# sine2pi/ASR-model

Hardware: AMD Instinct MI355X
Metric: audio-sec/sec fwd+bwd on 30s@16kHz LibriSpeech-shaped clips (whole job, all GPUs) (higher is better)
Workload: dtype bf16; 1 GPU; tiny (BASELINE configs[1]): log-mel + 4 enc/4 dec d=384 h=6 fwd+bwd, 32 x 30 s clips per GPU, T=256; model=tiny, global_batch=32, seq_len=3001, text_len=256, pitch_frames=3001, parallelism=dp1

## Files before the change

### asr-model_amd/asrx/gemm.py

```python
from __future__ import annotations

import torch

from . import lib, prec, probe

ACT = {"none": 0, "gelu": 1, "silu": 2, "sigmoid": 3, "relu": 4}


BF16 = torch.bfloat16


def is_bf16(t) -> bool:
    return t is not None and t.dtype == BF16


def gemm(A, B, C, *, M, N, K, lda, ldb, ldc, a_kc=True, b_kc=True, batch=1, sA=0, sB=0, sC=0,
         bias=None, Z=None, alpha=1.0, beta=0.0, act="none", conv_a=False, conv_b=False,
         conv_F=0, conv_C=0, splitk=1, precision=None):
    lib.require_gpu(A, B, C)
    if is_bf16(A) or is_bf16(B) or is_bf16(C):
        raise RuntimeError("asrx_gemm takes fp32 operands; bf16-stored activations go through the wide GEMM")
    p = prec.get() if precision is None else precision
    e0 = probe.begin("gemm")
    lib.call("asrx_gemm", p, lib.ptr(A), lda, sA, int(a_kc), int(conv_a), lib.ptr(B), ldb, sB,
# ... 234 lines not shown

def use_wide(K) -> bool:
    return prec.get() == prec.PREC_BF16 and K % 8 == 0


def gemm_wn_rows(A, Wb, C, *, M, N, K, lda, ldc, mtiles, bias=None, alpha=1.0, beta=0.0):
    return gemm_wn(A, Wb, C, M=M, N=N, K=K, lda=lda, ldc=ldc, bias=bias, alpha=alpha, beta=beta, mtiles=mtiles)


def row_tiles(next_i, layer, L, M, device=None):
    n = int(lib.load().asrx_row_tiles_max(M))
    dev = device if device is not None else next_i.device
    tl = torch.empty(n, dtype=torch.int32, device=dev)
    cnt = torch.empty(1, dtype=torch.int32, device=dev)
    lib.call("asrx_row_tiles", lib.ptr(next_i), layer, L, M, lib.ptr(tl), lib.ptr(cnt), lib.stream())
    return tl, cnt


def linear_fwd(x, W, b=None, act="none", out=None, preact=None, wbf=None, mtiles=None, out_bf16=False):
    x2 = _rows(x)
    if not x2.is_contiguous():
        x2 = x2.contiguous()
    M, K = x2.shape
    N = W.shape[0]
    wide = use_wide(K)
    if is_bf16(x2) and not wide:
        x2 = x2.float()
    odt = BF16 if (out_bf16 and wide and N % 4 == 0) else torch.float32
    y = out if out is not None else torch.empty(*x.shape[:-1], N, device=x.device, dtype=odt)
    if wide and mtiles is not None and act == "none" and preact is None:
        gemm_wn_rows(x2, weight_bf16(W) if wbf is None else wbf, y, M=M, N=N, K=K, lda=K, ldc=N, bias=b,
                     mtiles=mtiles)
    elif use_wide(K):
        gemm_wn(x2, weight_bf16(W) if wbf is None else wbf, y, M=M, N=N, K=K, lda=K, ldc=N, bias=b, act=act,
                Z=preact)
    else:
        gemm(x2, W, y, M=M, N=N, K=K, lda=K, ldb=K, ldc=N, a_kc=True, b_kc=True, bias=b, act=act,
             Z=preact)
    return y


def linear_rot_fwd(x, W, b, m, tab, L, hd, scale, preact=None):
    x2 = _rows(x)
    if not x2.is_contiguous():
        x2 = x2.contiguous()
    M, K = x2.shape
    N = W.shape[0]
    Wb = weight_bf16(W)
    y = torch.empty(*x.shape[:-1], N, device=x.device)
    nj = _nj(M, N)
    ab = int(is_bf16(x2))
    lib.require_gpu(x2, Wb, y, m, tab)
    e0 = probe.begin("gemm")
    lib.call("asrx_gemm_wn_rot", lib.ptr(x2), ab, K, lib.ptr(Wb), Wb.stride(0), lib.ptr(y), lib.ptr(preact), N,
             lib.ptr(b), lib.ptr(m), lib.ptr(tab), L, hd, float(scale), M, N, K, nj, lib.stream())
    probe.end("gemm", e0, 2.0 * M * N * K, ("wn", M, N, K, nj, 0, "rot", preact is not None, False, ab, 0, -1))
    return y


def linear_dgrad(dy, W, out=None, beta=0.0, mtiles=None):
    """dx = dy @ W for dy (..., N), W (N, K); mtiles as in linear_fwd."""
    d2 = _rows(dy)
    if not d2.is_contiguous():
        d2 = d2.contiguous()
    M, N = d2.shape
    K = W.shape[1]
    dx = out if out is not None else torch.empty(*dy.shape[:-1], K, device=dy.device, dtype=torch.float32)
    if use_wide(N) and mtiles is not None:
        gemm_wn_rows(d2, weight_bf16(W, trans=True), dx, M=M, N=K, K=N, lda=N, ldc=K, beta=beta, mtiles=mtiles)
    elif use_wide(N):
        gemm_wn(d2, weight_bf16(W, trans=True), dx, M=M, N=K, K=N, lda=N, ldc=K, beta=beta)
    else:
        gemm(d2, W, dx, M=M, N=K, K=N, lda=N, ldb=K, ldc=K, a_kc=True, b_kc=False, beta=beta)
    return dx


def _splitk_for(m_rows: int, tiles: int) -> int:
    want = max(1, 512 // max(tiles, 1))
    return int(max(1, min(want, m_rows // 256)))


FUSED_BIAS_GRAD = True
BIAS_CHECK = None


def _wgrad(A, lda, x2, out, M, K, rows, db=None):
    tiles = ((M + 127) // 128) * ((K + 127) // 128)
    sk = _splitk_for(rows, tiles)

    def staged(a_bf16, b_bf16, name, *tag):
        lib.require_gpu(A, x2, out)
        e0 = probe.begin("gemm")
        if db is not None and not FUSED_BIAS_GRAD:
            staged_db, db_ = db, None
        else:
            staged_db, db_ = None, db
        if db_ is not None:
            before = db_.clone() if BIAS_CHECK is not None else None
            lib.call("asrx_wgrad_bias", lib.ptr(A), a_bf16, lda, lib.ptr(x2), b_bf16, K, lib.ptr(out), out.stride(0),
                     lib.ptr(db), M, K, rows, sk, lib.stream())
            if before is not None:
                Af = A.float() if a_bf16 else A
                ref = torch.zeros(M, device=A.device)
                lib.call("asrx_colsum_ld", lib.ptr(Af), Af.stride(0) if a_bf16 else lda, lib.ptr(ref), rows, M,
                         lib.stream())
                absum = Af.as_strided((rows, M), (Af.stride(0) if a_bf16 else lda, 1)).abs().sum(0)
                tol = 1e-5 * absum + 2.0 ** -22 * (before.abs() + ref.abs())
                BIAS_CHECK.append((db_ - before, ref, tol, dict(M=M, K=K, rows=rows, sk=sk, a_bf16=a_bf16,
                                                                  b_bf16=b_bf16, lda=lda, ldo=out.stride(0))))
        elif name == "asrx_wgrad_bf16":
            lib.call(name, lib.ptr(A), lda, lib.ptr(x2), K, lib.ptr(out), out.stride(0), M, K, rows, sk, lib.stream())
        else:
            lib.call(name, lib.ptr(A), lda, lib.ptr(x2), b_bf16, K, lib.ptr(out), out.stride(0), M, K, rows, sk,
                     lib.stream())
        probe.end("gemm", e0, 2.0 * M * K * rows, ("wgrad", M, K, rows, sk) + tag)
        if staged_db is not None:
            Af = A.float() if a_bf16 else A
            lib.call("asrx_colsum_ld", lib.ptr(Af), Af.stride(0) if a_bf16 else lda, lib.ptr(staged_db), rows, M,
                     lib.stream())
        return out

    if is_bf16(A):
        xb = is_bf16(x2)
        if M % 8 or K % (8 if xb else 4) or lda % 8 or x2.stride(0) != K or A.data_ptr() % 16 or x2.data_ptr() % 16:
            A = A.float()
            lda = A.stride(0)
        else:
            return staged(1, int(xb), "asrx_wgrad_bf16_ab", 2 + int(xb))
    if is_bf16(x2):
        if M % 4 or K % 8 or lda % 4 or x2.stride(0) != K or A.data_ptr() % 16:
            x2 = x2.float()
        else:
            return staged(0, 1, "asrx_wgrad_bf16_ex", 1)
    ok4 = M % 4 == 0 and K % 4 == 0 and lda % 4 == 0 and A.data_ptr() % 16 == 0 and x2.data_ptr() % 16 == 0
    if prec.get() == prec.PREC_BF16 and ok4 and x2.stride(0) == K and (tiles <= 9 or rows <= 16384
                                                                        or (rows <= 50000 and tiles <= 72)):
        return staged(0, 0, "asrx_wgrad_bf16")
    gemm(A, x2, out, M=M, N=K, K=rows, lda=lda, ldb=K, ldc=K, a_kc=False, b_kc=False, beta=1.0, splitk=sk)
    if db is not None:
        lib.call("asrx_colsum_ld", lib.ptr(A), lda, lib.ptr(db), rows, M, lib.stream())
    return out


def wgrad_cols(dy, c0, n, x, out):
    rows, ld = dy.shape
    return _wgrad(dy[:, c0:], ld, x, out, n, x.shape[1], rows)


def linear_wgrad(dy, x, out=None, accumulate=False, db=None):
    d2 = _rows(dy)
    x2 = _rows(x)
    if not d2.is_contiguous():
        d2 = d2.contiguous()
    if not x2.is_contiguous():
        x2 = x2.contiguous()
    M, N = d2.shape
    K = x2.shape[1]
    if out is None:
        out = torch.zeros(N, K, device=dy.device, dtype=torch.float32)
    elif not accumulate:
        out.zero_()
    return _wgrad(d2, N, x2, out, N, K, M, db=db)
```

### asr-model_amd/asrx/lib.py

```python
from __future__ import annotations

import ctypes
import os

import torch

_HERE = os.path.dirname(os.path.abspath(__file__))
LIB_PATH = os.environ.get("ASRX_LIB") or os.path.join(_HERE, "libasrx.so")

_i64 = ctypes.c_int64
_i32 = ctypes.c_int
_f32 = ctypes.c_float
_p = ctypes.c_void_p
_u32 = ctypes.c_uint32

SIGNATURES = {
    "asrx_last_error": (ctypes.c_char_p, []),
    "asrx_abi_version": (_i32, []),
    "asrx_noise_hash": (_u32, [_u32, _u32]),
    "asrx_set_noise_epoch": (_i32, [_u32, _p]),
    "asrx_set_gemm_variant": (_i32, [_i32]),
    "asrx_set_attn_variant": (_i32, [_i32]),
    "asrx_set_wgrad_variant": (_i32, [_i32]),
    "asrx_mel_frames": (_i32, [_i64]),
    "asrx_logmel_ws_bytes": (_i64, [_i64, _i64]),
    "asrx_flac_info": (_i32, [_p, _i64, _p, _p, _p, _p, _p]),
    "asrx_flac_decode": (_i32, [_p, _i64, _p, _i64]),
    "asrx_pcm_normalize": (_i32, [_p, _i32, _i64, _i64, _i64, _p, _p, _p, _i64, _i32, _p]),
    "asrx_logmel": (_i32, [_p, _i64, _i64, _i64, _p, _p, _p, _p, _i32, _i64, _p, _p, _i64, _p]),
    "asrx_gemm": (
        _i32,
        [_i32, _p, _i64, _i64, _i32, _i32, _p, _i64, _i64, _i32, _i32, _p, _i64, _i64, _p, _p,
         _i64, _i64, _i64, _i64, _f32, _f32, _i32, _i64, _i64, _i32, _p],
    ),
    "asrx_abby_fwd": (_i32, [_p, _p, _p, _p, _p, _p, _p, _i64, _i64, _i64, _i64, _i64, _u32, _i32, _p]),
    "asrx_abby_fwd_logits": (_i32, [_p, _p, _p, _p, _p, _p, _i64, _i64, _i64, _i64, _i64, _u32, _i32, _p]),
    "asrx_abby_bwd": (_i32, [_p, _p, _p, _p, _p, _p, _p, _p, _p, _p, _i64, _i64, _p]),
    "asrx_attn_fwd": (_i32, [_i32, _p, _p, _p, _p, _p, _p, _p, _p, _p, _i64, _i64, _i64, _i64, _i64, _i32, _f32, _p]),
    "asrx_attn_bwd": (_i32, [_i32, _p, _p, _p, _p, _p, _p, _p, _p, _p, _p, _p, _p, _p, _p, _p, _p, _p, _p,
                             _i64, _i64, _i64, _i64, _i64, _i32, _f32, _p]),
    "asrx_layernorm_fwd": (_i32, [_p, _p, _p, _p, _p, _p, _i64, _i64, _f32, _p]),
    "asrx_layernorm_bwd": (_i32, [_p, _p, _p, _p, _p, _p, _p, _p, _i64, _i64, _p]),
    "asrx_layernorm_bwd_acc": (_i32, [_p, _p, _p, _p, _p, _p, _p, _p, _i64, _i64, _i32, _p]),
    "asrx_small_linear_fwd": (_i32, [_p, _p, _p, _p, _i64, _i64, _i64, _i32, _p]),
    "asrx_small_linear_bwd": (_i32, [_p, _p, _p, _p, _p, _p, _p, _i64, _i64, _i64, _i32, _f32, _p]),
    "asrx_rownorm": (_i32, [_p, _p, _i64, _i64, _p]),
    "asrx_rownorm_bwd": (_i32, [_p, _p, _p, _p, _i64, _i64, _p]),
    "asrx_row_normalize": (_i32, [_p, _p, _p, _i64, _i64, _p]),
    "asrx_row_normalize_bwd": (_i32, [_p, _p, _p, _p, _i64, _i64, _i32, _p]),
    "asrx_softmax_small": (_i32, [_p, _p, _i64, _i64, _p]),
    "asrx_softmax_small_bwd": (_i32, [_p, _p, _p, _i64, _i64, _p]),
    "asrx_zero": (_i32, [_p, _i64, _p]),
    "asrx_rotary_fwd": (_i32, [_p, _p, _p, _p, _i64, _i64, _i64, _i64, _f32, _p]),
    "asrx_rotary_bwd": (_i32, [_p, _p, _p, _p, _p, _p, _i64, _i64, _i64, _i64, _f32, _p]),
    "asrx_abby_bwd2": (_i32, [_p] * 10 + [_i64, _i64, _i32, _p]),
    "asrx_rownorm_bwd2": (_i32, [_p, _p, _p, _p, _i64, _i64, _i32, _p]),
    "asrx_colsum_ld": (_i32, [_p, _i64, _p, _i64, _i64, _p]),
    "asrx_ce_fwd1": (_i32, [_p] * 6 + [_i64, _i64, _p]),
    "asrx_ce_bwd2": (_i32, [_p] * 6 + [_i64, _i64, _p]),
    "asrx_bn_running": (_i32, [_p] * 5 + [_i64, _i64, _i64, _f32, _f32, _p]),
    "asrx_rsqrt_eps": (_i32, [_p, _p, _i64, _f32, _p]),
    "asrx_conv3_weight": (_i32, [_p, _p, _i64, _i64] + [_p] * 6),
    "asrx_conv3_weight_bwd": (_i32, [_p] * 4 + [_i64, _i64] + [_p] * 3),
    "asrx_blend_fwd": (_i32, [_p] * 4 + [_i64, _p]),
    "asrx_blend_bwd": (_i32, [_p] * 7 + [_i64, _p]),
    "asrx_add_segments": (_i32, [_p, _i64, _p, _p, _p, _i64, _p]),
    "asrx_cat3": (_i32, [_p] * 3 + [_i64, _p, _p]),
    "asrx_layernorm_fwd2": (_i32, [_p] * 10 + [_i32, _i64, _i64, _f32, _p]),
    "asrx_vgate_weights": (_i32, [_p] * 7 + [_i64, _i64, _i64, _p]),
    "asrx_msheath_row_fwd": (_i32, [_p] * 6 + [_i64] + [_p] * 14 + [_i64] * 4 + [_f32, _f32, _p, _i64, _i64, _p]),
    "asrx_msheath_row_bwd": (_i32, [_p] * 11 + [_i64] + [_p] * 18 + [_i64] * 4 + [_f32, _p, _i64, _i64, _p]),
    "asrx_gemm_wn_rows": (_i32, [_p, _i64, _p, _i64, _p, _i64, _p, _p, _i64, _i64, _i64, _f32, _f32, _i32, _i32, _p,
                                 _p, _p]),
    "asrx_row_tiles_max": (_i64, [_i64]),
    "asrx_wgrad_bf16": (_i32, [_p, _i64, _p, _i64, _p, _i64, _i64, _i64, _i64, _i64, _p]),
    "asrx_pitch_dio": (_i32, [_p, _i64, _i64, _i64] + [ctypes.c_double] * 5 + [_p, _i64, _p, _p, _p, _p, _i64]
                       + [_p] * 4 + [_i64] + [_p] * 4 + [_i64, _p]),
    "asrx_pitch_stonemask": (_i32, [_p, _i64, _i64, _i64, ctypes.c_double, _p, ctypes.c_double, _i64, _p, _p]),
    "asrx_wconv_entry_bytes": (_i64, []),
    "asrx_weights_to_bf16": (_i32, [_p, _i64, _i64, _p]),
    "asrx_row_tiles": (_i32, [_p, _i64, _i64, _i64, _p, _p, _p]),
    "asrx_msheath_ctrl_fwd3": (_i32, [_p, _p, _i64, _p, _p, _p, _p, _p, _i64, _p, _p, _p, _p] + [_i64] * 5 + [_p] * 8),
    "asrx_mem_chunks": (_i64, [_i64]),
    "asrx_seg_colsum_det": (_i32, [_p, _p, _p, _i64, _i64, _i64, _f32, _p]),
    "asrx_msheath_ctrl_bwd3": (_i32, [_p, _p, _p, _p, _p, _p, _i64, _p, _p, _p] + [_i64] * 4 + [_p, _i32] + [_p] * 8),
    "asrx_axpy_row2_colsum": (_i32, [_p] * 6 + [_i64] * 3 + [_p, _i64, _p]),
    "asrx_vgate_fwd": (_i32, [_p, _p, _p, _p, _p, _p, _p, _p, _p, _p, _p, _p, _p, _i64, _i64, _i64, _f32, _p]),
    "asrx_vgate_bwd": (_i32, [_p, _p, _p, _p, _p, _p, _p, _p, _p, _p, _p, _p, _p, _p, _p, _p, _p,
                              _i64, _i64, _i64, _f32, _p]),
    "asrx_tgate_fwd": (_i32, [_p, _p, _p, _i64, _i64, _p]),
    "asrx_tgate_bwd": (_i32, [_p, _p, _p, _p, _p, _i64, _i64, _p]),
    "asrx_axpy_row": (_i32, [_p, _p, _p, _p, _i64, _i64, _p]),
    "asrx_axpy_row_bwd": (_i32, [_p, _p, _p, _p, _p, _i64, _i64, _p]),
    "asrx_axpy_row_bwd2": (_i32, [_p, _p, _p, _p, _p, _p, _i64, _i64, _p]),
    "asrx_jump_select": (_i32, [_p, _p, _p, _p, _p, _p, _p, _p, _i64, _i64, _i64, _p]),
    "asrx_jump_select_bwd": (_i32, [_p, _p, _p, _p, _p, _p, _p, _p, _p, _p, _p, _p, _i64, _i64, _i64, _p]),
    "asrx_seg_colsum": (_i32, [_p, _p, _i64, _i64, _i64, _f32, _i32, _p]),
    "asrx_msheath_ctrl_fwd": (_i32, [_p, _p, _i64, _p, _p, _p, _p, _p, _p, _i64, _i64, _i64, _i64, _i64,
                                     _p, _p, _p, _p, _p, _p, _p, _p]),
    "asrx_msheath_ctrl_bwd": (_i32, [_p, _p, _p, _p, _p, _p, _p, _p, _p, _i64, _i64, _i64, _i64, _p, _p, _p, _p, _p,
                                     _p]),
    "asrx_msheath_rec_bytes": (_i64, []),
    "asrx_msheath_ctrl_fwd2": (_i32, [_p, _p, _i64, _p, _p, _p, _i64, _p, _p, _p, _i64, _i64, _i64, _i64, _i64,
                                      _p, _p, _p, _p, _p, _p, _p, _p]),
    "asrx_msheath_ctrl_bwd2": (_i32, [_p, _p, _p, _p, _p, _p, _i64, _p, _p, _p, _i64, _i64, _i64, _i64, _p, _i32,
                                      _p, _p, _p, _p, _p, _p]),
    "asrx_jump_select4_bwd_acc": (_i32, [_p, _p, _p, _p, _p, _p, _p, _p, _p, _p, _p, _p, _p, _i64, _i64, _i64, _p]),
    "asrx_jump_bwd_part_floats": (_i64, [_i64, _i64, _i64]),
    "asrx_jump_select4_bwd_part": (_i32, [_p] * 11 + [_i64, _i64, _i64, _p]),
    "asrx_msheath_ctrl_bwd4": (_i32, [_p, _i64, _p, _p, _p, _i64, _p, _p, _p, _i64, _i64, _i64, _i64, _p, _i32]
                               + [_p] * 8),
    "asrx_axpy_row2_bwd_acc": (_i32, [_p, _p, _f32, _p, _p, _p, _p, _p, _p, _p, _p, _i64, _i64, _i64, _p]),
    "asrx_msheath_dx_final": (_i32, [_p, _p, _p, _p, _i64, _i64, _i64, _p]),
    "asrx_axpy_row2": (_i32, [_p, _p, _p, _p, _p, _i64, _i64, _p]),
    "asrx_axpy_row2_bwd": (_i32, [_p, _p, _p, _p, _p, _p, _p, _i64, _i64, _p]),
    "asrx_jump_select4": (_i32, [_p, _p, _p, _p, _p, _p, _p, _p, _i64, _i64, _i64, _p]),
    "asrx_jump_select4_bwd": (_i32, [_p, _p, _p, _p, _p, _p, _p, _p, _p, _p, _p, _p, _i64, _i64, _i64, _p]),
    "asrx_colsum": (_i32, [_p, _p, _i64, _i64, _p]),
    "asrx_add_rows": (_i32, [_p, _p, _p, _p, _i64, _i64, _i64, _p]),
    "asrx_lincomb": (_i32, [_p, _p, _p, _f32, _f32, _f32, _p, _i64, _p]),
    "asrx_act_fwd": (_i32, [_p, _p, _i64, _i32, _p]),
    "asrx_act_bwd": (_i32, [_p, _p, _p, _i64, _i32, _p]),
    "asrx_glu_fwd": (_i32, [_p, _p, _i64, _i64, _p]),
    "asrx_glu_bwd": (_i32, [_p, _p, _p, _i64, _i64, _p]),
    "asrx_dropout": (_i32, [_p, _p, _i64, _i64, _i64, _i64, _u32, _f32, _p]),
    "asrx_act_dropout_fwd": (_i32, [_p, _p, _p, _i64, _i64, _i64, _i64, _u32, _f32, _i32, _i32, _p]),
    "asrx_act_dropout_bwd": (_i32, [_p, _p, _p, _i64, _i64, _i64, _i64, _u32, _f32, _i32, _i32, _p]),
    "asrx_dwconv_fwd": (_i32, [_p, _p, _p, _p, _i64, _i64, _i64, _i64, _p]),
    "asrx_dwconv_bwd": (_i32, [_p, _p, _p, _p, _p, _p, _i64, _i64, _i64, _i64, _p]),
    "asrx_bn_fwd": (_i32, [_p, _p, _p, _p, _p, _p, _i64, _i64, _i64, _f32, _i32, _p]),
    "asrx_bn_bwd": (_i32, [_p, _p, _p, _p, _p, _p, _p, _p, _p, _p, _i64, _i64, _i64, _p]),
    "asrx_dwconv_pre_bwd": (_i32, [_p, _p, _p, _p, _p, _p, _p, _i64, _i64, _i64, _i64, _i32, _p]),
    "asrx_bn_silu_fwd": (_i32, [_p, _p, _p, _p, _p, _p, _i64, _i64, _i64, _f32, _i32, _p]),
    "asrx_bn_silu_bwd": (_i32, [_p, _p, _p, _p, _p, _p, _p, _p, _p, _p, _p, _i64, _i64, _i64, _p]),
    "asrx_stem1_fwd": (_i32, [_p, _p, _p, _p, _i64, _i64, _i64, _p]),
    "asrx_stem1_bwd": (_i32, [_p, _p, _p, _p, _i64, _i64, _i64, _p]),
    "asrx_embed_fwd": (_i32, [_p, _p, _p, _i64, _i64, _p]),
    "asrx_embed_bwd": (_i32, [_p, _p, _p, _i64, _i64, _p]),
    "asrx_ce_fwd": (_i32, [_p, _p, _p, _p, _i64, _i64, _p]),
    "asrx_ce_bwd": (_i32, [_p, _p, _p, _p, _p, _i64, _i64, _p]),
    "asrx_policy_noise": (_i32, [_p, _i64, _i64, _i64, _u32, _p]),
    "asrx_weight_to_bf16": (_i32, [_p, _p, _i64, _i64, _i64, _i32, _p]),
    "asrx_gemm_wn_router": (_i32, [_p, _i64, _p, _i64, _p, _p, _p, _i64, _p, _i64, _i64, _i64, _p]),
    "asrx_gemm_wn": (_i32, [_p, _i64, _i32, _i64, _i64, _p, _i64, _p, _i64, _p, _p, _i64, _i64, _i64, _f32, _f32,
                            _i32, _i32, _p]),
    "asrx_gemm_wn_ex": (_i32, [_p, _i32, _i64, _i32, _i64, _i64, _p, _i64, _p, _i32, _i64, _p, _p, _i64, _i64, _i64,
                               _f32, _f32, _i32, _i32, _p, _p, _p]),
    "asrx_wgrad_bf16_ex": (_i32, [_p, _i64, _p, _i32, _i64, _p, _i64, _i64, _i64, _i64, _i64, _p]),
    "asrx_abby_fwd2": (_i32, [_p, _p, _p, _p, _p, _i32, _p, _p, _i64, _i64, _i64, _i64, _i64, _u32, _i32, _p, _p, _p,
                              _p]),
    "asrx_gemm_wn_gact": (_i32, [_p, _i32, _i64, _p, _i64, _p, _p, _i64, _p, _i64, _p, _i64, _i64, _i64, _i32, _i32,
                                 _p]),
    "asrx_rotary_table": (_i32, [_p, _p, _i64, _i64, _p]),
    "asrx_rotary_fwd2": (_i32, [_p, _p, _p, _p, _p, _i64, _i64, _i64, _i64, _f32, _p]),
    "asrx_rotary_bwd2": (_i32, [_p, _p, _p, _p, _p, _p, _p, _i64, _i64, _i64, _i64, _f32, _p]),
    "asrx_abby_fwd3": (_i32, [_p, _p, _p, _p, _p, _p, _i32, _p, _p, _i64, _i64, _i64, _i64, _i64, _u32, _i32, _p, _p,
                               _p, _p, _p]),
    "asrx_abby_fwd_logits2": (_i32, [_p, _p, _p, _p, _i32, _p, _p, _i64, _i64, _i64, _i64, _i64, _u32, _i32, _p, _p,
                                     _p, _p]),
    "asrx_attn_fwd2": (_i32, [_i32, _i32, _p, _p, _p, _p, _p, _p, _p, _p, _p, _i64, _i64, _i64, _i64, _i64, _i32, _f32,
                              _p]),
    "asrx_attn_bwd2": (_i32, [_i32, _i32, _p, _p, _p, _p, _p, _p, _p, _p, _p, _p, _p, _p, _p, _p, _p, _p, _p, _p,
                              _i64, _i64, _i64, _i64, _i64, _i32, _f32, _p]),
    "asrx_small_linear_fwd2": (_i32, [_p, _i32, _p, _p, _p, _i64, _i64, _i64, _i32, _p]),
    "asrx_small_linear_bwd2": (_i32, [_p, _p, _p, _i32, _p, _p, _p, _p, _i64, _i64, _i64, _i32, _f32, _p]),
    "asrx_tgate_fwd2": (_i32, [_p, _p, _p, _i32, _i64, _i64, _p]),
    "asrx_msheath_row_fwd2": (_i32, [_p] * 6 + [_i64] + [_p] * 7 + [_i32] + [_p] * 7 + [_i64] * 4
                                    + [_f32, _f32, _p, _i64, _i64, _p]),
    "asrx_msheath_row_fwd3": (_i32, [_p] * 6 + [_i64] + [_p] * 16 + [_i64] * 4 + [_f32, _f32, _p, _i64, _i64, _p]),
    "asrx_layernorm_fwd3": (_i32, [_p, _p, _p, _p, _i32] + [_p] * 6 + [_i32, _i64, _i64, _f32, _p]),
    "asrx_jump_axpy_inplace": (_i32, [_p] * 10 + [_i64, _i64, _i64, _p]),
    "asrx_wave_pool": (_i32, [_p, _i64, _i64, _i64, _i64, _p, _p]),
    "asrx_maxfactor_param_bytes": (_i32, []),
    "asrx_maxfactor_step": (_i32, [_p, _i32, _i64, _i64, _i64, _i64, _i64, _p, _p]),
    "asrx_maxfactor_step_ex": (_i32, [_p, _i32, _i64, _i64, _i64, _i64, _i64, _p, _p, _i32, _p]),
    "asrx_grad_stats_param_bytes": (_i32, []),
    "asrx_grad_stats": (_i32, [_p, _i32, _i64, _f32, _f32, _f32, _p, _p, _p]),
    "asrx_abby_record_cond": (_i32, [_p]),
    "asrx_gemm_wn_ce": (_i32, [_p, _i64, _p, _i64, _p, _i64, _p, _i64, _i64, _i64, _i32, _p]),
    "asrx_gemm_wn_ce_f32": (_i32, [_p, _i64, _p, _i64, _p, _i64, _p, _i64, _i64, _i64, _i32, _p]),
    "asrx_ce_part_fwd": (_i32, [_p, _i64] + [_p] * 6 + [_i64, _i64, _p]),
    "asrx_ce_part_fwd_f32": (_i32, [_p, _i64] + [_p] * 6 + [_i64, _i64, _p]),
    "asrx_ce_bwd_bf16": (_i32, [_p] * 6 + [_i64, _i64, _p]),
    "asrx_ce_bwd_f32in": (_i32, [_p] * 6 + [_i64, _i64, _p]),
    "asrx_wgrad_bf16_ab": (_i32, [_p, _i64, _p, _i32, _i64, _p, _i64, _i64, _i64, _i64, _i64, _p]),
    "asrx_wgrad_bias": (_i32, [_p, _i32, _i64, _p, _i32, _i64, _p, _i64, _p, _i64, _i64, _i64, _i64, _p]),
    "asrx_act_bwd_bias": (_i32, [_p, _p, _p, _p, _i64, _i64, _i32, _p]),
    "asrx_abby_fwd_res": (_i32, [_p] * 9 + [_i64] * 5 + [_u32, _i32, _p]),
    "asrx_gemm_wn_res": (_i32, [_p, _i64, _p, _i64, _p, _i64, _p, _p, _i64, _i64, _i64, _i64, _i32, _p]),
    "asrx_gemm_wn_rot": (_i32, [_p, _i32, _i64, _p, _i64, _p, _p, _i64, _p, _p, _p, _i64, _i64, _f32, _i64, _i64,
                                _i64, _i32, _p]),
    "asrx_msheath_plan_bytes": (_i64, []),
    "asrx_msheath_layer_bytes": (_i64, []),
    "asrx_msheath_fwd_ws_bytes": (_i64, [_p, _i64, _i64, _i64]),
    "asrx_msheath_fwd": (_i32, [_p, _p, _p, _i64, _p, _p, _i64, _i64, _i64, _i64, _p]),
# ... 95 lines not shown
```

### asr-model_amd/asrx/msheath.py

```python
from __future__ import annotations

import ctypes
import math

import torch

from . import gemm as G
from . import decisions, lib, ops, prec

_E = torch.empty
_P = lib.ptr
_S = lib.stream
SIG = G.ACT["sigmoid"]
SILU = G.ACT["silu"]

_REC = None

ROW_DIMS = (128, 256, 384, 512, 768, 1024)

DETERMINISTIC = True
ROW_COLSUM = __import__("os").environ.get("ASRX_ROW_COLSUM", "1") != "0"


def _rec_bytes():
    global _REC
    if _REC is None:
        _REC = int(lib.load().asrx_msheath_rec_bytes())
    return _REC


def supported(mod, D):
    return D in ROW_DIMS and all(lay["v_gate"].mkey.shape[0] <= 64 for lay in mod.layers)


def _params(mod):
    ps = [mod.pnet.net[0].weight, mod.pnet.net[0].bias, mod.pnet.net[2].weight, mod.pnet.net[2].bias, mod.mem_w,
          mod.mem_gate[0].weight, mod.mem_gate[0].bias, mod.jump_s, mod.mlp_gate[0].weight, mod.mlp_gate[0].bias,
          mod.mlp_ln.weight, mod.mlp_ln.bias, mod.mlp[0].weight, mod.mlp[0].bias, mod.mlp[2].weight, mod.mlp[2].bias]
    for i, lay in enumerate(mod.layers):
        vg = lay["v_gate"]
        ps += [lay["ln"].weight, lay["ln"].bias, lay["gate"][0].weight, lay["gate"][0].bias, vg.mkey, vg.mval,
               vg.mlp[0].weight, vg.mlp[0].bias, vg.mlp[2].weight, vg.mlp[2].bias, vg.concat.weight, vg.concat.bias]
        if lay["adapter"] is not None:
            ps += [lay["adapter"].weight, lay["adapter"].bias]
    return ps


ACT_SOFTMAX = 16


def forward(mod, x0, gpol, save, tag=None):
    B, L, D = x0.shape
    rows = B * L
    dev = x0.device
    st = _S()
    sv = {} if save else None
    nchunk = int(lib.load().asrx_mem_chunks(L))
    part = _E(len(mod.layers) + 1, B, nchunk, D, device=dev)
    pooled = _E(B, D, device=dev)
    lib.call("asrx_seg_colsum_det", _P(x0), _P(part[-1]), _P(pooled), B, L, D, 1.0 / L, st)
    net = mod.pnet.net
    zp = _E(B, net[0].weight.shape[0], device=dev) if save else None
    hp = G.linear_fwd(pooled, net[0].weight, net[0].bias, act="silu", preact=zp)
    policy = _E(B, 3, device=dev)
    lib.call("asrx_small_linear_fwd", _P(hp), _P(net[2].weight), _P(net[2].bias), _P(policy), B, hp.shape[1], 3,
             ACT_SOFTMAX, st)
    nl = len(mod.layers)
    wide = G.use_wide(D)
    mg = mod.mem_gate[0]
    mem_w, ld_mw = mod.mem_w, 0
    next_i = None
    x = x0
    rec_bytes = _rec_bytes()
    wsr = _E(nl, 7, rows, device=dev)
    wsb = _E(nl, 5, B, device=dev)
    wsd = _E(nl, 3, B, D, device=dev)
    wsc = _E(nl, B * rec_bytes, dtype=torch.uint8, device=dev)
    a_r, a_b, a_d, a_c = wsr.data_ptr(), wsb.data_ptr(), wsd.data_ptr(), wsc.data_ptr()
    if save:
        sv["ws"] = (wsr, wsb, wsd, wsc)
    inv_sqrt_d = 1.0 / math.sqrt(D)
    layers = []
    for i, lay in enumerate(mod.layers):
        vg = lay["v_gate"]
        Dh = vg.mlp[0].weight.shape[0]
        M = vg.mkey.shape[0]
        N = M + Dh

        def build(vg=vg, M=M, Dh=Dh, N=N):
            Wc, bc, mkn = _E(N, D, device=dev), _E(N, device=dev), _E(M, device=dev)
            wb = _E(N, D, dtype=torch.int16, device=dev) if wide else None
            lib.call("asrx_vgate_weights", _P(vg.mkey), _P(vg.mlp[0].weight), _P(vg.mlp[0].bias), _P(Wc), _P(bc),
                     _P(mkn), _P(wb), M, Dh, D, st)
            return Wc, bc, mkn, wb

        Wc, bc, mkn, wb = G.derived(("vgate", bool(wide)), build, (vg.mkey, vg.mlp[0].weight, vg.mlp[0].bias))
        mt = G.row_tiles(next_i, i, L, rows, dev) if (wide and next_i is not None) else None
        SH = G.linear_fwd(x, Wc, bc, wbf=wb, mtiles=mt)
        ln, gt = lay["ln"], lay["gate"][0]
        ad = lay["adapter"]
        pxb = int(ad is not None and wide and prec.bf16_storage())
        px = _E(B, L, D, device=dev, dtype=torch.bfloat16 if pxb else torch.float32)
        mean, rstd, nx, gv, ion, kv, m2 = (a_r + 4 * rows * (7 * i + j) for j in range(7))
        x_new = _E(B, L, D, device=dev) if save else None
        if ad is None and ROW_COLSUM:
            lib.call("asrx_msheath_row_fwd3", _P(x), _P(ln.weight), _P(ln.bias), _P(gt.weight), _P(gt.bias), _P(SH),
                     N, _P(vg.mval), _P(vg.mlp[2].weight), _P(vg.mlp[2].bias), _P(vg.concat.weight),
                     _P(vg.concat.bias), _P(vg.tx), _P(px), _P(mean), _P(rstd), _P(nx), _P(gv), _P(ion), _P(kv), _P(m2),
                     _P(x_new), _P(part[i]), rows, D, M, Dh, float(ln.eps), inv_sqrt_d, _P(next_i), i, L, st)
            out = px
        else:
            lib.call("asrx_msheath_row_fwd2", _P(x), _P(ln.weight), _P(ln.bias), _P(gt.weight), _P(gt.bias), _P(SH),
                     N, _P(vg.mval), _P(vg.mlp[2].weight), _P(vg.mlp[2].bias), _P(vg.concat.weight),
                     _P(vg.concat.bias), _P(vg.tx), _P(px), pxb, _P(mean), _P(rstd), _P(nx), _P(gv), _P(ion), _P(kv),
                     _P(m2), rows, D, M, Dh, float(ln.eps), inv_sqrt_d, _P(next_i), i, L, st)
            out = G.linear_fwd(px, ad.weight, ad.bias, mtiles=mt) if ad is not None else px
            lib.call("asrx_axpy_row2_colsum", _P(x), _P(gv), _P(ion), _P(out), _P(x_new), _P(part[i]), B, L, D,
                     _P(next_i), i, st)
        alpha, beta, active, next_out, mem_v = (a_b + 4 * B * (5 * i + j) for j in range(5))
        gam, mwo, mem = (a_d + 4 * B * D * (3 * i + j) for j in range(3))
        rec = a_c + B * rec_bytes * i
        gp = gpol[:, i]
        lib.call("asrx_msheath_ctrl_fwd3", _P(policy), _P(gp), gp.stride(0), _P(ion), _P(mg.weight), _P(mg.bias),
                 _P(mem_v), _P(mem_w), ld_mw, _P(part[i]), _P(mem), _P(mod.jump_s), _P(next_i), i, nl, B, L, D,
                 _P(alpha), _P(beta), _P(gam), _P(mwo), _P(active), _P(next_out), _P(rec), st)
        if tag is not None and decisions.active():
            decisions.msheath_layer(tag[0], tag[1], i, wsr[i, 4].view(B, L), wsc[i].view(torch.float32).view(B, -1))
        if save:
            x_out = _E(B, L, D, device=dev)
            lib.call("asrx_jump_select4", _P(x_new), _P(x0), _P(x), _P(active), _P(alpha), _P(beta), _P(gam),
                     _P(x_out), B, L, D, st)
        else:
            x_out = _E(B, L, D, device=dev) if i == 0 else x
            lib.call("asrx_jump_axpy_inplace", _P(x), _P(x_out), _P(gv), _P(ion), _P(out), _P(x0), _P(active),
                     _P(alpha), _P(beta), _P(gam), B, L, D, st)
        if save:
            layers.append(dict(x=x, Wc=Wc, mkn=mkn, SH=SH, nx=nx, kv=kv, m2=m2, px=px, mean=mean, rstd=rstd,
                               out=out, g=gv, ion=ion, x_new=x_new, mem=mem, mem_v=mem_v, mem_w=mem_w, ld_mw=ld_mw,
                               rec=rec, active=active, alpha=alpha, beta=beta, next_i=next_i, mt=mt))
        mem_w, ld_mw, next_i = mwo, D, next_out
        x = x_out
    gate = _E(rows, device=dev)
    hb = int(wide and prec.bf16_storage())
    hln = _E(B, L, D, device=dev, dtype=torch.bfloat16 if hb else torch.float32)
    mean2, rstd2 = _E(rows, device=dev), _E(rows, device=dev)
    lib.call("asrx_layernorm_fwd3", _P(x), _P(mod.mlp_ln.weight), _P(mod.mlp_ln.bias), _P(hln), hb, _P(mean2),
             _P(rstd2), None, _P(mod.mlp_gate[0].weight), _P(mod.mlp_gate[0].bias), _P(gate), 1, rows, D,
             float(mod.mlp_ln.eps), st)
    rec1 = save and G.can_recompute_act(hln, mod.mlp[0].weight, "silu")
    z1 = _E(B, L, mod.mlp[0].weight.shape[0], device=dev) if save and not rec1 else None
    a1 = G.linear_fwd(hln, mod.mlp[0].weight, mod.mlp[0].bias, act="silu", preact=z1,
                      out_bf16=prec.bf16_storage())
    hh = G.linear_fwd(a1, mod.mlp[2].weight, mod.mlp[2].bias)
    y = _E(B, L, D, device=dev)
    lib.call("asrx_axpy_row", _P(x), _P(gate), _P(hh), _P(y), rows, D, st)
    if save:
        sv.update(x0=x0, pooled=pooled, zp=zp, hp=hp, policy=policy, layers=layers, x=x, gate=gate, hln=hln,
                  mean2=mean2, rstd2=rstd2, z1=z1, a1=a1, hh=hh)
    return y, sv


class MSheathFn(torch.autograd.Function):
    @staticmethod
    def forward(ctx, x0, gpol, mod, tag, *params):
        x0 = x0 if x0.is_contiguous() else x0.contiguous()
        y, sv = forward(mod, x0, gpol, save=True, tag=tag)
        ctx.mod, ctx.sv = mod, sv
        return y

    @staticmethod
    def backward(ctx, gy):
        mod, sv = ctx.mod, ctx.sv
        ctx.sv = None
        gy = gy if gy.is_contiguous() else gy.contiguous()
        x0 = sv["x0"]
        B, L, D = x0.shape
        rows = B * L
        dev = x0.device
        st = _S()
        touched = []

        def gb(p):
            touched.append(p)
            return ops._gbuf(p, True)

        x = sv["x"]
        dx = _E(B, L, D, device=dev)
        dhh = _E(B, L, D, device=dev)
        dgate = _E(rows, device=dev)
        lib.call("asrx_axpy_row_bwd2", _P(gy), _P(sv["gate"]), _P(sv["hh"]), _P(dhh), _P(dgate), _P(dx), rows, D, st)
        mg = mod.mlp_gate[0]
        lib.call("asrx_small_linear_bwd", _P(dgate), _P(sv["gate"]), _P(x), _P(mg.weight), _P(dx), _P(gb(mg.weight)),
                 _P(gb(mg.bias)), rows, D, 1, SIG, 1.0, st)
        m0, m2l = mod.mlp[0], mod.mlp[2]
        da1 = G.linear_dgrad(dhh, m2l.weight)
        G.linear_wgrad(dhh, sv["a1"], out=gb(m2l.weight), accumulate=True, db=gb(m2l.bias))
        H1 = da1.shape[-1]
        if sv["z1"] is None:
            ga1 = _E(da1.shape, dtype=torch.bfloat16, device=dev)
            G.linear_gact(sv["hln"], m0.weight, m0.bias, da1, ga1, "silu", db=gb(m0.bias))
            da1 = ga1
        elif prec.get() == prec.PREC_BF16 and H1 % 8 == 0 and G.use_wide(H1):
            ga1 = _E(da1.shape, dtype=torch.bfloat16, device=dev)
            lib.call("asrx_act_bwd_bias", _P(da1), _P(sv["z1"]), _P(ga1), _P(gb(m0.bias)), rows, H1, SILU, st)
            da1 = ga1
        else:
            lib.call("asrx_act_bwd", _P(da1), _P(sv["z1"]), _P(da1), da1.numel(), SILU, st)
            ops.colsum(da1.view(rows, -1), out=gb(m0.bias))
        dhln = G.linear_dgrad(da1, m0.weight)
        G.linear_wgrad(da1, sv["hln"], out=gb(m0.weight), accumulate=True)
        lib.call("asrx_layernorm_bwd_acc", _P(dhln), _P(x), _P(mod.mlp_ln.weight), _P(sv["mean2"]), _P(sv["rstd2"]),
                 _P(dx), _P(gb(mod.mlp_ln.weight)), _P(gb(mod.mlp_ln.bias)), rows, D, 1, st)
        del dhh, da1, dhln
        nl = len(mod.layers)
        g_policy = _E(B, 3, device=dev)
        has_orig = _E(B, dtype=torch.int32, device=dev)
        lib.call("asrx_zero", _P(has_orig), B * 4, st)
        dorig = _E(B, L, D, device=dev)
        g_mwo = None
        mg_w, mg_b = mod.mem_gate[0].weight, mod.mem_gate[0].bias
        inv_sqrt_d = 1.0 / math.sqrt(D)
        for i in range(nl - 1, -1, -1):
            s = sv["layers"][i]
            lay = mod.layers[i]
            vg = lay["v_gate"]
            M, Dh = vg.mkey.shape[0], vg.mlp[0].weight.shape[0]
            N = M + Dh
            xi = s["x"]
            dxi = _E(B, L, D, device=dev)
            dxn = _E(B, L, D, device=dev)
            g_mem_w, g_mem = _E(B, D, device=dev), _E(B, D, device=dev)
            if DETERMINISTIC:
                part = _E(int(lib.load().asrx_jump_bwd_part_floats(B, L, D)), device=dev)
                lib.call("asrx_jump_select4_bwd_part", _P(dx), _P(s["x_new"]), _P(x0), _P(s["active"]),
                         _P(s["alpha"]), _P(s["beta"]), _P(has_orig), _P(dxn), _P(dorig), _P(dxi), _P(part), B, L, D,
                         st)
                lib.call("asrx_msheath_ctrl_bwd4", _P(part), L, _P(g_mwo), _P(s["mem_v"]), _P(s["mem_w"]),
                         s["ld_mw"], _P(s["mem"]), _P(mod.jump_s), _P(s["rec"]), i, nl, B, D, _P(g_policy),
                         int(i != nl - 1), _P(g_mem_w), _P(g_mem), _P(gb(mod.jump_s)), _P(has_orig), _P(mg_w),
                         _P(gb(mg_w)), _P(gb(mg_b)), st)
            else:
                dctl = _E(B * (2 + D), device=dev)
                dalpha, dbeta, dgam = dctl[:B], dctl[B:2 * B], dctl[2 * B:]
                lib.call("asrx_jump_select4_bwd_acc", _P(dx), _P(s["x_new"]), _P(x0), _P(s["active"]),
                         _P(s["alpha"]), _P(s["beta"]), _P(has_orig), _P(dxn), _P(dorig), _P(dxi), _P(dalpha),
                         _P(dbeta), _P(dgam), B, L, D, st)
                lib.call("asrx_msheath_ctrl_bwd3", _P(dalpha), _P(dbeta), _P(dgam), _P(g_mwo), _P(s["mem_v"]),
                         _P(s["mem_w"]), s["ld_mw"], _P(s["mem"]), _P(mod.jump_s), _P(s["rec"]), i, nl, B, D,
                         _P(g_policy), int(i != nl - 1), _P(g_mem_w), _P(g_mem), _P(gb(mod.jump_s)), _P(has_orig),
                         _P(mg_w), _P(gb(mg_w)), _P(gb(mg_b)), st)
            dout = _E(B, L, D, device=dev)
            dgv, dion = _E(rows, device=dev), _E(rows, device=dev)
            lib.call("asrx_axpy_row2_bwd_acc", _P(dxn), _P(g_mem), 1.0 / L, _P(s["active"]), _P(s["g"]), _P(s["ion"]),
                     _P(s["out"]), _P(dout), _P(dgv), _P(dion), _P(dxi), B, L, D, st)
            del dxn
            ad = lay["adapter"]
            if ad is not None:
                dpx = G.linear_dgrad(dout, ad.weight, mtiles=s["mt"])
                G.linear_wgrad(dout, s["px"], out=gb(ad.weight), accumulate=True, db=gb(ad.bias))
            else:
                dpx = dout
            ln, gt = lay["ln"], lay["gate"][0]
            dSH = _E(rows, N, device=dev)
            lib.call("asrx_msheath_row_bwd", _P(dpx), _P(xi), _P(ln.weight), _P(ln.bias), _P(s["mean"]),
                     _P(s["rstd"]), _P(dgv), _P(s["g"]), _P(gt.weight), _P(dion), _P(s["SH"]), N, _P(s["nx"]),
                     _P(vg.mval), _P(vg.mlp[2].weight), _P(vg.concat.weight), _P(s["kv"]), _P(s["m2"]), _P(dxi),
                     _P(gb(ln.weight)), _P(gb(ln.bias)), _P(gb(gt.weight)), _P(gb(gt.bias)), _P(dSH),
                     _P(gb(vg.mval)), _P(gb(vg.mlp[2].weight)), _P(gb(vg.mlp[2].bias)), _P(gb(vg.concat.weight)),
                     _P(gb(vg.concat.bias)), _P(gb(vg.mlp[0].bias)), rows, D, M, Dh, inv_sqrt_d, _P(s["next_i"]), i,
                     L, st)
            del dout, dpx
            G.linear_dgrad(dSH, s["Wc"], out=dxi, beta=1.0, mtiles=s["mt"])
            x2 = xi.view(rows, D)
            dmk = _E(M, D, device=dev)
            lib.call("asrx_zero", _P(dmk), dmk.numel() * 4, st)
            G.wgrad_cols(dSH, 0, M, x2, dmk)
            lib.call("asrx_row_normalize_bwd", _P(dmk), _P(s["Wc"]), _P(s["mkn"]), _P(gb(vg.mkey)), M, D, 1, st)
            G.wgrad_cols(dSH, M, Dh, x2, gb(vg.mlp[0].weight))
            del dSH, dmk
            g_mwo = g_mem_w
            dx = dxi
        lib.call("asrx_colsum", _P(g_mwo), _P(gb(mod.mem_w)), B, D, st)
        net = mod.pnet.net
        g_pl = _E(B, 3, device=dev)
        lib.call("asrx_softmax_small_bwd", _P(g_policy), _P(sv["policy"]), _P(g_pl), B, 3, st)
        dhp = _E(sv["hp"].shape, device=dev)
        lib.call("asrx_small_linear_bwd", _P(g_pl), None, _P(sv["hp"]), _P(net[2].weight), _P(dhp),
                 _P(gb(net[2].weight)), _P(gb(net[2].bias)), B, dhp.shape[1], 3, 0, 0.0, st)
        lib.call("asrx_act_bwd", _P(dhp), _P(sv["zp"]), _P(dhp), dhp.numel(), SILU, st)
        dpooled = G.linear_dgrad(dhp, net[0].weight)
        G.linear_wgrad(dhp, sv["pooled"], out=gb(net[0].weight), accumulate=True)
        ops.colsum(dhp, out=gb(net[0].bias))
        u = _E(B, D, device=dev)
        lib.call("asrx_lincomb", _P(dpooled), None, None, 1.0 / L, 0.0, 0.0, _P(u), B * D, st)
        lib.call("asrx_msheath_dx_final", _P(dx), _P(dorig), _P(has_orig), _P(u), B, L, D, st)
        seen = set()
        for p in touched:
            if id(p) not in seen:
                seen.add(id(p))
                ops._gret(p, p.grad, True)
        return (dx, None, None, None) + (None,) * len(ctx.needs_input_grad[4:])


COMPOSITE = True


class _Layer(ctypes.Structure):
    _fields_ = [(n, ctypes.c_void_p) for n in ("ln_w", "ln_b", "gate_w", "gate_b", "mval", "vw2", "vb2", "cw", "cb",
                                                "tx", "bc", "wcb", "ad_wb", "ad_b")] + \
               [("M", ctypes.c_int64), ("Dh", ctypes.c_int64), ("ln_eps", ctypes.c_float), ("px_bf16", ctypes.c_int32)]


class _Plan(ctypes.Structure):
    _fields_ = [("p0_wb", ctypes.c_void_p), ("p0_b", ctypes.c_void_p), ("p2_w", ctypes.c_void_p),
                ("p2_b", ctypes.c_void_p), ("p_hidden", ctypes.c_int64), ("mem_w", ctypes.c_void_p),
                ("mg_w", ctypes.c_void_p), ("mg_b", ctypes.c_void_p), ("jump_s", ctypes.c_void_p),
                ("mln_w", ctypes.c_void_p), ("mln_b", ctypes.c_void_p), ("mln_eps", ctypes.c_float),
                ("hln_bf16", ctypes.c_int32), ("mgate_w", ctypes.c_void_p), ("mgate_b", ctypes.c_void_p),
                ("m0_wb", ctypes.c_void_p), ("m0_b", ctypes.c_void_p), ("m2_wb", ctypes.c_void_p),
                ("m2_b", ctypes.c_void_p), ("H1", ctypes.c_int64), ("a1_bf16", ctypes.c_int32),
                ("n_layers", ctypes.c_int32), ("layers", ctypes.c_void_p)]


def _composite_ok(mod, x, gpol, tag):
    from . import probe
    D = x.shape[-1]
    H1 = mod.mlp[0].weight.shape[0]
    return (COMPOSITE and ROW_COLSUM and prec.get() == prec.PREC_BF16 and G.use_wide(D) and G.use_wide(H1) and H1 % 4 == 0
            and G._nj_override is None and not probe.active() and not (tag is not None and decisions.active())
            and x.is_cuda and gpol.is_contiguous() and gpol.dtype == torch.float32 and x.dtype == torch.float32)


def _build_plan(mod, D):
    dev = mod.mem_w.device
    st = _S()
    wide = True
    store = prec.bf16_storage()
    keep = []

    def a(t):
        if t is None:
            return None
        keep.append(t)
        return t.data_ptr()

    layers = (_Layer * len(mod.layers))()
    for i, lay in enumerate(mod.layers):
        vg = lay["v_gate"]
        Dh, M = vg.mlp[0].weight.shape[0], vg.mkey.shape[0]
        N = M + Dh

        def build(vg=vg, M=M, Dh=Dh, N=N):
            Wc, bc, mkn = _E(N, D, device=dev), _E(N, device=dev), _E(M, device=dev)
            wb = _E(N, D, dtype=torch.int16, device=dev) if wide else None
            lib.call("asrx_vgate_weights", _P(vg.mkey), _P(vg.mlp[0].weight), _P(vg.mlp[0].bias), _P(Wc), _P(bc),
                     _P(mkn), _P(wb), M, Dh, D, st)
            return Wc, bc, mkn, wb

        Wc, bc, mkn, wb = G.derived(("vgate", bool(wide)), build, (vg.mkey, vg.mlp[0].weight, vg.mlp[0].bias))
        ad = lay["adapter"]
        ln, gt = lay["ln"], lay["gate"][0]
# ... 47 lines not shown
```

### asr-model_amd/csrc/gemm_wg.hip

```cpp
#include "common.h"

namespace asrx {
namespace wg {

constexpr int TM = 128, TN = 128, TK = 32, NT = 256;
typedef __attribute__((ext_vector_type(8))) __bf16 bf16x8;
typedef __attribute__((ext_vector_type(4))) float f32x4;
typedef short v4i16 __attribute__((ext_vector_type(4)));
typedef __attribute__((address_space(3))) v4i16 lds_v4i16;

__device__ __attribute__((aligned(16))) float zero16[4];

struct Params {
  const float* A;
  const float* B;
  float* C;
  int64_t lda, ldb, ldc;
  int M, N;
  int64_t R, kchunk;
  int splitk;
  float* db;
};

__device__ __forceinline__ int off(int row, int ch) { return 256 * row + 16 * (ch ^ (((row & 3) << 2) | ((row >> 2) & 3))); }

typedef unsigned u32x4 __attribute__((ext_vector_type(4)));
template <bool ABF, bool BBF>
struct Stage {
  float4 a[4], b[4];
};
template <>
struct Stage<false, true> {
  float4 a[4];
  u32x4 bh[2];
};
template <>
struct Stage<true, true> {
  u32x4 ah[2], bh[2];
};
template <>
struct Stage<true, false> {
  u32x4 ah[2];
  float4 b[4];
};

template <bool ABF, bool BBF>
__device__ __forceinline__ void load(const Params& p, Stage<ABF, BBF>& st, int64_t r0, int64_t rend, int m0, int n0) {
  const int t = threadIdx.x;
  const int c = 4 * (t & 31);
  const int cb = 8 * (t & 15);
  if constexpr (BBF) {
    const unsigned short* Bh = reinterpret_cast<const unsigned short*>(p.B);
#pragma unroll
    for (int i = 0; i < 2; ++i) {
      const int64_t r = r0 + (t >> 4) + 16 * i;
      st.bh[i] = *reinterpret_cast<const u32x4*>((r < rend && n0 + cb < p.N) ? (const void*)(Bh + r * p.ldb + n0 + cb)
                                                                            : (const void*)zero16);
    }
  }
  if constexpr (ABF) {
    const unsigned short* Ah = reinterpret_cast<const unsigned short*>(p.A);
#pragma unroll
    for (int i = 0; i < 2; ++i) {
      const int64_t r = r0 + (t >> 4) + 16 * i;
      st.ah[i] = *reinterpret_cast<const u32x4*>((r < rend && m0 + cb < p.M) ? (const void*)(Ah + r * p.lda + m0 + cb)
                                                                            : (const void*)zero16);
    }
    if constexpr (!BBF) {
#pragma unroll
      for (int i = 0; i < 4; ++i) {
        const int64_t r = r0 + (t >> 5) + 8 * i;
        st.b[i] = *reinterpret_cast<const float4*>((r < rend && n0 + c < p.N) ? (const void*)(p.B + r * p.ldb + n0 + c)
                                                                              : (const void*)zero16);
      }
    }
  } else {
#pragma unroll
    for (int i = 0; i < 4; ++i) {
      const int64_t r = r0 + (t >> 5) + 8 * i;
      const bool okr = r < rend;
      st.a[i] = *reinterpret_cast<const float4*>((okr && m0 + c < p.M) ? (const void*)(p.A + r * p.lda + m0 + c)
                                                                       : (const void*)zero16);
      if constexpr (!BBF)
        st.b[i] = *reinterpret_cast<const float4*>((okr && n0 + c < p.N) ? (const void*)(p.B + r * p.ldb + n0 + c)
                                                                         : (const void*)zero16);
    }
  }
}

template <bool ABF, bool BBF>
__device__ __forceinline__ void store(const Stage<ABF, BBF>& st, char* Ai, char* Bi) {
  const int t = threadIdx.x;
  const int c = 4 * (t & 31);
  const int ch = c >> 3, hb = (c >> 2) & 1;
  typedef __attribute__((ext_vector_type(4))) __bf16 bf16x4;
  if constexpr (ABF) {
#pragma unroll
    for (int i = 0; i < 2; ++i) *reinterpret_cast<u32x4*>(Ai + off((t >> 4) + 16 * i, t & 15)) = st.ah[i];
    if constexpr (!BBF) {
#pragma unroll
      for (int i = 0; i < 4; ++i) {
        const int row = (t >> 5) + 8 * i;
        bf16x4 hb4;
        hb4[0] = (__bf16)st.b[i].x; hb4[1] = (__bf16)st.b[i].y; hb4[2] = (__bf16)st.b[i].z; hb4[3] = (__bf16)st.b[i].w;
        *reinterpret_cast<bf16x4*>(Bi + off(row, ch) + 8 * hb) = hb4;
      }
    }
  } else {
#pragma unroll
    for (int i = 0; i < 4; ++i) {
      const int row = (t >> 5) + 8 * i;
      bf16x4 ha;
      ha[0] = (__bf16)st.a[i].x; ha[1] = (__bf16)st.a[i].y; ha[2] = (__bf16)st.a[i].z; ha[3] = (__bf16)st.a[i].w;
      *reinterpret_cast<bf16x4*>(Ai + off(row, ch) + 8 * hb) = ha;
      if constexpr (!BBF) {
        bf16x4 hb4;
        hb4[0] = (__bf16)st.b[i].x; hb4[1] = (__bf16)st.b[i].y; hb4[2] = (__bf16)st.b[i].z; hb4[3] = (__bf16)st.b[i].w;
        *reinterpret_cast<bf16x4*>(Bi + off(row, ch) + 8 * hb) = hb4;
      }
    }
  }
  if constexpr (BBF) {
#pragma unroll
    for (int i = 0; i < 2; ++i) *reinterpret_cast<u32x4*>(Bi + off((t >> 4) + 16 * i, t & 15)) = st.bh[i];
  }
}

__device__ __forceinline__ bf16x8 frag(const char* img, int c0, int lane) {
  const int g = lane >> 4, gi = lane & 15, q = gi >> 2, p = gi & 3;
  const int col = c0 + 4 * p;
  const int ch = col >> 3, hb = (col >> 2) & 1;
  const v4i16 t1 = __builtin_amdgcn_ds_read_tr16_b64_v4i16((lds_v4i16*)(img + off(8 * g + q, ch) + 8 * hb));
  const v4i16 t2 = __builtin_amdgcn_ds_read_tr16_b64_v4i16((lds_v4i16*)(img + off(8 * g + 4 + q, ch) + 8 * hb));
  typedef short v8i16 __attribute__((ext_vector_type(8)));
  const v8i16 a8 = {t1[0], t1[1], t1[2], t1[3], t2[0], t2[1], t2[2], t2[3]};
  return __builtin_bit_cast(bf16x8, a8);
}

__device__ __forceinline__ int xcd_item(int bid, int nblk) {
  const int xcd = bid & 7, q = nblk >> 3, r = nblk & 7;
  return (xcd < r ? xcd * (q + 1) : r * (q + 1) + (xcd - r) * q) + (bid >> 3);
}

template <bool ABF, bool BBF>
__device__ __forceinline__ void colacc(const Stage<ABF, BBF>& st, float (&cs)[8]) {
  if constexpr (ABF) {
#pragma unroll
    for (int i = 0; i < 2; ++i)
#pragma unroll
      for (int w = 0; w < 4; ++w) {
        const unsigned u = st.ah[i][w];
        cs[2 * w] += __builtin_bit_cast(float, u << 16);
        cs[2 * w + 1] += __builtin_bit_cast(float, u & 0xffff0000u);
      }
  } else {
#pragma unroll
    for (int i = 0; i < 4; ++i) {
      cs[0] += st.a[i].x;
      cs[1] += st.a[i].y;
      cs[2] += st.a[i].z;
      cs[3] += st.a[i].w;
    }
  }
}

template <bool ABF, bool BBF>
__global__ __launch_bounds__(NT, 2) void wgrad_wr_kernel(Params p) {
  __shared__ __attribute__((aligned(16))) char Ai[2][TK * TM * 2];
  __shared__ __attribute__((aligned(16))) char Bi[2][TK * TN * 2];
  const int nN = (p.N + TN - 1) / TN, nM = (p.M + TM - 1) / TM;
  const int ntile = nM * nN;
  const int item = xcd_item(blockIdx.x, gridDim.x);
  const int split = item / ntile, tile = item % ntile;
  const int m0 = (tile / nN) * TM, n0 = (tile % nN) * TN;
  const int64_t rb = (int64_t)split * p.kchunk, re = min<int64_t>(p.R, rb + p.kchunk);
  const int nk = rb < re ? (int)((re - rb + TK - 1) / TK) : 0;
  const int lane = threadIdx.x & 63, wid = threadIdx.x >> 6;
  const int wm = wid >> 1, wn = wid & 1;

  f32x4 acc[4][4];
#pragma unroll
  for (int i = 0; i < 4; ++i)
#pragma unroll
    for (int j = 0; j < 4; ++j) acc[i][j] = f32x4{0.f, 0.f, 0.f, 0.f};

  Stage<ABF, BBF> s0, s1;
  const bool dbon = p.db && n0 == 0;
  float cs[8] = {0.f, 0.f, 0.f, 0.f, 0.f, 0.f, 0.f, 0.f};
  load(p, s0, rb, re, m0, n0);
  load(p, s1, rb + TK, re, m0, n0);
  if (dbon && nk > 0) colacc(s0, cs);
  store(s0, Ai[0], Bi[0]);
  __syncthreads();

  auto kstep = [&](int s, Stage<ABF, BBF>& cur, const Stage<ABF, BBF>& nxt) __attribute__((always_inline)) {
    load(p, cur, rb + (int64_t)(s + 2) * TK, re, m0, n0);
    const char* At = Ai[s & 1];
    const char* Bt = Bi[s & 1];
    bf16x8 a[4], b[4];
#pragma unroll
    for (int mt = 0; mt < 4; ++mt) a[mt] = frag(At, wm * 64 + mt * 16, lane);
#pragma unroll
    for (int nt = 0; nt < 4; ++nt) b[nt] = frag(Bt, wn * 64 + nt * 16, lane);
#pragma unroll
    for (int mt = 0; mt < 4; ++mt)
#pragma unroll
      for (int nt = 0; nt < 4; ++nt)
        acc[mt][nt] = __builtin_amdgcn_mfma_f32_16x16x32_bf16(a[mt], b[nt], acc[mt][nt], 0, 0, 0);
    if (s + 1 < nk) {
      if (dbon) colacc(nxt, cs);
      store(nxt, Ai[(s + 1) & 1], Bi[(s + 1) & 1]);
    }
    __syncthreads();
  };
  for (int s = 0; s < nk; s += 2) {
    kstep(s, s0, s1);
    if (s + 1 < nk) kstep(s + 1, s1, s0);
  }

  const int ln = lane & 15, lm = 4 * (lane >> 4);
#pragma unroll
  for (int mt = 0; mt < 4; ++mt)
#pragma unroll
    for (int nt = 0; nt < 4; ++nt) {
      const int n = n0 + wn * 64 + nt * 16 + ln;
      if (n >= p.N) continue;
#pragma unroll
      for (int r = 0; r < 4; ++r) {
        const int m = m0 + wm * 64 + mt * 16 + lm + r;
        if (m < p.M && nk > 0) atomicAdd(p.C + (int64_t)m * p.ldc + n, acc[mt][nt][r]);
      }
    }
  if (dbon && nk > 0) {
    constexpr int F = ABF ? 8 : 4;
#pragma unroll
    for (int f = 0; f < F; ++f) {
      cs[f] += __shfl_xor(cs[f], 32);
      if (ABF) cs[f] += __shfl_xor(cs[f], 16);
    }
    __syncthreads();
    float* red = reinterpret_cast<float*>(Ai[0]);
    const int t = threadIdx.x, lane = t & 63;
    const bool wr = ABF ? lane < 16 : lane < 32;
    if (wr) {
      const int f0 = ABF ? 8 * (lane & 15) : 4 * (lane & 31);
#pragma unroll
      for (int f = 0; f < F; ++f) red[(t >> 6) * TM + f0 + f] = cs[f];
    }
    __syncthreads();
    if (t < TM && m0 + t < p.M)
      atomicAdd(p.db + m0 + t, red[t] + red[TM + t] + red[2 * TM + t] + red[3 * TM + t]);
  }
}

constexpr int TN3 = 384, NT3 = 512;
__device__ __forceinline__ int off3(int row, int ch) {
  return 768 * row + 16 * ((ch & ~15) | ((ch ^ (((row & 3) << 2) | ((row >> 2) & 3))) & 15));
}
__device__ __forceinline__ bf16x8 frag3(const char* img, int c0, int lane) {
  const int g = lane >> 4, gi = lane & 15, q = gi >> 2, p = gi & 3;
  const int col = c0 + 4 * p;
  const int ch = col >> 3, hb = (col >> 2) & 1;
  const v4i16 t1 = __builtin_amdgcn_ds_read_tr16_b64_v4i16((lds_v4i16*)(img + off3(8 * g + q, ch) + 8 * hb));
  const v4i16 t2 = __builtin_amdgcn_ds_read_tr16_b64_v4i16((lds_v4i16*)(img + off3(8 * g + 4 + q, ch) + 8 * hb));
  typedef short v8i16 __attribute__((ext_vector_type(8)));
  const v8i16 a8 = {t1[0], t1[1], t1[2], t1[3], t2[0], t2[1], t2[2], t2[3]};
  return __builtin_bit_cast(bf16x8, a8);
}
template <bool BBF>
struct Stage3 {
  float4 a[2];
  float4 b[6];
};
template <>
struct Stage3<true> {
  float4 a[2];
  u32x4 bh[3];
};
template <bool BBF>
__device__ __forceinline__ void load3(const Params& p, Stage3<BBF>& st, int64_t r0, int64_t rend, int m0, int n0) {
  const int t = threadIdx.x;
  const int c = 4 * (t & 31);
#pragma unroll
  for (int i = 0; i < 2; ++i) {
    const int64_t r = r0 + (t >> 5) + 16 * i;
    st.a[i] = *reinterpret_cast<const float4*>((r < rend && m0 + c < p.M) ? (const void*)(p.A + r * p.lda + m0 + c)
                                                                          : (const void*)zero16);
  }
  if constexpr (BBF) {
    const unsigned short* Bh = reinterpret_cast<const unsigned short*>(p.B);
#pragma unroll
    for (int i = 0; i < 3; ++i) {
      const int q = t + NT3 * i;
      const int64_t r = r0 + q / 48;
      const int f = 8 * (q % 48);
      st.bh[i] = *reinterpret_cast<const u32x4*>((r < rend && n0 + f < p.N) ? (const void*)(Bh + r * p.ldb + n0 + f)
                                                                            : (const void*)zero16);
    }
  } else {
#pragma unroll
    for (int i = 0; i < 6; ++i) {
      const int q = t + NT3 * i;
      const int64_t r = r0 + q / 96;
      const int f = 4 * (q % 96);
      st.b[i] = *reinterpret_cast<const float4*>((r < rend && n0 + f < p.N) ? (const void*)(p.B + r * p.ldb + n0 + f)
                                                                            : (const void*)zero16);
    }
  }
}
template <bool BBF>
__device__ __forceinline__ void store3(const Stage3<BBF>& st, char* Ai, char* Bi) {
  const int t = threadIdx.x;
  typedef __attribute__((ext_vector_type(4))) __bf16 bf16x4;
// ... 115 lines not shown
    if (t < TM && m0 + t < p.M) {
      float v = red[t];
#pragma unroll
      for (int w = 1; w < NT3 / 64; ++w) v += red[w * TM + t];
      atomicAdd(p.db + m0 + t, v);
    }
  }
}

}
}

using namespace asrx;

static int g_wgrad_variant = 1;
extern "C" int asrx_set_wgrad_variant(int v) {
  const int old = g_wgrad_variant;
  g_wgrad_variant = v;
  return old;
}

static int wgrad_launch(const void* A, int a_bf16, int64_t lda, const void* B, int b_bf16, int64_t ldb, float* C,
                        int64_t ldc, int64_t M, int64_t N, int64_t R, int64_t splitk, hipStream_t stream,
                        float* db = nullptr) {
  ASRX_REQUIRE(M > 0 && N > 0 && R >= 0, "asrx_wgrad_bf16: empty problem");
  ASRX_REQUIRE(M % 4 == 0 && N % 4 == 0 && lda % 4 == 0 && ldb % 4 == 0, "asrx_wgrad_bf16: M, N, lda, ldb %% 4 required");
  ASRX_REQUIRE(!b_bf16 || (N % 8 == 0 && ldb % 8 == 0), "asrx_wgrad_bf16: a bf16 X needs N, ldb %% 8");
  ASRX_REQUIRE(!a_bf16 || (M % 8 == 0 && lda % 8 == 0), "asrx_wgrad_bf16: a bf16 dY needs M, lda %% 8");
  ASRX_REQUIRE((((uintptr_t)A | (uintptr_t)B) & 15) == 0, "asrx_wgrad_bf16: operands must be 16-byte aligned");
  if (R == 0) return 0;
  if (splitk < 1) splitk = 1;
  int64_t kchunk = (R + splitk - 1) / splitk;
  kchunk = (kchunk + wg::TK - 1) / wg::TK * wg::TK;
  splitk = (R + kchunk - 1) / kchunk;
  if (!a_bf16 && b_bf16 && g_wgrad_variant == 1 && N % wg::TN3 == 0 && R >= 4096 &&
      ((M + wg::TM - 1) / wg::TM) * (N / wg::TN3) >= 8) {
    static int cus = 0;
    if (!cus) {
      int dev = 0;
      (void)hipGetDevice(&dev);
      (void)hipDeviceGetAttribute(&cus, hipDeviceAttributeMultiprocessorCount, dev);
      cus = cus > 0 ? cus : 1;
    }
    const int64_t tiles = ((M + wg::TM - 1) / wg::TM) * (N / wg::TN3);
    int64_t sk = cus / tiles;
    if (sk > R / 512) sk = R / 512;
    if (sk < 1) sk = 1;
    int64_t kc = (R + sk - 1) / sk;
    kc = (kc + wg::TK - 1) / wg::TK * wg::TK;
    sk = (R + kc - 1) / kc;
    wg::Params p3{(const float*)A, (const float*)B, C, lda, ldb, ldc, (int)M, (int)N, R, kc, (int)sk, db};
    wg::wgrad_w3_kernel<true><<<(unsigned)(tiles * sk), wg::NT3, 0, stream>>>(p3);
    ASRX_LAUNCHED("asrx_wgrad_bf16");
  }
  wg::Params p{(const float*)A, (const float*)B, C, lda, ldb, ldc, (int)M, (int)N, R, kchunk, (int)splitk, db};
  const int64_t items = ((M + wg::TM - 1) / wg::TM) * ((N + wg::TN - 1) / wg::TN) * splitk;
  ASRX_REQUIRE(items < (1LL << 31), "asrx_wgrad_bf16: too many work items");
  if (a_bf16 && b_bf16)
    wg::wgrad_wr_kernel<true, true><<<(unsigned)items, wg::NT, 0, stream>>>(p);
  else if (a_bf16)
    wg::wgrad_wr_kernel<true, false><<<(unsigned)items, wg::NT, 0, stream>>>(p);
  else if (b_bf16)
    wg::wgrad_wr_kernel<false, true><<<(unsigned)items, wg::NT, 0, stream>>>(p);
  else
    wg::wgrad_wr_kernel<false, false><<<(unsigned)items, wg::NT, 0, stream>>>(p);
  ASRX_LAUNCHED("asrx_wgrad_bf16");
}

extern "C" int asrx_wgrad_bf16(const float* A, int64_t lda, const float* B, int64_t ldb, float* C, int64_t ldc,
                               int64_t M, int64_t N, int64_t R, int64_t splitk, hipStream_t stream) {
  return wgrad_launch(A, 0, lda, B, 0, ldb, C, ldc, M, N, R, splitk, stream);
}

extern "C" int asrx_wgrad_bf16_ex(const float* A, int64_t lda, const void* B, int b_bf16, int64_t ldb, float* C,
                                  int64_t ldc, int64_t M, int64_t N, int64_t R, int64_t splitk, hipStream_t stream) {
  return wgrad_launch(A, 0, lda, B, b_bf16, ldb, C, ldc, M, N, R, splitk, stream);
}

extern "C" int asrx_wgrad_bf16_ab(const void* A, int64_t lda, const void* B, int b_bf16, int64_t ldb, float* C,
                                  int64_t ldc, int64_t M, int64_t N, int64_t R, int64_t splitk, hipStream_t stream) {
  return wgrad_launch(A, 1, lda, B, b_bf16, ldb, C, ldc, M, N, R, splitk, stream);
}

extern "C" int asrx_wgrad_bias(const void* A, int a_bf16, int64_t lda, const void* B, int b_bf16, int64_t ldb,
                               float* C, int64_t ldc, float* db, int64_t M, int64_t N, int64_t R, int64_t splitk,
                               hipStream_t stream) {
  ASRX_REQUIRE(db, "asrx_wgrad_bias: db required");
  return wgrad_launch(A, a_bf16, lda, B, b_bf16, ldb, C, ldc, M, N, R, splitk, stream, db);
}
```

### asr-model_amd/csrc/msheath.hip

```cpp
#include <type_traits>
#include "common.h"

namespace asrx {

struct CtrlRec {
  float ys[3];
  float action;
  float low;
  float jump_g;
  float cg;
  float act;
};

template <int CT>
__global__ __launch_bounds__(CT) void msheath_ctrl_fwd_kernel(
    const float* __restrict__ policy, const float* __restrict__ gpol, int64_t ld_gpol, const float* __restrict__ ion,
    const float* __restrict__ mem_v, const float* __restrict__ mem_w, const float* __restrict__ mem,
    const float* __restrict__ jump_s, const float* __restrict__ next_i, int layer_i, int layers, int64_t L, int D,
    float* __restrict__ alpha, float* __restrict__ beta, float* __restrict__ gam, float* __restrict__ mem_w_out,
    float* __restrict__ active, float* __restrict__ next_out, CtrlRec* __restrict__ rec, int64_t ld_mem_w,
    const float* __restrict__ mg_w, const float* __restrict__ mg_b, float* __restrict__ mem_v_out,
    const float* __restrict__ mem_part, int nchunk, float* __restrict__ mem_out) {
  __shared__ float red[CT / 64];
  const int64_t b = blockIdx.x;
// ... 361 lines not shown
  const int64_t l0 = (int64_t)(blockIdx.x / cchunks) * lchunk;
  const int64_t l1 = min(L, l0 + lchunk);
  const int c4 = cc * 32 + lane;
  const bool a = act[b] != 0.f;
  const float al = alpha[b], be = beta[b];
  float sa = 0.f, sb = 0.f;
  float4 sgv = make_float4(0.f, 0.f, 0.f, 0.f);
  const float4 z4 = make_float4(0.f, 0.f, 0.f, 0.f);
  if (c4 < d4) {
    for (int64_t l = l0 + grp; l < l1; l += 8) {
      const int64_t i = (b * L + l) * d4 + c4;
      const float4 gv = g[i];
      if (a) {
        const float4 u = xn[i], v = orig[i];
        sa += gv.x * u.x + gv.y * u.y + gv.z * u.z + gv.w * u.w;
        sb += gv.x * v.x + gv.y * v.y + gv.z * v.z + gv.w * v.w;
        sgv.x += gv.x; sgv.y += gv.y; sgv.z += gv.z; sgv.w += gv.w;
        dxn[i] = make_float4(al * gv.x, al * gv.y, al * gv.z, al * gv.w);
        dorig[i] = make_float4(be * gv.x, be * gv.y, be * gv.z, be * gv.w);
        dxold[i] = z4;
      } else {
        dxn[i] = z4;
        dorig[i] = z4;
        dxold[i] = gv;
      }
    }
  }
  if (!a) return;
  sg_s[grp][lane] = sgv;
  sa = wave_sum(sa);
  sb = wave_sum(sb);
  if ((threadIdx.x & 63) == 0) {
    red[0][threadIdx.x >> 6] = sa;
    red[1][threadIdx.x >> 6] = sb;
  }
  __syncthreads();
  if (threadIdx.x < 128) {
    const int cl = threadIdx.x >> 2, q = threadIdx.x & 3;
    const int c4b = cc * 32 + cl;
    if (c4b < d4) {
      float t = 0.f;
      for (int g2 = 0; g2 < 8; ++g2) {
        const float4 v = sg_s[g2][cl];
        t += q == 0 ? v.x : q == 1 ? v.y : q == 2 ? v.z : v.w;
      }
      atomicAdd(dgam + b * 4 * d4 + 4 * c4b + q, t);
    }
  } else if (threadIdx.x == 128) {
    atomicAdd(dalpha + b, red[0][0] + red[0][1] + red[0][2] + red[0][3]);
    atomicAdd(dbeta + b, red[1][0] + red[1][1] + red[1][2] + red[1][3]);
  }
}

__global__ __launch_bounds__(256) void jump_select4_bwd_acc_kernel(
    const float4* __restrict__ g, const float4* __restrict__ xn, const float4* __restrict__ orig,
    const float* __restrict__ act, const float* __restrict__ alpha, const float* __restrict__ beta,
    const int* __restrict__ has_orig, float4* __restrict__ dxn, float4* __restrict__ dorig, float4* __restrict__ dx,
    float* __restrict__ dalpha, float* __restrict__ dbeta, float* __restrict__ dgam, int64_t L, int d4, int lchunk,
    float2* __restrict__ part_ab = nullptr, float* __restrict__ part_g = nullptr) {
  __shared__ float4 sg_s[8][32];
  __shared__ float red[2][4];
  const int lane = threadIdx.x & 31, grp = threadIdx.x >> 5;
  const int cchunks = (d4 + 31) / 32;
  const int cc = blockIdx.x % cchunks;
  const int lc = blockIdx.x / cchunks, nlc = gridDim.x / cchunks;
  const int64_t b = blockIdx.y;
  const int64_t l0 = (int64_t)lc * lchunk;
  const int64_t l1 = min(L, l0 + lchunk);
  const int c4 = cc * 32 + lane;
  const bool a = act[b] != 0.f;
  const float al = alpha[b], be = beta[b];
  const bool jo = be != 0.f, acc_o = has_orig[b] != 0;
  float sa = 0.f, sb = 0.f;
  float4 sgv = make_float4(0.f, 0.f, 0.f, 0.f);
  if (c4 < d4) {
    for (int64_t l = l0 + grp; l < l1; l += 8) {
      const int64_t i = (b * L + l) * d4 + c4;
      const float4 gv = g[i];
      if (a) {
        const float4 u = xn[i], v = orig[i];
        sa += gv.x * u.x + gv.y * u.y + gv.z * u.z + gv.w * u.w;
        sb += gv.x * v.x + gv.y * v.y + gv.z * v.z + gv.w * v.w;
        sgv.x += gv.x; sgv.y += gv.y; sgv.z += gv.z; sgv.w += gv.w;
        dxn[i] = make_float4(al * gv.x, al * gv.y, al * gv.z, al * gv.w);
        if (jo) {
          float4 o = make_float4(be * gv.x, be * gv.y, be * gv.z, be * gv.w);
          if (acc_o) {
            const float4 p = dorig[i];
            o.x += p.x; o.y += p.y; o.z += p.z; o.w += p.w;
          }
          dorig[i] = o;
        }
      } else {
        dx[i] = gv;
      }
    }
  }
  if (!a && !part_g) return;
  sg_s[grp][lane] = sgv;
  sa = wave_sum(sa);
  sb = wave_sum(sb);
  if ((threadIdx.x & 63) == 0) {
    red[0][threadIdx.x >> 6] = sa;
    red[1][threadIdx.x >> 6] = sb;
  }
  __syncthreads();
  if (threadIdx.x < 128) {
    const int cl = threadIdx.x >> 2, q = threadIdx.x & 3;
    const int c4b = cc * 32 + cl;
    if (c4b < d4) {
      float t = 0.f;
      for (int g2 = 0; g2 < 8; ++g2) {
        const float4 v = sg_s[g2][cl];
        t += q == 0 ? v.x : q == 1 ? v.y : q == 2 ? v.z : v.w;
      }
      if (part_g)
        part_g[(b * nlc + lc) * 4 * d4 + 4 * c4b + q] = t;
      else
        atomicAdd(dgam + b * 4 * d4 + 4 * c4b + q, t);
    }
  } else if (threadIdx.x == 128) {
    const float A = red[0][0] + red[0][1] + red[0][2] + red[0][3];
    const float Bv = red[1][0] + red[1][1] + red[1][2] + red[1][3];
    if (part_ab) {
      part_ab[(b * nlc + lc) * cchunks + cc] = make_float2(A, Bv);
    } else {
      atomicAdd(dalpha + b, A);
      atomicAdd(dbeta + b, Bv);
    }
  }
}

__global__ __launch_bounds__(256) void axpy_row2_bwd_acc_kernel(const float4* __restrict__ dxn,
                                                                const float* __restrict__ gm, float invL,
                                                                const float* __restrict__ act,
                                                                const float* __restrict__ s1, const float* __restrict__ s2,
                                                                const float4* __restrict__ y, float4* __restrict__ dy,
                                                                float* __restrict__ ds1, float* __restrict__ ds2,
                                                                float4* __restrict__ dx, int64_t rows, int64_t L, int d4) {
  const int lane = threadIdx.x & 63;
  const float4 z4 = make_float4(0.f, 0.f, 0.f, 0.f);
  for (int64_t r = (int64_t)blockIdx.x * 4 + (threadIdx.x >> 6); r < rows; r += (int64_t)gridDim.x * 4) {
    const int64_t b = r / L;
    if (act[b] == 0.f) {
      for (int j = lane; j < d4; j += 64) dy[r * d4 + j] = z4;
      if (lane == 0) {
        ds1[r] = 0.f;
        if (ds2) ds2[r] = 0.f;
      }
      continue;
    }
    const float a = s1[r], c = s2 ? s2[r] : 1.f;
    const float sc = a * c;
    const float4* gm4 = reinterpret_cast<const float4*>(gm + b * 4 * d4);
    float t = 0.f;
    for (int j = lane; j < d4; j += 64) {
      float4 gv = dxn[r * d4 + j];
      if (gm) {
        const float4 m = gm4[j];
        gv.x += m.x * invL; gv.y += m.y * invL; gv.z += m.z * invL; gv.w += m.w * invL;
      }
      const float4 yv = y[r * d4 + j];
      t += gv.x * yv.x + gv.y * yv.y + gv.z * yv.z + gv.w * yv.w;
      dy[r * d4 + j] = make_float4(sc * gv.x, sc * gv.y, sc * gv.z, sc * gv.w);
      dx[r * d4 + j] = gv;
    }
    t = wave_sum(t);
    if (lane == 0) {
      ds1[r] = c * t;
      if (ds2) ds2[r] = a * t;
    }
  }
}

__global__ void msheath_dx_final_kernel(float4* __restrict__ dx, const float4* __restrict__ dorig,
                                        const int* __restrict__ has_orig, const float4* __restrict__ u, int64_t B,
                                        int64_t L, int d4) {
  const int64_t total = B * L * d4;
  for (int64_t i = (int64_t)blockIdx.x * blockDim.x + threadIdx.x; i < total; i += (int64_t)gridDim.x * blockDim.x) {
    const int64_t b = i / (L * d4);
    float4 v = dx[i];
    if (u) {
      const float4 w = u[b * d4 + i % d4];
      v.x += w.x; v.y += w.y; v.z += w.z; v.w += w.w;
    }
    if (has_orig[b]) {
      const float4 w = dorig[i];
      v.x += w.x; v.y += w.y; v.z += w.z; v.w += w.w;
    }
    dx[i] = v;
  }
}

}

using namespace asrx;


template <typename... A>
static void ctrl_fwd_launch(int64_t D, int64_t B, hipStream_t stream, A... a) {
  if (D > 512) msheath_ctrl_fwd_kernel<512><<<(unsigned)B, 512, 0, stream>>>(a...);
  else msheath_ctrl_fwd_kernel<256><<<(unsigned)B, 256, 0, stream>>>(a...);
}

extern "C" {

int asrx_jump_select4_bwd_acc(const float* g, const float* xn, const float* orig, const float* act,
                              const float* alpha, const float* beta, const int* has_orig, float* dxn, float* dorig,
                              float* dx, float* dalpha, float* dbeta, float* dgam, int64_t B, int64_t L, int64_t d,
                              hipStream_t stream) {
  ASRX_REQUIRE(d % 4 == 0, "asrx_jump_select4_bwd_acc: d % 4 != 0");
  if (B * L == 0) return 0;
  if (dbeta == dalpha + B && dgam == dalpha + 2 * B) {
    (void)hipMemsetAsync(dalpha, 0, B * (2 + d) * sizeof(float), stream);
  } else {
    (void)hipMemsetAsync(dalpha, 0, B * sizeof(float), stream);
    (void)hipMemsetAsync(dbeta, 0, B * sizeof(float), stream);
    (void)hipMemsetAsync(dgam, 0, B * d * sizeof(float), stream);
  }
  const int d4 = (int)(d / 4);
  const int lchunk = 128;
  dim3 grid((unsigned)(((d4 + 31) / 32) * ((L + lchunk - 1) / lchunk)), (unsigned)B);
  jump_select4_bwd_acc_kernel<<<grid, 256, 0, stream>>>((const float4*)g, (const float4*)xn, (const float4*)orig, act,
                                                        alpha, beta, has_orig, (float4*)dxn, (float4*)dorig,
                                                        (float4*)dx, dalpha, dbeta, dgam, L, d4, lchunk);
  ASRX_LAUNCHED("asrx_jump_select4_bwd_acc");
}

int64_t asrx_jump_bwd_part_floats(int64_t B, int64_t L, int64_t d) {
  const int64_t nlc = (L + 127) / 128, ncc = (d / 4 + 31) / 32;
  return B * nlc * (2 * ncc + d);
}

int asrx_jump_select4_bwd_part(const float* g, const float* xn, const float* orig, const float* act,
                               const float* alpha, const float* beta, const int* has_orig, float* dxn, float* dorig,
                               float* dx, float* part, int64_t B, int64_t L, int64_t d, hipStream_t stream) {
  ASRX_REQUIRE(d % 4 == 0, "asrx_jump_select4_bwd_part: d % 4 != 0");
  if (B * L == 0) return 0;
  const int d4 = (int)(d / 4);
  const int lchunk = 128;
  const int64_t nlc = (L + lchunk - 1) / lchunk, ncc = (d4 + 31) / 32;
  float2* part_ab = reinterpret_cast<float2*>(part);
  float* part_g = part + 2 * B * nlc * ncc;
  dim3 grid((unsigned)(ncc * nlc), (unsigned)B);
  jump_select4_bwd_acc_kernel<<<grid, 256, 0, stream>>>((const float4*)g, (const float4*)xn, (const float4*)orig, act,
                                                        alpha, beta, has_orig, (float4*)dxn, (float4*)dorig,
                                                        (float4*)dx, nullptr, nullptr, nullptr, L, d4, lchunk,
                                                        part_ab, part_g);
  ASRX_LAUNCHED("asrx_jump_select4_bwd_part");
}

int asrx_axpy_row2_bwd_acc(const float* dxn, const float* gm, float invL, const float* act, const float* s1,
                           const float* s2, const float* y, float* dy, float* ds1, float* ds2, float* dx, int64_t B,
                           int64_t L, int64_t d, hipStream_t stream) {
  ASRX_REQUIRE(d % 4 == 0, "asrx_axpy_row2_bwd_acc: d % 4 != 0");
  const int64_t rows = B * L;
  if (rows == 0) return 0;
  axpy_row2_bwd_acc_kernel<<<(unsigned)std::min<int64_t>((rows + 3) / 4, 8192), 256, 0, stream>>>(
      (const float4*)dxn, gm, invL, act, s1, s2, (const float4*)y, (float4*)dy, ds1, ds2, (float4*)dx, rows, L,
      (int)(d / 4));
  ASRX_LAUNCHED("asrx_axpy_row2_bwd_acc");
}

int asrx_msheath_dx_final(float* dx, const float* dorig, const int* has_orig, const float* u, int64_t B, int64_t L,
                          int64_t d, hipStream_t stream) {
  ASRX_REQUIRE(d % 4 == 0, "asrx_msheath_dx_final: d % 4 != 0");
  if (B * L == 0) return 0;
  const int64_t n = B * L * d / 4;
  msheath_dx_final_kernel<<<(unsigned)std::min<int64_t>((n + 255) / 256, 16384), 256, 0, stream>>>(
      (float4*)dx, (const float4*)dorig, has_orig, (const float4*)u, B, L, (int)(d / 4));
  ASRX_LAUNCHED("asrx_msheath_dx_final");
}

int asrx_msheath_ctrl_fwd(const float* policy, const float* gpol, int64_t ld_gpol, const float* ion,
                          const float* mem_v, const float* mem_w, const float* mem, const float* jump_s,
                          const float* next_i, int64_t layer_i, int64_t layers, int64_t B, int64_t L, int64_t D,
                          float* alpha, float* beta, float* gam, float* mem_w_out, float* active, float* next_out,
                          void* rec, hipStream_t stream) {
  if (B == 0) return 0;
  ctrl_fwd_launch(D, B, stream, policy, gpol, ld_gpol, ion, mem_v, mem_w, mem, jump_s,
                                                           next_i, (int)layer_i, (int)layers, L, (int)D, alpha, beta,
                                                           gam, mem_w_out, active, next_out, (CtrlRec*)rec, D, nullptr,
                                                           nullptr, nullptr, nullptr, 0, nullptr);
  ASRX_LAUNCHED("asrx_msheath_ctrl_fwd");
}

int asrx_msheath_ctrl_fwd2(const float* policy, const float* gpol, int64_t ld_gpol, const float* ion,
                           const float* mem_v, const float* mem_w, int64_t ld_mem_w, const float* mem,
                           const float* jump_s, const float* next_i, int64_t layer_i, int64_t layers, int64_t B,
                           int64_t L, int64_t D, float* alpha, float* beta, float* gam, float* mem_w_out, float* active,
                           float* next_out, void* rec, hipStream_t stream) {
  if (B == 0) return 0;
  ctrl_fwd_launch(D, B, stream, policy, gpol, ld_gpol, ion, mem_v, mem_w, mem, jump_s,
                                                           next_i, (int)layer_i, (int)layers, L, (int)D, alpha, beta,
                                                           gam, mem_w_out, active, next_out, (CtrlRec*)rec, ld_mem_w,
                                                           nullptr, nullptr, nullptr, nullptr, 0, nullptr);
  ASRX_LAUNCHED("asrx_msheath_ctrl_fwd2");
}

int asrx_msheath_ctrl_fwd3(const float* policy, const float* gpol, int64_t ld_gpol, const float* ion,
                           const float* mg_w, const float* mg_b, float* mem_v_out, const float* mem_w,
                           int64_t ld_mem_w, const float* mem_part, float* mem, const float* jump_s,
                           const float* next_i, int64_t layer_i, int64_t layers, int64_t B, int64_t L, int64_t D,
                           float* alpha, float* beta, float* gam, float* mem_w_out, float* active, float* next_out,
                           void* rec, hipStream_t stream) {
  if (B == 0) return 0;
  const int nchunk = (int)((L + MEM_CHUNK - 1) / MEM_CHUNK);
  ctrl_fwd_launch(D, B, stream, policy, gpol, ld_gpol, ion, nullptr, mem_w, mem, jump_s,
                                                           next_i, (int)layer_i, (int)layers, L, (int)D, alpha, beta,
                                                           gam, mem_w_out, active, next_out, (CtrlRec*)rec, ld_mem_w,
                                                           mg_w, mg_b, mem_v_out, mem_part, nchunk, mem);
  ASRX_LAUNCHED("asrx_msheath_ctrl_fwd3");
}

int asrx_msheath_ctrl_bwd(const float* g_alpha, const float* g_beta, const float* g_gam, const float* g_mwo,
                          const float* mem_v, const float* mem_w, const float* mem, const float* jump_s,
                          const void* rec, int64_t layer_i, int64_t layers, int64_t B, int64_t D, float* g_policy,
                          float* g_mem_v, float* g_mem_w, float* g_mem, float* g_jump_s, hipStream_t stream) {
  if (B == 0) return 0;
  msheath_ctrl_bwd_kernel<<<(unsigned)B, 256, 0, stream>>>(g_alpha, g_beta, g_gam, g_mwo, mem_v, mem_w, mem, jump_s,
                                                           (const CtrlRec*)rec, (int)layer_i, (int)layers, (int)D,
                                                           g_policy, g_mem_v, g_mem_w, g_mem, g_jump_s, D, nullptr, 0,
                                                           nullptr, nullptr, nullptr);
  ASRX_LAUNCHED("asrx_msheath_ctrl_bwd");
}

int asrx_msheath_ctrl_bwd2(const float* g_alpha, const float* g_beta, const float* g_gam, const float* g_mwo,
                           const float* mem_v, const float* mem_w, int64_t ld_mem_w, const float* mem,
                           const float* jump_s, const void* rec, int64_t layer_i, int64_t layers, int64_t B, int64_t D,
                           float* g_policy, int acc_policy, float* g_mem_v, float* g_mem_w, float* g_mem,
                           float* g_jump_s, int* has_orig, hipStream_t stream) {
  if (B == 0) return 0;
  msheath_ctrl_bwd_kernel<<<(unsigned)B, 256, 0, stream>>>(g_alpha, g_beta, g_gam, g_mwo, mem_v, mem_w, mem, jump_s,
                                                           (const CtrlRec*)rec, (int)layer_i, (int)layers, (int)D,
                                                           g_policy, g_mem_v, g_mem_w, g_mem, g_jump_s, ld_mem_w,
                                                           has_orig, acc_policy, nullptr, nullptr, nullptr);
  ASRX_LAUNCHED("asrx_msheath_ctrl_bwd2");
}

int asrx_msheath_ctrl_bwd3(const float* g_alpha, const float* g_beta, const float* g_gam, const float* g_mwo,
                           const float* mem_v, const float* mem_w, int64_t ld_mem_w, const float* mem,
                           const float* jump_s, const void* rec, int64_t layer_i, int64_t layers, int64_t B, int64_t D,
                           float* g_policy, int acc_policy, float* g_mem_w, float* g_mem, float* g_jump_s,
                           int* has_orig, const float* mg_w, float* g_mg_w, float* g_mg_b, hipStream_t stream) {
// ... 105 lines not shown
```

### asr-model_amd/csrc/rowops.hip

```cpp
#include "common.h"
#include <algorithm>
#include <mutex>
#include <map>
#include <unordered_map>
#include <utility>

namespace asrx {

constexpr int RW = 4;

__device__ __forceinline__ int64_t row_begin() { return (int64_t)blockIdx.x * RW + (threadIdx.x >> 6); }
__device__ __forceinline__ int64_t row_step() { return (int64_t)gridDim.x * RW; }

static unsigned row_grid(int64_t rows, int64_t cap = 8192) {
  int64_t g = (rows + RW - 1) / RW;
  if (g > cap) g = cap;
  if (g < 1) g = 1;
  return (unsigned)g;
}
static unsigned ew_grid(int64_t n, int64_t cap = 16384) {
  int64_t g = (n + 255) / 256;
  if (g > cap) g = cap;
  if (g < 1) g = 1;
  return (unsigned)g;
// ... 521 lines not shown
                                                                const float* __restrict__ W1,
                                                                const float* __restrict__ b1, float* __restrict__ Wc,
                                                                float* __restrict__ bc, float* __restrict__ mkn,
                                                                unsigned short* __restrict__ wb, int M, int Dh, int D) {
  const int lane = threadIdx.x & 63;
  for (int64_t r = row_begin(); r < M + Dh; r += row_step()) {
    const bool key = r < M;
    const float* src = key ? mkey + r * D : W1 + (r - M) * D;
    float nn = 1.f;
    if (key) {
      float s = 0.f;
      for (int j = lane; j < D; j += 64) s += src[j] * src[j];
      nn = fmaxf(sqrtf(wave_sum(s)), 1e-12f);
    }
    for (int j = lane; j < D; j += 64) {
      const float v = key ? src[j] / nn : src[j];
      Wc[r * D + j] = v;
      if (wb) wb[r * D + j] = __builtin_bit_cast(unsigned short, (__bf16)v);
    }
    if (lane == 0) {
      if (key) mkn[r] = nn;
      bc[r] = key ? 0.f : b1[r - M];
    }
  }
}

struct MSRowFwd {
  const float *x, *lnw, *lnb, *gw, *gb;
  const float *SH, *mval, *w2, *b2, *cw, *cb, *tx;
  float *px, *mean, *rstd, *nx, *g, *ion, *kv, *m2;
  int64_t rows, ldsh;
  int M, Dh;
  float eps, inv_sqrt_d;
  const float* next_i;
  int layer;
  int64_t L;
  unsigned short* pxb;
  float* part;
  float* xnew;
  int nchunk;
  int nofill;
};

template <int E>
__global__ __launch_bounds__(64 * RW) void msheath_row_fwd_kernel(MSRowFwd p) {
  constexpr int D = 64 * E;
  const int lane = threadIdx.x & 63;
  float wv[E], bv[E], gwv[E];
  ld_lane<E>(p.lnw, lane, wv);
  ld_lane<E>(p.lnb, lane, bv);
  ld_lane<E>(p.gw, lane, gwv);
  const float gbias = p.gb[0];
  const float mv_l = lane < p.M ? p.mval[lane] : 0.f;
  const float b2 = p.b2[0], cw0 = p.cw[0], cw1 = p.cw[1], cb = p.cb[0], tx = p.tx[0];
  extern __shared__ float ni_s[];
  if (p.next_i) {
    const int nb = (int)((p.rows + p.L - 1) / p.L);
    for (int b = threadIdx.x; b < nb; b += 64 * RW) ni_s[b] = p.next_i[b];
    __syncthreads();
  }
  auto at_layer = [&](int64_t rr) __attribute__((always_inline)) -> bool {
    return !p.next_i || ni_s[(unsigned)rr / (unsigned)p.L] == (float)p.layer;
  };
  constexpr int HQ = (E + 1) / 2;
  float w2v[HQ];
#pragma unroll
  for (int i = 0; i < HQ; ++i) w2v[i] = lane + 64 * i < p.Dh ? p.w2[lane + 64 * i] : 0.f;
  float csum[E];
  auto fetch = [&](int64_t rr, float (&xs)[E], float& ss, float (&hs)[HQ]) __attribute__((always_inline)) {
    const int64_t rc = (rr < p.rows && at_layer(rr)) ? rr : 0;
    ld_lane<E>(p.x + rc * D, lane, xs);
    const float* S = p.SH + rc * p.ldsh;
    ss = S[lane < p.M ? lane : 0];
#pragma unroll
    for (int i = 0; i < HQ; ++i) hs[i] = S[p.M + min(lane + 64 * i, p.Dh - 1)];
  };
  auto row_body = [&](int64_t r, const float (&xv)[E], float sv, const float (&hv)[HQ]) __attribute__((always_inline)) {
    if (!at_layer(r)) {
      if (p.nofill) return;
      float z[E];
#pragma unroll
      for (int e = 0; e < E; ++e) z[e] = 0.f;
      if (p.pxb) st_lane<E>(p.pxb + r * D, lane, z);
      else st_lane<E>(p.px + r * D, lane, z);
      if (lane == 0) {
        p.mean[r] = 0.f;
        p.rstd[r] = 0.f;
        p.nx[r] = 0.f;
        p.g[r] = 0.f;
        p.ion[r] = 0.f;
        p.kv[r] = 0.f;
        p.m2[r] = 0.f;
      }
      return;
    }
    float s = 0.f, q = 0.f;
#pragma unroll
    for (int e = 0; e < E; ++e) {
      s += xv[e];
      q += xv[e] * xv[e];
    }
    float acc = 0.f;
#pragma unroll
    for (int i = 0; i < HQ; ++i)
      if (lane + 64 * i < p.Dh) acc += silu_f(hv[i]) * w2v[i];
    wave_sum3_dpp(s, q, acc);
    const float mu = s * (1.0f / D);
    const float nrm = sqrtf(q);
    const float m2 = acc + b2;
    float v = 0.f;
#pragma unroll
    for (int e = 0; e < E; ++e) {
      const float t = xv[e] - mu;
      v += t * t;
    }
    const float inx = 1.0f / fmaxf(nrm, 1e-12f);
    const float z = lane < p.M ? sv * inx * p.inv_sqrt_d : -INFINITY;
    float zm = z;
    wave_sum_max_dpp(v, zm);
    const float rs = rsqrtf(v * (1.0f / D) + p.eps);
    float yv[E], gd = 0.f;
#pragma unroll
    for (int e = 0; e < E; ++e) {
      yv[e] = __builtin_fmaf((xv[e] - mu) * rs, wv[e], bv[e]);
      gd += yv[e] * gwv[e];
    }
    if (p.pxb) st_lane<E>(p.pxb + r * D, lane, yv);
    else st_lane<E>(p.px + r * D, lane, yv);
    const float ez = lane < p.M ? expf(z - zm) : 0.f;
    float se = ez;
    wave_sum2_dpp(gd, se);
    const float gate = sigmoid_f(gd + gbias);
    const float kv = wave_sum_dpp(lane < p.M ? ez / se * mv_l : 0.f);
    const float xval = cw0 * kv + cw1 * m2 + cb;
    if (p.part) {
      const float sc = gate * (xval > tx ? 1.f : 0.f);
      float xn[E];
#pragma unroll
      for (int e = 0; e < E; ++e) {
        xn[e] = __builtin_fmaf(sc, yv[e], xv[e]);
        csum[e] += xn[e];
      }
      if (p.xnew) st_lane<E>(p.xnew + r * D, lane, xn);
    }
    if (lane == 0) {
      p.mean[r] = mu;
      p.rstd[r] = rs;
      p.nx[r] = nrm;
      p.g[r] = gate;
      p.ion[r] = xval > tx ? 1.f : 0.f;
      p.kv[r] = kv;
      p.m2[r] = m2;
    }
  };
  if (p.part) {
    float* red = ni_s + (p.next_i ? (((p.rows + p.L - 1) / p.L + 3) & ~(int64_t)3) : 0);
    const int w = threadIdx.x >> 6;
    const int64_t nb = (p.rows + p.L - 1) / p.L, nc = (int64_t)nb * p.nchunk;
    for (int64_t cid = blockIdx.x; cid < nc; cid += gridDim.x) {
      const int64_t b = cid / p.nchunk, c = cid - b * p.nchunk;
      const int64_t r0 = b * p.L + c * 64, r1 = min(min(r0 + 64, (b + 1) * p.L), p.rows);
#pragma unroll
      for (int e = 0; e < E; ++e) csum[e] = 0.f;
      const bool act = r0 < r1 && at_layer(r0);
      if (act) {
        float xa[E], sa, ha[HQ];
        fetch(r0 + w, xa, sa, ha);
        for (int64_t r = r0 + w; r < r1; r += RW) {
          float xv[E], hv[HQ];
#pragma unroll
          for (int e = 0; e < E; ++e) xv[e] = xa[e];
#pragma unroll
          for (int i = 0; i < HQ; ++i) hv[i] = ha[i];
          const float sv = sa;
          fetch(r + RW < r1 ? r + RW : r0, xa, sa, ha);
          row_body(r, xv, sv, hv);
        }
      } else {
        float xv[E], hv[HQ];
        for (int64_t r = r0 + w; r < r1; r += RW) row_body(r, xv, 0.f, hv);
      }
      if (act) {
        st_lane<E>(red + w * D, lane, csum);
        __syncthreads();
        if (w == 0) {
          for (int k = 1; k < RW; ++k) {
            float t[E];
            ld_lane<E>(red + k * D, lane, t);
#pragma unroll
            for (int e = 0; e < E; ++e) csum[e] += t[e];
          }
        }
        __syncthreads();
      }
      if (w == 0) st_lane<E>(p.part + cid * D, lane, csum);
    }
    return;
  }
  const int64_t st = row_step();
  int64_t r = row_begin();
  float xa[E], xb[E], sa, sb, ha[HQ], hb[HQ];
  fetch(r, xa, sa, ha);
  fetch(r + st, xb, sb, hb);
  for (; r < p.rows; r += 2 * st) {
    {
      float xv[E], hv[HQ];
#pragma unroll
      for (int e = 0; e < E; ++e) xv[e] = xa[e];
#pragma unroll
      for (int i = 0; i < HQ; ++i) hv[i] = ha[i];
      const float sv = sa;
      fetch(r + 2 * st, xa, sa, ha);
      row_body(r, xv, sv, hv);
    }
    if (r + st >= p.rows) break;
    {
      float xv[E], hv[HQ];
#pragma unroll
      for (int e = 0; e < E; ++e) xv[e] = xb[e];
#pragma unroll
      for (int i = 0; i < HQ; ++i) hv[i] = hb[i];
      const float sv = sb;
      fetch(r + 3 * st, xb, sb, hb);
      row_body(r + st, xv, sv, hv);
    }
  }
}

struct MSRowBwd {
  const float *dpx;
  const float *x, *lnw, *lnb, *mean, *rstd;
  const float *dg, *g, *gw;
  const float *dion, *SH, *nx, *mval, *w2, *cw, *kv, *m2;
  float *dx;
  float *dlnw, *dlnb, *dgw, *dgb;
  float *dSH, *dmval, *dw2, *db2, *dcw, *dcb, *db1;
  int64_t rows, ldsh;
  int M, Dh;
  float inv_sqrt_d;
  const float* next_i;
  int layer;
  int64_t L;
};

template <int E>
__global__ __launch_bounds__(64 * RW) void msheath_row_bwd_kernel(MSRowBwd p) {
  constexpr int D = 64 * E;
  extern __shared__ float part[];
  const int lane = threadIdx.x & 63, wid = threadIdx.x >> 6;
  const int M = p.M, Dh = p.Dh;
  const int PN = M + 2 * Dh + 5;
  float* pw = part + RW * 3 * D + wid * PN;
  for (int j = lane; j < PN; j += 64) pw[j] = 0.f;
  float wv[E], bv[E], gwv[E], aw[E], ab[E], ag[E];
  ld_lane<E>(p.lnw, lane, wv);
  ld_lane<E>(p.lnb, lane, bv);
  ld_lane<E>(p.gw, lane, gwv);
#pragma unroll
  for (int e = 0; e < E; ++e) aw[e] = ab[e] = ag[e] = 0.f;
  const float mv_l = lane < M ? p.mval[lane] : 0.f;
  const float cw0 = p.cw[0], cw1 = p.cw[1];
  constexpr int HQ = (E + 1) / 2;
  struct Pre {
    float x[E], gp[E], dx[E], h[HQ];
    float s, gi, nx, g, dg, mu, rs, kv, m2;
  };
  const int ni_off = RW * (3 * D + PN);
  if (p.next_i) {
    const int nb = (int)((p.rows + p.L - 1) / p.L);
    for (int b = threadIdx.x; b < nb; b += 64 * RW) part[ni_off + b] = p.next_i[b];
  }
  __syncthreads();
  auto at_layer = [&](int64_t rr) __attribute__((always_inline)) -> bool {
    return !p.next_i || part[ni_off + (int)((unsigned)rr / (unsigned)p.L)] == (float)p.layer;
  };
  float w2v[HQ];
#pragma unroll
  for (int i = 0; i < HQ; ++i) w2v[i] = lane + 64 * i < Dh ? p.w2[lane + 64 * i] : 0.f;
  auto fetch = [&](int64_t rr, Pre& q) __attribute__((always_inline)) {
    const int64_t rc = (rr < p.rows && at_layer(rr)) ? rr : 0;
    const float* S = p.SH + rc * p.ldsh;
    q.s = S[lane < M ? lane : 0];
#pragma unroll
    for (int i = 0; i < HQ; ++i) q.h[i] = S[M + min(lane + 64 * i, Dh - 1)];
    ld_lane<E>(p.x + rc * D, lane, q.x);
    ld_lane<E>(p.dpx + rc * D, lane, q.gp);
    ld_lane<E>(p.dx + rc * D, lane, q.dx);
    q.gi = p.dion[rc];
    q.nx = p.nx[rc];
    q.g = p.g[rc];
    q.dg = p.dg[rc];
    q.mu = p.mean[rc];
    q.rs = p.rstd[rc];
    q.kv = p.kv[rc];
    q.m2 = p.m2[rc];
  };
  const int64_t st = row_step();
  int64_t r0 = row_begin();
  Pre pa, pb;
  fetch(r0, pa);
  fetch(r0 + st, pb);
  auto row_body = [&](int64_t r, Pre& q) __attribute__((always_inline)) {
    const Pre c = q;
    fetch(r + 2 * st, q);
    if (!at_layer(r)) {
      float* dz = p.dSH + r * p.ldsh;
      for (int j = lane; j < M + Dh; j += 64) dz[j] = 0.f;
      return;
    }
    const float gi = c.gi;
    const float nxr = c.nx;
    const float inx = 1.0f / fmaxf(nxr, 1e-12f);
    float* dS = p.dSH + r * p.ldsh;
    float* dh = dS + M;
    const float sl = c.s;
    const float z = lane < M ? sl * inx * p.inv_sqrt_d : -INFINITY;
    const float zm = wave_max_dpp(z);
    const float ez = lane < M ? expf(z - zm) : 0.f;
    const float key = ez / wave_sum_dpp(ez);
    const float dkv = gi * cw0, dm2 = gi * cw1;
    const float dkey = lane < M ? dkv * mv_l : 0.f;
    const float dot = wave_sum_dpp(key * dkey);
    const float dz = lane < M ? key * (dkey - dot) : 0.f;
    if (lane < M) {
      dS[lane] = dz * inx * p.inv_sqrt_d;
      pw[lane] += dkv * key;
    }
    const float dinx = wave_sum_dpp(lane < M ? dz * sl * p.inv_sqrt_d : 0.f);
    const float dnx = nxr > 1e-12f ? -dinx * inx * inx : 0.f;
#pragma unroll
    for (int i = 0; i < HQ; ++i) {
      const int j = lane + 64 * i;
      if (j < Dh) {
        const float hv = c.h[i];
        const float t = dm2 * w2v[i] * silu_grad(hv);
        dh[j] = t;
        pw[M + j] += dm2 * silu_f(hv);
        pw[M + Dh + j] += t;
      }
    }
    const float gg = c.g;
    const float dzg = c.dg * gg * (1.f - gg);
    if (lane == 0) {
      pw[M + 2 * Dh + 0] += dm2;
      pw[M + 2 * Dh + 1] += gi * c.kv;
      pw[M + 2 * Dh + 2] += gi * c.m2;
      pw[M + 2 * Dh + 3] += gi;
      pw[M + 2 * Dh + 4] += dzg;
    }
    float xv[E], gv[E];
#pragma unroll
    for (int e = 0; e < E; ++e) {
      xv[e] = c.x[e];
      gv[e] = c.gp[e];
    }
    const float mu = c.mu, rs = c.rs;
    const float cn = nxr > 0.f ? dnx / nxr : 0.f;
    float s1 = 0.f, s2 = 0.f, xh[E];
#pragma unroll
    for (int e = 0; e < E; ++e) {
      xh[e] = (xv[e] - mu) * rs;
      gv[e] += dzg * gwv[e];
      const float t = gv[e] * wv[e];
      s1 += t;
      s2 += t * xh[e];
      aw[e] += gv[e] * xh[e];
      ab[e] += gv[e];
      ag[e] += dzg * (xh[e] * wv[e] + bv[e]);
    }
    wave_sum2_dpp(s1, s2);
    s1 *= (1.0f / D);
    s2 *= (1.0f / D);
    float dv[E];
#pragma unroll
    for (int e = 0; e < E; ++e) dv[e] = c.dx[e] + rs * (gv[e] * wv[e] - s1 - xh[e] * s2) + cn * xv[e];
    st_lane<E>(p.dx + r * D, lane, dv);
  };
  for (int64_t r = r0; r < p.rows; r += 2 * st) {
    row_body(r, pa);
    if (r + st >= p.rows) break;
    row_body(r + st, pb);
  }
  float* pl = part + wid * 3 * D;
#pragma unroll
  for (int e = 0; e < E; ++e) {
    pl[lane_feat<E>(lane, e)] = aw[e];
    pl[D + lane_feat<E>(lane, e)] = ab[e];
    pl[2 * D + lane_feat<E>(lane, e)] = ag[e];
  }
  __syncthreads();
  for (int j = threadIdx.x; j < 3 * D; j += 64 * RW) {
    float a = 0.f;
#pragma unroll
    for (int ww = 0; ww < RW; ++ww) a += part[ww * 3 * D + j];
    atomicAdd(j < D ? p.dlnw + j : j < 2 * D ? p.dlnb + (j - D) : p.dgw + (j - 2 * D), a);
  }
  const float* pv = part + RW * 3 * D;
  for (int j = threadIdx.x; j < PN; j += 64 * RW) {
    float a = 0.f;
    for (int ww = 0; ww < RW; ++ww) a += pv[ww * PN + j];
    float* dst = j < M ? p.dmval + j
                 : j < M + Dh ? p.dw2 + (j - M)
                 : j < M + 2 * Dh ? p.db1 + (j - M - Dh)
                 : j == M + 2 * Dh ? p.db2
                 : j == M + 2 * Dh + 1 ? p.dcw
                 : j == M + 2 * Dh + 2 ? p.dcw + 1
                 : j == M + 2 * Dh + 3 ? p.dcb
                                       : p.dgb;
    atomicAdd(dst, a);
  }
}

template <typename TO = float>
__global__ __launch_bounds__(64 * RW) void tgate_fwd_kernel(const float* __restrict__ G, const float* __restrict__ c,
                                                            TO* __restrict__ out, int64_t rows, int D) {
  const int lane = threadIdx.x & 63;
  for (int64_t r = row_begin(); r < rows; r += row_step()) {
    const float c0 = c[r * 3], c1 = c[r * 3 + 1], c2 = c[r * 3 + 2];
    const float cm = fmaxf(c0, fmaxf(c1, c2));
    const float e0 = expf(c0 - cm), e1 = expf(c1 - cm), e2 = expf(c2 - cm);
    const float inv = 1.f / (e0 + e1 + e2);
    const float t0 = e0 * inv, t1 = e1 * inv, t2 = e2 * inv;
    const float* gr = G + r * 3 * D;
    for (int j = lane; j < D; j += 64) {
      const float v = __builtin_fmaf(gr[2 * D + j], t2, __builtin_fmaf(gr[D + j], t1, gr[j] * t0));
      if constexpr (sizeof(TO) == 4) out[r * D + j] = v;
      else out[r * D + j] = __builtin_bit_cast(unsigned short, (__bf16)v);
    }
  }
}

__global__ __launch_bounds__(64 * RW) void tgate_bwd_kernel(const float* __restrict__ dout, const float* __restrict__ G,
                                                            const float* __restrict__ c, float* __restrict__ dGz,
                                                            float* __restrict__ dc, int64_t rows, int D) {
  const int lane = threadIdx.x & 63;
  for (int64_t r = row_begin(); r < rows; r += row_step()) {
    const float c0 = c[r * 3], c1 = c[r * 3 + 1], c2 = c[r * 3 + 2];
    const float cm = fmaxf(c0, fmaxf(c1, c2));
    const float e0 = expf(c0 - cm), e1 = expf(c1 - cm), e2 = expf(c2 - cm);
    const float inv = 1.f / (e0 + e1 + e2);
    const float t0 = e0 * inv, t1 = e1 * inv, t2 = e2 * inv;
    const float* gr = G + r * 3 * D;
    float* dg = dGz + r * 3 * D;
    float a0 = 0.f, a1 = 0.f, a2 = 0.f;
    for (int j = lane; j < D; j += 64) {
      const float go = dout[r * D + j];
      const float g0 = gr[j], g1 = gr[D + j], g2 = gr[2 * D + j];
      a0 += go * g0;
      a1 += go * g1;
      a2 += go * g2;
      dg[j] = go * t0 * g0 * (1.f - g0);
      dg[D + j] = go * t1 * g1 * (1.f - g1);
      dg[2 * D + j] = go * t2 * g2 * (1.f - g2);
    }
    wave_sum3_dpp(a0, a1, a2);
    const float dot = t0 * a0 + t1 * a1 + t2 * a2;
    if (lane == 0) {
      dc[r * 3] = t0 * (a0 - dot);
// ... 1430 lines not shown
                   const float* b2, const float* cw, const float* cb, const float* tx, float* ion, float* xval,
                   float* kv, float* m2, int64_t rows, int64_t M, int64_t Dh, float inv_sqrt_d, hipStream_t stream) {
  ASRX_REQUIRE(M <= 64, "vgate: memory size must be <= 64");
  if (rows == 0) return 0;
  LAUNCH_ROWS(vgate_fwd_kernel, rows, 0, S, nx, mval, h, w2, b2, cw, cb, tx, ion, xval, kv, m2, rows, (int)M,
              (int)Dh, inv_sqrt_d);
  ASRX_LAUNCHED("asrx_vgate_fwd");
}

int asrx_vgate_bwd(const float* dion, const float* S, const float* nx, const float* mval, const float* h,
                   const float* w2, const float* cw, const float* kv, const float* m2, float* dS, float* dnx,
                   float* dh, float* dmval, float* dw2, float* db2, float* dcw, float* dcb, int64_t rows, int64_t M,
                   int64_t Dh, float inv_sqrt_d, hipStream_t stream) {
  if (rows == 0) return 0;
  const size_t shm = (size_t)RW * (M + Dh + 4) * sizeof(float);
  vgate_bwd_kernel<<<row_grid(rows, 1024), 64 * RW, shm, stream>>>(dion, S, nx, mval, h, w2, cw, kv, m2, dS, dnx, dh,
                                                                    dmval, dw2, db2, dcw, dcb, rows, (int)M, (int)Dh,
                                                                    inv_sqrt_d);
  ASRX_LAUNCHED("asrx_vgate_bwd");
}

int asrx_vgate_weights(const float* mkey, const float* W1, const float* b1, float* Wc, float* bc, float* mkn,
                       unsigned short* wb, int64_t M, int64_t Dh, int64_t D, hipStream_t stream) {
  if (M + Dh == 0) return 0;
  LAUNCH_ROWS(vgate_weights_kernel, M + Dh, 0, mkey, W1, b1, Wc, bc, mkn, wb, (int)M, (int)Dh, (int)D);
  ASRX_LAUNCHED("asrx_vgate_weights");
}

#define MS_DISPATCH(KER, GRID, SHM, P)                                             \
  switch (d) {                                                                     \
    case 128: KER<2><<<GRID, 64 * RW, SHM, stream>>>(P); break;                    \
    case 256: KER<4><<<GRID, 64 * RW, SHM, stream>>>(P); break;                    \
    case 384: KER<6><<<GRID, 64 * RW, SHM, stream>>>(P); break;                    \
    case 512: KER<8><<<GRID, 64 * RW, SHM, stream>>>(P); break;                    \
    case 768: KER<12><<<GRID, 64 * RW, SHM, stream>>>(P); break;                   \
    case 1024: KER<16><<<GRID, 64 * RW, SHM, stream>>>(P); break;                  \
    default: ASRX_REQUIRE(false, #KER ": d=%ld unsupported", (long)d);             \
  }

static bool ms_aligned(std::initializer_list<const void*> ps) {
  for (const void* q : ps)
    if ((uintptr_t)q & 7) return false;
  return true;
}

}
namespace asrx {
static bool g_row_nofill = false;
void set_msheath_row_nofill(bool on) { g_row_nofill = on; }
}
extern "C" {

int asrx_msheath_row_fwd2(const float* x, const float* lnw, const float* lnb, const float* gw, const float* gb,
                          const float* SH, int64_t ldsh, const float* mval, const float* w2, const float* b2,
                          const float* cw, const float* cb, const float* tx, void* px, int px_bf16, float* mean,
                          float* rstd, float* nx, float* g, float* ion, float* kv, float* m2, int64_t rows, int64_t d,
                          int64_t M, int64_t Dh, float eps, float inv_sqrt_d, const float* next_i, int64_t layer,
                          int64_t L, hipStream_t stream) {
  ASRX_REQUIRE(M <= 64 && ldsh >= M + Dh, "asrx_msheath_row_fwd: M <= 64 and ldsh >= M + Dh required");
  ASRX_REQUIRE(Dh <= 64 * ((d / 64 + 1) / 2), "asrx_msheath_row_fwd: v_gate hidden size Dh <= d / 2 required");
  ASRX_REQUIRE(ms_aligned({x, lnw, lnb, gw, (const float*)px}), "asrx_msheath_row_fwd: 8-byte aligned rows required");
  ASRX_REQUIRE(!next_i || L > 0, "asrx_msheath_row_fwd: L > 0 required with next_i");
  if (rows == 0) return 0;
  MSRowFwd p{x, lnw, lnb, gw, gb, SH, mval, w2, b2, cw, cb, tx, px_bf16 ? nullptr : (float*)px, mean, rstd, nx, g,
             ion, kv, m2, rows, ldsh, (int)M, (int)Dh, eps, inv_sqrt_d, next_i, (int)layer, L > 0 ? L : 1,
             px_bf16 ? (unsigned short*)px : nullptr, nullptr, nullptr, 0, asrx::g_row_nofill ? 1 : 0};
  const size_t shm = next_i ? (size_t)((rows + p.L - 1) / p.L) * sizeof(float) : 0;
  ASRX_REQUIRE(shm <= 48 * 1024, "msheath_row_fwd: %ld samples exceed the next_i LDS copy", (long)(shm / 4));
  MS_DISPATCH(msheath_row_fwd_kernel, row_grid(rows), shm, p);
  ASRX_LAUNCHED("asrx_msheath_row_fwd");
}

int asrx_msheath_row_fwd3(const float* x, const float* lnw, const float* lnb, const float* gw, const float* gb,
                          const float* SH, int64_t ldsh, const float* mval, const float* w2, const float* b2,
                          const float* cw, const float* cb, const float* tx, float* px, float* mean, float* rstd,
                          float* nx, float* g, float* ion, float* kv, float* m2, float* xnew, float* part, int64_t rows,
                          int64_t d, int64_t M, int64_t Dh, float eps, float inv_sqrt_d, const float* next_i,
                          int64_t layer, int64_t L, hipStream_t stream) {
  ASRX_REQUIRE(M <= 64 && ldsh >= M + Dh, "asrx_msheath_row_fwd3: M <= 64 and ldsh >= M + Dh required");
  ASRX_REQUIRE(Dh <= 64 * ((d / 64 + 1) / 2), "asrx_msheath_row_fwd3: v_gate hidden size Dh <= d / 2 required");
  ASRX_REQUIRE(ms_aligned({x, lnw, lnb, gw, (const float*)px, (const float*)xnew, (const float*)part}),
               "asrx_msheath_row_fwd3: 8-byte aligned rows required");
  ASRX_REQUIRE(part && L > 0 && rows % L == 0, "asrx_msheath_row_fwd3: part and rows = B L required");
  if (rows == 0) return 0;
  MSRowFwd p{x, lnw, lnb, gw, gb, SH, mval, w2, b2, cw, cb, tx, px, mean, rstd, nx, g, ion, kv, m2, rows, ldsh,
             (int)M, (int)Dh, eps, inv_sqrt_d, next_i, (int)layer, L, nullptr, part, xnew, (int)((L + 63) / 64),
             asrx::g_row_nofill ? 1 : 0};
  const size_t shm = (next_i ? (size_t)((rows / L + 3) & ~(int64_t)3) : 0) * sizeof(float) + (size_t)RW * d * sizeof(float);
  ASRX_REQUIRE(shm <= 48 * 1024, "msheath_row_fwd3: %ld samples exceed the next_i LDS copy", (long)(rows / L));
  const int64_t chunks = (rows / L) * p.nchunk;
  MS_DISPATCH(msheath_row_fwd_kernel, (unsigned)std::min<int64_t>(chunks, 65535), shm, p);
  ASRX_LAUNCHED("asrx_msheath_row_fwd3");
}

int asrx_msheath_row_fwd(const float* x, const float* lnw, const float* lnb, const float* gw, const float* gb,
                         const float* SH, int64_t ldsh, const float* mval, const float* w2, const float* b2,
                         const float* cw, const float* cb, const float* tx, float* px, float* mean, float* rstd,
                         float* nx, float* g, float* ion, float* kv, float* m2, int64_t rows, int64_t d, int64_t M,
                         int64_t Dh, float eps, float inv_sqrt_d, const float* next_i, int64_t layer, int64_t L,
                         hipStream_t stream) {
  return asrx_msheath_row_fwd2(x, lnw, lnb, gw, gb, SH, ldsh, mval, w2, b2, cw, cb, tx, px, 0, mean, rstd, nx, g, ion,
                               kv, m2, rows, d, M, Dh, eps, inv_sqrt_d, next_i, layer, L, stream);
}

int asrx_msheath_row_bwd(const float* dpx, const float* x, const float* lnw, const float* lnb, const float* mean,
                         const float* rstd, const float* dg, const float* g, const float* gw, const float* dion,
                         const float* SH, int64_t ldsh, const float* nx, const float* mval, const float* w2,
                         const float* cw, const float* kv, const float* m2, float* dx, float* dlnw, float* dlnb,
                         float* dgw, float* dgb, float* dSH, float* dmval, float* dw2, float* db2, float* dcw,
                         float* dcb, float* db1, int64_t rows, int64_t d, int64_t M, int64_t Dh, float inv_sqrt_d,
                         const float* next_i, int64_t layer, int64_t L, hipStream_t stream) {
  ASRX_REQUIRE(M <= 64 && ldsh >= M + Dh, "asrx_msheath_row_bwd: M <= 64 and ldsh >= M + Dh required");
  ASRX_REQUIRE(Dh <= 64 * ((d / 64 + 1) / 2), "asrx_msheath_row_bwd: v_gate hidden size Dh <= d / 2 required");
  ASRX_REQUIRE(ms_aligned({dpx, x, lnw, lnb, gw, dx}), "asrx_msheath_row_bwd: 8-byte aligned rows required");
  ASRX_REQUIRE(!next_i || L > 0, "asrx_msheath_row_bwd: L > 0 required with next_i");
  if (rows == 0) return 0;
  MSRowBwd p{dpx, x, lnw, lnb, mean, rstd, dg, g, gw, dion, SH, nx, mval, w2, cw, kv, m2, dx, dlnw, dlnb, dgw, dgb,
             dSH, dmval, dw2, db2, dcw, dcb, db1, rows, ldsh, (int)M, (int)Dh, inv_sqrt_d, next_i, (int)layer,
             L > 0 ? L : 1};
  const size_t nb = next_i ? (size_t)((rows + p.L - 1) / p.L) : 0;
  const size_t shm = ((size_t)RW * (3 * d + M + 2 * Dh + 5) + nb) * sizeof(float);
  ASRX_REQUIRE(shm <= 160 * 1024, "msheath_row_bwd: %ld samples exceed the LDS budget", (long)nb);
  MS_DISPATCH(msheath_row_bwd_kernel, row_grid(rows, 1024), shm, p);
  ASRX_LAUNCHED("asrx_msheath_row_bwd");
}
#undef MS_DISPATCH

int asrx_tgate_fwd2(const float* G, const float* c, void* out, int out_bf16, int64_t rows, int64_t D,
                    hipStream_t stream) {
  if (rows == 0) return 0;
  if (out_bf16)
    LAUNCH_ROWS(tgate_fwd_kernel<unsigned short>, rows, 0, G, c, (unsigned short*)out, rows, (int)D);
  else
    LAUNCH_ROWS(tgate_fwd_kernel<float>, rows, 0, G, c, (float*)out, rows, (int)D);
  ASRX_LAUNCHED("asrx_tgate_fwd");
}

int asrx_tgate_fwd(const float* G, const float* c, float* out, int64_t rows, int64_t D, hipStream_t stream) {
  return asrx_tgate_fwd2(G, c, out, 0, rows, D, stream);
}

int asrx_tgate_bwd(const float* dout, const float* G, const float* c, float* dGz, float* dc, int64_t rows, int64_t D,
                   hipStream_t stream) {
  if (rows == 0) return 0;
  LAUNCH_ROWS(tgate_bwd_kernel, rows, 0, dout, G, c, dGz, dc, rows, (int)D);
  ASRX_LAUNCHED("asrx_tgate_bwd");
}

int asrx_axpy_row(const float* x, const float* s, const float* y, float* out, int64_t rows, int64_t d,
                  hipStream_t stream) {
  if (rows == 0) return 0;
  if (d % 4 == 0 && rows * d / 4 < (1LL << 31) &&
      ((((uintptr_t)x | (uintptr_t)y | (uintptr_t)out) & 15) == 0)) {
    const int64_t n4 = rows * d / 4;
    axpy_row4_kernel<<<ew_grid((n4 + 1) / 2, 8192), 256, 0, stream>>>((const float4*)x, s, (const float4*)y,
                                                                      (float4*)out, (uint32_t)n4, (uint32_t)(d / 4));
  } else {
    LAUNCH_EW(axpy_row_kernel, rows * d, x, s, y, out, rows, (int)d);
  }
  ASRX_LAUNCHED("asrx_axpy_row");
}

int asrx_axpy_row_bwd(const float* g, const float* s, const float* y, float* dy, float* ds, int64_t rows, int64_t d,
                      hipStream_t stream) {
  if (rows == 0) return 0;
  LAUNCH_ROWS(axpy_row_bwd_kernel, rows, 0, g, s, y, dy, ds, rows, (int)d, (float*)nullptr);
  ASRX_LAUNCHED("asrx_axpy_row_bwd");
}

int asrx_axpy_row_bwd2(const float* g, const float* s, const float* y, float* dy, float* ds, float* dxc, int64_t rows,
                       int64_t d, hipStream_t stream) {
  if (rows == 0) return 0;
  LAUNCH_ROWS(axpy_row_bwd_kernel, rows, 0, g, s, y, dy, ds, rows, (int)d, dxc);
  ASRX_LAUNCHED("asrx_axpy_row_bwd2");
}

int asrx_jump_select(const float* xn, const float* orig, const float* xold, const float* act, const float* alpha,
                     const float* beta, const float* gam, float* out, int64_t B, int64_t L, int64_t d,
                     hipStream_t stream) {
  if (B * L == 0) return 0;
  LAUNCH_EW(jump_select_kernel, B * L * d, xn, orig, xold, act, alpha, beta, gam, out, B, L, (int)d);
  ASRX_LAUNCHED("asrx_jump_select");
}

int asrx_jump_select_bwd(const float* g, const float* xn, const float* orig, const float* act, const float* alpha,
                         const float* beta, float* dxn, float* dorig, float* dxold, float* dalpha, float* dbeta,
                         float* dgam, int64_t B, int64_t L, int64_t d, hipStream_t stream) {
  if (B * L == 0) return 0;
  dim3 grid((unsigned)((d + 63) / 64), (unsigned)B);
  jump_select_bwd_kernel<<<grid, 256, 0, stream>>>(g, xn, orig, act, alpha, beta, dxn, dorig, dxold, dalpha, dbeta,
                                                   dgam, L, (int)d);
  ASRX_LAUNCHED("asrx_jump_select_bwd");
}

int asrx_seg_colsum(const float* x, float* out, int64_t B, int64_t L, int64_t d, float scale, int accumulate,
                    hipStream_t stream) {
  if (B == 0) return 0;
  if (!accumulate) (void)hipMemsetAsync(out, 0, (size_t)B * d * sizeof(float), stream);
  const int64_t chunk = 64;
  dim3 grid((unsigned)((d + 63) / 64), (unsigned)B, (unsigned)((L + chunk - 1) / chunk));
  seg_colsum_kernel<<<grid, 256, 0, stream>>>(x, out, L, (int)d, scale, chunk);
  ASRX_LAUNCHED("asrx_seg_colsum");
}

int asrx_seg_colsum_det(const float* x, float* part, float* out, int64_t B, int64_t L, int64_t d, float scale,
                        hipStream_t stream) {
  if (B == 0) return 0;
  const int64_t chunk = 64, nchunk = (L + chunk - 1) / chunk;
// ... 312 lines not shown
```

### include/asrx.h

```cpp
#ifndef ASRX_H
#define ASRX_H
#include <stdint.h>

#ifdef __cplusplus
extern "C" {
#endif

typedef void* asrx_stream_t;

const char* asrx_last_error(void);
int asrx_abi_version(void);
uint32_t asrx_noise_hash(uint32_t key, uint32_t idx);
int asrx_set_noise_epoch(uint32_t epoch, asrx_stream_t stream);
int asrx_set_gemm_variant(int variant);
int asrx_set_attn_variant(int variant);
int asrx_set_wgrad_variant(int variant);

int asrx_mel_frames(int64_t n_samples);
int64_t asrx_logmel_ws_bytes(int64_t B, int64_t N);
int asrx_logmel(const float* wav, int64_t B, int64_t N, int64_t ld_wav, const float* consts,
                const float* fbw, const int* fbs, float* out, int layout, int64_t ld_out,
                void* ws, float* pool, int64_t T_pool, asrx_stream_t stream);
int asrx_wave_pool(const float* wav, int64_t B, int64_t N, int64_t ld_wav, int64_t T, float* out,
                   asrx_stream_t stream);
// ... 83 lines not shown
int asrx_layernorm_fwd(const float* x, const float* w, const float* b, float* y, float* mean, float* rstd,
                       int64_t rows, int64_t d, float eps, asrx_stream_t stream);
int asrx_layernorm_bwd(const float* dy, const float* x, const float* w, const float* mean, const float* rstd,
                       float* dx, float* dw, float* db, int64_t rows, int64_t d, asrx_stream_t stream);
int asrx_layernorm_bwd_acc(const float* dy, const float* x, const float* w, const float* mean, const float* rstd,
                           float* dx, float* dw, float* db, int64_t rows, int64_t d, int acc, asrx_stream_t stream);

int asrx_layernorm_fwd2(const float* x, const float* w, const float* b, float* y, float* mean, float* rstd,
                        float* nrm, const float* gw, const float* gb, float* gout, int gate_on_x, int64_t rows,
                        int64_t d, float eps, asrx_stream_t stream);
int asrx_layernorm_fwd3(const float* x, const float* w, const float* b, void* y, int y_bf16, float* mean, float* rstd,
                        float* nrm, const float* gw, const float* gb, float* gout, int gate_on_x, int64_t rows,
                        int64_t d, float eps, asrx_stream_t stream);

int asrx_small_linear_fwd(const float* x, const float* W, const float* b, float* y, int64_t rows, int64_t K,
                          int64_t N, int act, asrx_stream_t stream);
int asrx_small_linear_bwd(const float* dy, const float* y, const float* x, const float* W, float* dx, float* dW,
                          float* db, int64_t rows, int64_t K, int64_t N, int act, float beta,
                          asrx_stream_t stream);
int asrx_small_linear_fwd2(const void* x, int x_bf16, const float* W, const float* b, float* y, int64_t rows,
                           int64_t K, int64_t N, int act, asrx_stream_t stream);
int asrx_small_linear_bwd2(const float* dy, const float* y, const void* x, int x_bf16, const float* W, float* dx,
                           float* dW, float* db, int64_t rows, int64_t K, int64_t N, int act, float beta,
                           asrx_stream_t stream);

int asrx_rownorm(const float* x, float* n, int64_t rows, int64_t d, asrx_stream_t stream);
int asrx_rownorm_bwd(const float* dn, const float* x, const float* n, float* dx, int64_t rows, int64_t d,
                     asrx_stream_t stream);
int asrx_rownorm_bwd2(const float* dn, const float* x, const float* n, float* dx, int64_t rows, int64_t d, int acc,
                      asrx_stream_t stream);
int asrx_row_normalize(const float* x, float* y, float* n, int64_t rows, int64_t d, asrx_stream_t stream);
int asrx_row_normalize_bwd(const float* dy, const float* y, const float* n, float* dx, int64_t rows, int64_t d,
                           int acc, asrx_stream_t stream);
int asrx_softmax_small(const float* x, float* y, int64_t rows, int64_t N, asrx_stream_t stream);
int asrx_softmax_small_bwd(const float* g, const float* y, float* dx, int64_t rows, int64_t N, asrx_stream_t stream);
int asrx_zero(void* p, int64_t bytes, asrx_stream_t stream);

int asrx_rotary_fwd(const float* x, const float* m, const float* f, float* y, int64_t BL, int64_t L, int64_t D,
                    int64_t hd, float scale, asrx_stream_t stream);
int asrx_rotary_bwd(const float* g, const float* x, const float* m, const float* f, float* dx, float* dm,
                    int64_t BL, int64_t L, int64_t D, int64_t hd, float scale, asrx_stream_t stream);
int asrx_rotary_table(const float* f, float* tab, int64_t L, int64_t hd, asrx_stream_t stream);
int asrx_rotary_fwd2(const float* x, const float* m, const float* f, const float* tab, float* y, int64_t BL, int64_t L,
                     int64_t D, int64_t hd, float scale, asrx_stream_t stream);
int asrx_rotary_bwd2(const float* g, const float* x, const float* m, const float* f, const float* tab, float* dx,
                     float* dm, int64_t BL, int64_t L, int64_t D, int64_t hd, float scale, asrx_stream_t stream);

int asrx_vgate_fwd(const float* S, const float* nx, const float* mval, const float* h, const float* w2,
                   const float* b2, const float* cw, const float* cb, const float* tx, float* ion, float* xval,
                   float* kv, float* m2, int64_t rows, int64_t M, int64_t Dh, float inv_sqrt_d,
                   asrx_stream_t stream);
int asrx_vgate_bwd(const float* dion, const float* S, const float* nx, const float* mval, const float* h,
                   const float* w2, const float* cw, const float* kv, const float* m2, float* dS, float* dnx,
                   float* dh, float* dmval, float* dw2, float* db2, float* dcw, float* dcb, int64_t rows, int64_t M,
                   int64_t Dh, float inv_sqrt_d, asrx_stream_t stream);

int asrx_vgate_weights(const float* mkey, const float* W1, const float* b1, float* Wc, float* bc, float* mkn,
                       unsigned short* wb, int64_t M, int64_t Dh, int64_t D, asrx_stream_t stream);
int asrx_msheath_row_fwd(const float* x, const float* lnw, const float* lnb, const float* gw, const float* gb,
                         const float* SH, int64_t ldsh, const float* mval, const float* w2, const float* b2,
                         const float* cw, const float* cb, const float* tx, float* px, float* mean, float* rstd,
                         float* nx, float* g, float* ion, float* kv, float* m2, int64_t rows, int64_t d, int64_t M,
                         int64_t Dh, float eps, float inv_sqrt_d, const float* next_i, int64_t layer, int64_t L,
                         asrx_stream_t stream);
int asrx_msheath_row_fwd2(const float* x, const float* lnw, const float* lnb, const float* gw, const float* gb,
                          const float* SH, int64_t ldsh, const float* mval, const float* w2, const float* b2,
                          const float* cw, const float* cb, const float* tx, void* px, int px_bf16, float* mean,
                          float* rstd, float* nx, float* g, float* ion, float* kv, float* m2, int64_t rows, int64_t d,
                          int64_t M, int64_t Dh, float eps, float inv_sqrt_d, const float* next_i, int64_t layer,
                          int64_t L, asrx_stream_t stream);
int asrx_msheath_row_fwd3(const float* x, const float* lnw, const float* lnb, const float* gw, const float* gb,
                          const float* SH, int64_t ldsh, const float* mval, const float* w2, const float* b2,
                          const float* cw, const float* cb, const float* tx, float* px, float* mean, float* rstd,
                          float* nx, float* g, float* ion, float* kv, float* m2, float* xnew, float* part, int64_t rows,
                          int64_t d, int64_t M, int64_t Dh, float eps, float inv_sqrt_d, const float* next_i,
                          int64_t layer, int64_t L, asrx_stream_t stream);
int asrx_msheath_row_bwd(const float* dpx, const float* x, const float* lnw, const float* lnb, const float* mean,
                         const float* rstd, const float* dg, const float* g, const float* gw, const float* dion,
                         const float* SH, int64_t ldsh, const float* nx, const float* mval, const float* w2,
                         const float* cw, const float* kv, const float* m2, float* dx, float* dlnw, float* dlnb,
                         float* dgw, float* dgb, float* dSH, float* dmval, float* dw2, float* db2, float* dcw,
                         float* dcb, float* db1, int64_t rows, int64_t d, int64_t M, int64_t Dh, float inv_sqrt_d,
                         const float* next_i, int64_t layer, int64_t L, asrx_stream_t stream);

int asrx_tgate_fwd(const float* G, const float* c, float* out, int64_t rows, int64_t D, asrx_stream_t stream);
int asrx_tgate_fwd2(const float* G, const float* c, void* out, int out_bf16, int64_t rows, int64_t D,
                    asrx_stream_t stream);
int asrx_tgate_bwd(const float* dout, const float* G, const float* c, float* dGz, float* dc, int64_t rows,
                   int64_t D, asrx_stream_t stream);

int asrx_axpy_row(const float* x, const float* s, const float* y, float* out, int64_t rows, int64_t d,
                  asrx_stream_t stream);
int asrx_axpy_row_bwd(const float* g, const float* s, const float* y, float* dy, float* ds, int64_t rows,
                      int64_t d, asrx_stream_t stream);
int asrx_axpy_row_bwd2(const float* g, const float* s, const float* y, float* dy, float* ds, float* dxc,
                       int64_t rows, int64_t d, asrx_stream_t stream);
int asrx_jump_select(const float* xn, const float* orig, const float* xold, const float* act, const float* alpha,
                     const float* beta, const float* gam, float* out, int64_t B, int64_t L, int64_t d,
                     asrx_stream_t stream);
int asrx_jump_select_bwd(const float* g, const float* xn, const float* orig, const float* act, const float* alpha,
                         const float* beta, float* dxn, float* dorig, float* dxold, float* dalpha, float* dbeta,
                         float* dgam, int64_t B, int64_t L, int64_t d, asrx_stream_t stream);
int asrx_msheath_ctrl_fwd(const float* policy, const float* gpol, int64_t ld_gpol, const float* ion,
                          const float* mem_v, const float* mem_w, const float* mem, const float* jump_s,
                          const float* next_i, int64_t layer_i, int64_t layers, int64_t B, int64_t L, int64_t D,
                          float* alpha, float* beta, float* gam, float* mem_w_out, float* active, float* next_out,
                          void* rec, asrx_stream_t stream);
int asrx_msheath_ctrl_bwd(const float* g_alpha, const float* g_beta, const float* g_gam, const float* g_mwo,
                          const float* mem_v, const float* mem_w, const float* mem, const float* jump_s,
                          const void* rec, int64_t layer_i, int64_t layers, int64_t B, int64_t D, float* g_policy,
                          float* g_mem_v, float* g_mem_w, float* g_mem, float* g_jump_s, asrx_stream_t stream);
int64_t asrx_msheath_rec_bytes(void);
int asrx_msheath_ctrl_fwd2(const float* policy, const float* gpol, int64_t ld_gpol, const float* ion,
                           const float* mem_v, const float* mem_w, int64_t ld_mem_w, const float* mem,
                           const float* jump_s, const float* next_i, int64_t layer_i, int64_t layers, int64_t B,
                           int64_t L, int64_t D, float* alpha, float* beta, float* gam, float* mem_w_out, float* active,
                           float* next_out, void* rec, asrx_stream_t stream);
int asrx_msheath_ctrl_bwd2(const float* g_alpha, const float* g_beta, const float* g_gam, const float* g_mwo,
                           const float* mem_v, const float* mem_w, int64_t ld_mem_w, const float* mem,
                           const float* jump_s, const void* rec, int64_t layer_i, int64_t layers, int64_t B, int64_t D,
                           float* g_policy, int acc_policy, float* g_mem_v, float* g_mem_w, float* g_mem,
                           float* g_jump_s, int* has_orig, asrx_stream_t stream);
int asrx_msheath_ctrl_fwd3(const float* policy, const float* gpol, int64_t ld_gpol, const float* ion,
                           const float* mg_w, const float* mg_b, float* mem_v_out, const float* mem_w,
                           int64_t ld_mem_w, const float* mem_part, float* mem, const float* jump_s,
                           const float* next_i, int64_t layer_i, int64_t layers, int64_t B, int64_t L, int64_t D,
                           float* alpha, float* beta, float* gam, float* mem_w_out, float* active, float* next_out,
                           void* rec, asrx_stream_t stream);
int asrx_msheath_ctrl_bwd3(const float* g_alpha, const float* g_beta, const float* g_gam, const float* g_mwo,
                           const float* mem_v, const float* mem_w, int64_t ld_mem_w, const float* mem,
                           const float* jump_s, const void* rec, int64_t layer_i, int64_t layers, int64_t B, int64_t D,
                           float* g_policy, int acc_policy, float* g_mem_w, float* g_mem, float* g_jump_s,
                           int* has_orig, const float* mg_w, float* g_mg_w, float* g_mg_b, asrx_stream_t stream);
int64_t asrx_mem_chunks(int64_t L);
int asrx_axpy_row2_colsum(const float* x, const float* s1, const float* s2, const float* y, float* out, float* part,
                          int64_t B, int64_t L, int64_t d, const float* next_i, int64_t layer, asrx_stream_t stream);
int asrx_jump_select4_bwd_acc(const float* g, const float* xn, const float* orig, const float* act,
                              const float* alpha, const float* beta, const int* has_orig, float* dxn, float* dorig,
                              float* dx, float* dalpha, float* dbeta, float* dgam, int64_t B, int64_t L, int64_t d,
                              asrx_stream_t stream);
int asrx_axpy_row2_bwd_acc(const float* dxn, const float* gm, float invL, const float* act, const float* s1,
                           const float* s2, const float* y, float* dy, float* ds1, float* ds2, float* dx, int64_t B,
                           int64_t L, int64_t d, asrx_stream_t stream);
int64_t asrx_jump_bwd_part_floats(int64_t B, int64_t L, int64_t d);
int asrx_jump_select4_bwd_part(const float* g, const float* xn, const float* orig, const float* act,
                               const float* alpha, const float* beta, const int* has_orig, float* dxn, float* dorig,
                               float* dx, float* part, int64_t B, int64_t L, int64_t d, asrx_stream_t stream);
int asrx_msheath_ctrl_bwd4(const float* part, int64_t L, const float* g_mwo, const float* mem_v, const float* mem_w,
                           int64_t ld_mem_w, const float* mem, const float* jump_s, const void* rec, int64_t layer_i,
                           int64_t layers, int64_t B, int64_t D, float* g_policy, int acc_policy, float* g_mem_w,
                           float* g_mem, float* g_jump_s, int* has_orig, const float* mg_w, float* g_mg_w,
                           float* g_mg_b, asrx_stream_t stream);

int asrx_msheath_dx_final(float* dx, const float* dorig, const int* has_orig, const float* u, int64_t B, int64_t L,
                          int64_t d, asrx_stream_t stream);

typedef struct asrx_msheath_layer {
  const float *ln_w, *ln_b, *gate_w, *gate_b, *mval, *vw2, *vb2, *cw, *cb, *tx, *bc;
  const unsigned short *wcb;
  const unsigned short *ad_wb;
  const float *ad_b;
  int64_t M, Dh;
  float ln_eps;
  int32_t px_bf16;
} asrx_msheath_layer;
typedef struct asrx_msheath_plan {
  const unsigned short *p0_wb;
  const float *p0_b, *p2_w, *p2_b;
  int64_t p_hidden;
  const float *mem_w, *mg_w, *mg_b, *jump_s, *mln_w, *mln_b;
  float mln_eps;
  int32_t hln_bf16;
  const float *mgate_w, *mgate_b;
  const unsigned short *m0_wb;
  const float *m0_b;
  const unsigned short *m2_wb;
  const float *m2_b;
  int64_t H1;
  int32_t a1_bf16, n_layers;
  const asrx_msheath_layer* layers;
} asrx_msheath_plan;
int64_t asrx_msheath_plan_bytes(void);
int64_t asrx_msheath_layer_bytes(void);
int64_t asrx_msheath_fwd_ws_bytes(const asrx_msheath_plan* plan, int64_t B, int64_t L, int64_t D);
int asrx_msheath_fwd(const asrx_msheath_plan* plan, const float* x0, const float* gpol, int64_t ld_gpol, float* y,
                     void* ws, int64_t ws_bytes, int64_t B, int64_t L, int64_t D, asrx_stream_t stream);
int asrx_axpy_row2(const float* x, const float* s1, const float* s2, const float* y, float* out, int64_t rows,
                   int64_t d, asrx_stream_t stream);
int asrx_axpy_row2_bwd(const float* g, const float* s1, const float* s2, const float* y, float* dy, float* ds1,
                       float* ds2, int64_t rows, int64_t d, asrx_stream_t stream);
int asrx_jump_axpy_inplace(const float* xin, float* xout, const float* s1, const float* s2, const float* y,
                           const float* orig, const float* act, const float* alpha, const float* beta, const float* gam,
                           int64_t B, int64_t L, int64_t d, asrx_stream_t stream);
int asrx_jump_select4(const float* xn, const float* orig, const float* xold, const float* act, const float* alpha,
                      const float* beta, const float* gam, float* out, int64_t B, int64_t L, int64_t d,
                      asrx_stream_t stream);
int asrx_jump_select4_bwd(const float* g, const float* xn, const float* orig, const float* act, const float* alpha,
                          const float* beta, float* dxn, float* dorig, float* dxold, float* dalpha, float* dbeta,
                          float* dgam, int64_t B, int64_t L, int64_t d, asrx_stream_t stream);
int asrx_seg_colsum(const float* x, float* out, int64_t B, int64_t L, int64_t d, float scale, int accumulate,
                    asrx_stream_t stream);
int asrx_colsum(const float* x, float* out, int64_t rows, int64_t d, asrx_stream_t stream);
int asrx_seg_colsum_det(const float* x, float* part, float* out, int64_t B, int64_t L, int64_t d, float scale,
                        asrx_stream_t stream);
int asrx_colsum_ld(const float* x, int64_t ld, float* out, int64_t rows, int64_t d, asrx_stream_t stream);
int asrx_add_rows(const float* x, const float* t, const float* u, float* out, int64_t B, int64_t L, int64_t d,
                  asrx_stream_t stream);
int asrx_lincomb(const float* x, const float* y, const float* z, float a, float b, float c, float* out, int64_t n,
                 asrx_stream_t stream);
int asrx_policy_noise(float* out, int64_t B, int64_t layers, int64_t sid_base, uint32_t key,
                      asrx_stream_t stream);

int asrx_act_fwd(const float* x, float* y, int64_t n, int act, asrx_stream_t stream);
int asrx_act_bwd(const float* g, const float* x, float* dx, int64_t n, int act, asrx_stream_t stream);
int asrx_glu_fwd(const float* x, float* y, int64_t rows, int64_t C, asrx_stream_t stream);
int asrx_glu_bwd(const float* g, const float* x, float* dx, int64_t rows, int64_t C, asrx_stream_t stream);
int asrx_dropout(const float* x, float* y, int64_t B, int64_t T, int64_t C, int64_t sid_base, uint32_t key,
                 float p, asrx_stream_t stream);
int asrx_act_dropout_fwd(const float* z, const float* res, float* y, int64_t B, int64_t T, int64_t C,
                         int64_t sid_base, uint32_t key, float p, int act, int act2, asrx_stream_t stream);
int asrx_act_dropout_bwd(const float* g, const float* z, float* dz, int64_t B, int64_t T, int64_t C,
                         int64_t sid_base, uint32_t key, float p, int act, int act2, asrx_stream_t stream);
int asrx_dwconv_fwd(const float* x, const float* w, const float* b, float* y, int64_t B, int64_t T, int64_t C,
                    int64_t K, asrx_stream_t stream);
int asrx_dwconv_bwd(const float* g, const float* x, const float* w, float* dx, float* dw, float* db, int64_t B,
                    int64_t T, int64_t C, int64_t K, asrx_stream_t stream);
int asrx_dwconv_pre_bwd(const float* g, const float* x, const float* z, const float* w, float* dz, float* dw,
                        float* db, int64_t B, int64_t T, int64_t C, int64_t K, int pre, asrx_stream_t stream);
int asrx_bn_fwd(const float* x, const float* w, const float* b, float* y, float* mean, float* rstd, int64_t B,
                int64_t T, int64_t C, float eps, int use_batch_stats, asrx_stream_t stream);
int asrx_bn_bwd(const float* g, const float* x, const float* mean, const float* rstd, const float* w, float* sg_ws,
                float* sgx_ws, float* dx, float* dw, float* db, int64_t B, int64_t T, int64_t C,
                asrx_stream_t stream);
int asrx_bn_silu_fwd(const float* x, const float* w, const float* b, float* y, float* mean, float* rstd, int64_t B,
                     int64_t T, int64_t C, float eps, int use_batch_stats, asrx_stream_t stream);
int asrx_bn_silu_bwd(const float* g, const float* x, const float* mean, const float* rstd, const float* w,
                     const float* b, float* sg_ws, float* sgx_ws, float* dx, float* dw, float* db, int64_t B,
                     int64_t T, int64_t C, asrx_stream_t stream);
int asrx_stem1_fwd(const float* x, const float* W, const float* bias, float* y, int64_t B, int64_t T, int64_t D,
                   asrx_stream_t stream);
int asrx_stem1_bwd(const float* g, const float* x, float* dW, float* db, int64_t B, int64_t T, int64_t D,
                   asrx_stream_t stream);

int asrx_embed_fwd(const int64_t* ids, const float* E, float* y, int64_t rows, int64_t d, asrx_stream_t stream);
int asrx_embed_bwd(const int64_t* ids, const float* g, float* dE, int64_t rows, int64_t d, asrx_stream_t stream);
int asrx_ce_fwd(const float* z, const int64_t* labels, float* loss, float* lse, int64_t rows, int64_t V,
                asrx_stream_t stream);
int asrx_ce_bwd(const float* z, const int64_t* labels, const float* lse, const float* scale, float* dz,
                int64_t rows, int64_t V, asrx_stream_t stream);

int asrx_maxfactor_param_bytes(void);
int asrx_maxfactor_step(const void* table, int np, int64_t nrows, int64_t ncols, int64_t ncc, int64_t nmats,
                        int64_t nitems, float* ws, asrx_stream_t stream);
int asrx_maxfactor_step_ex(const void* table, int np, int64_t nrows, int64_t ncols, int64_t ncc, int64_t nmats,
                           int64_t nitems, float* ws, const float* ctl, int clip_any, asrx_stream_t stream);

int asrx_grad_stats_param_bytes(void);
int asrx_grad_stats(const void* table, int np, int64_t nitems, float inv_scale, float max_norm, float eps,
                    float* stats, float* ws, asrx_stream_t stream);


int asrx_ce_fwd1(const float* z, const int64_t* labels, float* loss_r, float* lse, float* loss, float* count,
                 int64_t rows, int64_t V, asrx_stream_t stream);
int asrx_ce_bwd2(const float* z, const int64_t* labels, const float* lse, const float* g, const float* count, float* dz,
                 int64_t rows, int64_t V, asrx_stream_t stream);
int asrx_gemm_wn_ce(const void* A, int64_t lda, const unsigned short* W, int64_t ldw, unsigned short* Zb, int64_t ldc,
                    float* part, int64_t M, int64_t N, int64_t K, int nj, asrx_stream_t stream);
int asrx_ce_part_fwd(const float* part, int64_t nparts, const unsigned short* zb, const int64_t* labels, float* loss_r,
                     float* lse, float* loss, float* count, int64_t rows, int64_t V, asrx_stream_t stream);
int asrx_ce_bwd_bf16(const unsigned short* zb, const int64_t* labels, const float* lse, const float* g,
                     const float* count, unsigned short* dzb, int64_t rows, int64_t V, asrx_stream_t stream);
int asrx_gemm_wn_ce_f32(const void* A, int64_t lda, const unsigned short* W, int64_t ldw, float* Zf, int64_t ldc,
                        float* part, int64_t M, int64_t N, int64_t K, int nj, asrx_stream_t stream);
int asrx_ce_part_fwd_f32(const float* part, int64_t nparts, const float* zf, const int64_t* labels, float* loss_r,
                         float* lse, float* loss, float* count, int64_t rows, int64_t V, asrx_stream_t stream);
int asrx_ce_bwd_f32in(const float* zf, const int64_t* labels, const float* lse, const float* g, const float* count,
                      unsigned short* dzb, int64_t rows, int64_t V, asrx_stream_t stream);
int asrx_gemm_wn_gact(const void* A, int a_bf16, int64_t lda, const unsigned short* W, int64_t ldw, const float* bias,
                      const float* G, int64_t ldg, unsigned short* gz, int64_t ldc, float* db, int64_t M, int64_t N,
                      int64_t K, int act, int nj, asrx_stream_t stream);
int asrx_gemm_wn_rot(const void* A, int a_bf16, int64_t lda, const unsigned short* W, int64_t ldw, float* C, float* Z,
                     int64_t ldc, const float* bias, const float* m, const float* tab, int64_t L, int64_t hd,
                     float scale, int64_t M, int64_t N, int64_t K, int nj, asrx_stream_t stream);
int asrx_gemm_lt(const void* A, int64_t lda, const unsigned short* W, int64_t ldw, void* C, int c_bf16, int64_t ldc,
                 const float* bias, int64_t M, int64_t N, int64_t K, float alpha, float beta, asrx_stream_t stream);
int asrx_gemm_wn_res(const float* A, int64_t lda, const unsigned short* W, int64_t ldw, float* C, int64_t ldc,
                     const float* bias, const float* R, int64_t ldr, int64_t M, int64_t N, int64_t K, int nj,
                     asrx_stream_t stream);
int asrx_act_bwd_bias(const float* g, const float* z, unsigned short* gz, float* db, int64_t rows, int64_t N, int act,
                      asrx_stream_t stream);
int asrx_wgrad_bf16_ab(const void* A, int64_t lda, const void* B, int b_bf16, int64_t ldb, float* C, int64_t ldc,
                       int64_t M, int64_t N, int64_t R, int64_t splitk, asrx_stream_t stream);
int asrx_wgrad_bias(const void* A, int a_bf16, int64_t lda, const void* B, int b_bf16, int64_t ldb, float* C,
                    int64_t ldc, float* db, int64_t M, int64_t N, int64_t R, int64_t splitk, asrx_stream_t stream);
int asrx_bn_running(const float* mean, const float* rstd, float* rm, float* rv, int64_t* nbt, int64_t B, int64_t C,
                    int64_t T, float eps, float momentum, asrx_stream_t stream);
int asrx_rsqrt_eps(const float* v, float* out, int64_t n, float eps, asrx_stream_t stream);
int asrx_conv3_weight(const float* g, const float* v, int64_t Co, int64_t Ci, float* Wt, unsigned short* Wtb, float* Wf,
                      unsigned short* Wfb, float* nrm, asrx_stream_t stream);
int asrx_conv3_weight_bwd(const float* dWt, const float* g, const float* v, const float* nrm, int64_t Co, int64_t Ci,
                          float* dg, float* dv, asrx_stream_t stream);
int asrx_blend_fwd(const float* d, const float* g, const float* blend, float* out, int64_t n, asrx_stream_t stream);
int asrx_blend_bwd(const float* go, const float* d, const float* g, const float* blend, float* dd, float* dg,
                   float* dblend, int64_t n, asrx_stream_t stream);
int asrx_add_segments(const float* src, int64_t n, float* d0, float* d1, float* d2, int64_t nseg, asrx_stream_t stream);
int asrx_cat3(const float* a, const float* b, const float* c, int64_t n, float* out, asrx_stream_t stream);


int asrx_pitch_dio(const float* x, int64_t ldx, int64_t B, int64_t N, double fs, double f0_floor, double f0_ceil,
                   double fp, double allowed_range, const double* lc, int64_t c, const double* nut,
                   const int64_t* nut_off, const int64_t* nut_len, const double* bf0, int64_t nb, double* mean,
                   double* hp, double* f, double* ev, int64_t cap, double* cand, double* score, double* work,
                   double* f0, int64_t F, asrx_stream_t stream);
int asrx_pitch_stonemask(const float* x, int64_t ldx, int64_t B, int64_t N, double fs, const double* f0, double fp,
                         int64_t F, double* out, asrx_stream_t stream);

#ifdef __cplusplus
}
#endif
#endif
```

Baseline: 5488 audio-sec/sec.

## Fuse msheath backward elementwise pass into row kernel and merge split weight-grad GEMMs

```diff
diff --git a/asr-model_amd/asrx/gemm.py b/asr-model_amd/asrx/gemm.py
--- a/asr-model_amd/asrx/gemm.py
+++ b/asr-model_amd/asrx/gemm.py
@@ -340,6 +340,17 @@
 
 FUSED_BIAS_GRAD = True
 BIAS_CHECK = None
+
+
+def _staged_f32_dy(A, lda, x2, M, K, rows):
+    if is_bf16(x2):
+        return None if (M % 4 or K % 8 or lda % 4 or x2.stride(0) != K or A.data_ptr() % 16) else 1
+    tiles = ((M + 127) // 128) * ((K + 127) // 128)
+    ok4 = M % 4 == 0 and K % 4 == 0 and lda % 4 == 0 and A.data_ptr() % 16 == 0 and x2.data_ptr() % 16 == 0
+    if prec.get() == prec.PREC_BF16 and ok4 and x2.stride(0) == K and (tiles <= 9 or rows <= 16384
+                                                                        or (rows <= 50000 and tiles <= 72)):
+        return 0
+    return None
 
 
 def _wgrad(A, lda, x2, out, M, K, rows, db=None):
@@ -386,13 +397,11 @@
         else:
             return staged(1, int(xb), "asrx_wgrad_bf16_ab", 2 + int(xb))
     if is_bf16(x2):
-        if M % 4 or K % 8 or lda % 4 or x2.stride(0) != K or A.data_ptr() % 16:
+        if _staged_f32_dy(A, lda, x2, M, K, rows) != 1:
             x2 = x2.float()
         else:
             return staged(0, 1, "asrx_wgrad_bf16_ex", 1)
-    ok4 = M % 4 == 0 and K % 4 == 0 and lda % 4 == 0 and A.data_ptr() % 16 == 0 and x2.data_ptr() % 16 == 0
-    if prec.get() == prec.PREC_BF16 and ok4 and x2.stride(0) == K and (tiles <= 9 or rows <= 16384
-                                                                        or (rows <= 50000 and tiles <= 72)):
+    if _staged_f32_dy(A, lda, x2, M, K, rows) == 0:
         return staged(0, 0, "asrx_wgrad_bf16")
     gemm(A, x2, out, M=M, N=K, K=rows, lda=lda, ldb=K, ldc=K, a_kc=False, b_kc=False, beta=1.0, splitk=sk)
     if db is not None:
@@ -403,6 +412,25 @@
 def wgrad_cols(dy, c0, n, x, out):
     rows, ld = dy.shape
     return _wgrad(dy[:, c0:], ld, x, out, n, x.shape[1], rows)
+
+
+def wgrad_cols2(dy, n0, out0, out1, x):
+    rows, n = dy.shape
+    K = x.shape[1]
+    n1 = n - n0
+    if not (0 < n0 < n and n0 % 4 == 0 and out0.stride(1) == 1 and out1.stride(1) == 1
+            and not is_bf16(dy) and _staged_f32_dy(dy, n, x, n0, K, rows) == 0
+            and _staged_f32_dy(dy[:, n0:], n, x, n1, K, rows) == 0):
+        wgrad_cols(dy, 0, n0, x, out0)
+        return wgrad_cols(dy, n0, n1, x, out1)
+    lib.require_gpu(dy, x, out0, out1)
+    tiles = ((n + 127) // 128) * ((K + 127) // 128)
+    sk = _splitk_for(rows, tiles)
+    e0 = probe.begin("gemm")
+    lib.call("asrx_wgrad_split", lib.ptr(dy), n, lib.ptr(x), 0, K, lib.ptr(out0), out0.stride(0),
+             lib.ptr(out1), out1.stride(0), n0, n, K, rows, sk, lib.stream())
+    probe.end("gemm", e0, 2.0 * n * K * rows, ("wgrad", n, K, rows, sk, "split"))
+    return out1
 
 
 def linear_wgrad(dy, x, out=None, accumulate=False, db=None):
diff --git a/asr-model_amd/asrx/lib.py b/asr-model_amd/asrx/lib.py
--- a/asr-model_amd/asrx/lib.py
+++ b/asr-model_amd/asrx/lib.py
@@ -70,6 +70,8 @@
     "asrx_vgate_weights": (_i32, [_p] * 7 + [_i64, _i64, _i64, _p]),
     "asrx_msheath_row_fwd": (_i32, [_p] * 6 + [_i64] + [_p] * 14 + [_i64] * 4 + [_f32, _f32, _p, _i64, _i64, _p]),
     "asrx_msheath_row_bwd": (_i32, [_p] * 11 + [_i64] + [_p] * 18 + [_i64] * 4 + [_f32, _p, _i64, _i64, _p]),
+    "asrx_msheath_row_bwd2": (_i32, [_i32, _p, _p, _p, _f32, _p] + [_p] * 11 + [_i64] + [_p] * 18 + [_i64] * 4
+                              + [_f32, _p, _i64, _i64, _p]),
     "asrx_gemm_wn_rows": (_i32, [_p, _i64, _p, _i64, _p, _i64, _p, _p, _i64, _i64, _i64, _f32, _f32, _i32, _i32, _p,
                                  _p, _p]),
     "asrx_row_tiles_max": (_i64, [_i64]),
@@ -111,6 +113,10 @@
     "asrx_msheath_ctrl_bwd4": (_i32, [_p, _i64, _p, _p, _p, _i64, _p, _p, _p, _i64, _i64, _i64, _i64, _p, _i32]
                                + [_p] * 8),
     "asrx_axpy_row2_bwd_acc": (_i32, [_p, _p, _f32, _p, _p, _p, _p, _p, _p, _p, _p, _i64, _i64, _i64, _p]),
+    "asrx_jump_select4_bwd_part2": (_i32, [_p] * 11 + [_i64, _i64, _i64, _p]),
+    "asrx_jump_select4_bwd_acc2": (_i32, [_p] * 13 + [_i64, _i64, _i64, _p]),
+    "asrx_axpy_row2_bwd_acc2": (_i32, [_p, _p, _p, _f32, _p, _p, _p, _p, _p, _p, _p, _p, _i64, _i64, _i64, _p]),
+    "asrx_wgrad_split": (_i32, [_p, _i64, _p, _i32, _i64, _p, _i64, _p, _i64, _i64, _i64, _i64, _i64, _i64, _p]),
     "asrx_msheath_dx_final": (_i32, [_p, _p, _p, _p, _i64, _i64, _i64, _p]),
     "asrx_axpy_row2": (_i32, [_p, _p, _p, _p, _p, _i64, _i64, _p]),
     "asrx_axpy_row2_bwd": (_i32, [_p, _p, _p, _p, _p, _p, _p, _i64, _i64, _p]),
diff --git a/asr-model_amd/asrx/msheath.py b/asr-model_amd/asrx/msheath.py
--- a/asr-model_amd/asrx/msheath.py
+++ b/asr-model_amd/asrx/msheath.py
@@ -20,6 +20,8 @@
 
 DETERMINISTIC = True
 ROW_COLSUM = __import__("os").environ.get("ASRX_ROW_COLSUM", "1") != "0"
+BWD_FUSED = __import__("os").environ.get("ASRX_MSHEATH_BWD_FUSED", "1") != "0"
+WGRAD_MERGED = __import__("os").environ.get("ASRX_MSHEATH_WGRAD_MERGED", "1") != "0"
 
 
 def _rec_bytes():
@@ -79,6 +81,7 @@
     a_r, a_b, a_d, a_c = wsr.data_ptr(), wsb.data_ptr(), wsd.data_ptr(), wsc.data_ptr()
     if save:
         sv["ws"] = (wsr, wsb, wsd, wsc)
+        sv["bwd_fused"] = BWD_FUSED
     inv_sqrt_d = 1.0 / math.sqrt(D)
     layers = []
     for i, lay in enumerate(mod.layers):
@@ -100,7 +103,8 @@
         ln, gt = lay["ln"], lay["gate"][0]
         ad = lay["adapter"]
         pxb = int(ad is not None and wide and prec.bf16_storage())
-        px = _E(B, L, D, device=dev, dtype=torch.bfloat16 if pxb else torch.float32)
+        no_px = save and BWD_FUSED and ad is None and ROW_COLSUM
+        px = None if no_px else _E(B, L, D, device=dev, dtype=torch.bfloat16 if pxb else torch.float32)
         mean, rstd, nx, gv, ion, kv, m2 = (a_r + 4 * rows * (7 * i + j) for j in range(7))
         x_new = _E(B, L, D, device=dev) if save else None
         if ad is None and ROW_COLSUM:
@@ -220,6 +224,7 @@
         g_mwo = None
         mg_w, mg_b = mod.mem_gate[0].weight, mod.mem_gate[0].bias
         inv_sqrt_d = 1.0 / math.sqrt(D)
+        fused = sv["bwd_fused"]
         for i in range(nl - 1, -1, -1):
             s = sv["layers"][i]
             lay = mod.layers[i]
@@ -228,13 +233,13 @@
             N = M + Dh
             xi = s["x"]
             dxi = _E(B, L, D, device=dev)
-            dxn = _E(B, L, D, device=dev)
+            dxn = None if fused else _E(B, L, D, device=dev)
             g_mem_w, g_mem = _E(B, D, device=dev), _E(B, D, device=dev)
             if DETERMINISTIC:
                 part = _E(int(lib.load().asrx_jump_bwd_part_floats(B, L, D)), device=dev)
-                lib.call("asrx_jump_select4_bwd_part", _P(dx), _P(s["x_new"]), _P(x0), _P(s["active"]),
-                         _P(s["alpha"]), _P(s["beta"]), _P(has_orig), _P(dxn), _P(dorig), _P(dxi), _P(part), B, L, D,
-                         st)
+                lib.call("asrx_jump_select4_bwd_part2" if fused else "asrx_jump_select4_bwd_part",
+                         _P(dx), _P(s["x_new"]), _P(x0), _P(s["active"]), _P(s["alpha"]), _P(s["beta"]), _P(has_orig),
+                         _P(dxn), _P(dorig), _P(dxi), _P(part), B, L, D, st)
                 lib.call("asrx_msheath_ctrl_bwd4", _P(part), L, _P(g_mwo), _P(s["mem_v"]), _P(s["mem_w"]),
                          s["ld_mw"], _P(s["mem"]), _P(mod.jump_s), _P(s["rec"]), i, nl, B, D, _P(g_policy),
                          int(i != nl - 1), _P(g_mem_w), _P(g_mem), _P(gb(mod.jump_s)), _P(has_orig), _P(mg_w),
@@ -242,19 +247,27 @@
             else:
                 dctl = _E(B * (2 + D), device=dev)
                 dalpha, dbeta, dgam = dctl[:B], dctl[B:2 * B], dctl[2 * B:]
-                lib.call("asrx_jump_select4_bwd_acc", _P(dx), _P(s["x_new"]), _P(x0), _P(s["active"]),
-                         _P(s["alpha"]), _P(s["beta"]), _P(has_orig), _P(dxn), _P(dorig), _P(dxi), _P(dalpha),
-                         _P(dbeta), _P(dgam), B, L, D, st)
+                lib.call("asrx_jump_select4_bwd_acc2" if fused else "asrx_jump_select4_bwd_acc",
+                         _P(dx), _P(s["x_new"]), _P(x0), _P(s["active"]), _P(s["alpha"]), _P(s["beta"]), _P(has_orig),
+                         _P(dxn), _P(dorig), _P(dxi), _P(dalpha), _P(dbeta), _P(dgam), B, L, D, st)
                 lib.call("asrx_msheath_ctrl_bwd3", _P(dalpha), _P(dbeta), _P(dgam), _P(g_mwo), _P(s["mem_v"]),
                          _P(s["mem_w"]), s["ld_mw"], _P(s["mem"]), _P(mod.jump_s), _P(s["rec"]), i, nl, B, D,
                          _P(g_policy), int(i != nl - 1), _P(g_mem_w), _P(g_mem), _P(gb(mod.jump_s)), _P(has_orig),
                          _P(mg_w), _P(gb(mg_w)), _P(gb(mg_b)), st)
-            dout = _E(B, L, D, device=dev)
-            dgv, dion = _E(rows, device=dev), _E(rows, device=dev)
-            lib.call("asrx_axpy_row2_bwd_acc", _P(dxn), _P(g_mem), 1.0 / L, _P(s["active"]), _P(s["g"]), _P(s["ion"]),
-                     _P(s["out"]), _P(dout), _P(dgv), _P(dion), _P(dxi), B, L, D, st)
+            ad = lay["adapter"]
+            mode = 2 if fused and ad is None else 0
+            dout = dgv = dion = None
+            if not fused:
+                dout = _E(B, L, D, device=dev)
+                dgv, dion = _E(rows, device=dev), _E(rows, device=dev)
+                lib.call("asrx_axpy_row2_bwd_acc", _P(dxn), _P(g_mem), 1.0 / L, _P(s["active"]), _P(s["g"]),
+                         _P(s["ion"]), _P(s["out"]), _P(dout), _P(dgv), _P(dion), _P(dxi), B, L, D, st)
+            elif ad is not None:
+                dout = _E(B, L, D, device=dev)
+                dgv, dion = _E(rows, device=dev), _E(rows, device=dev)
+                lib.call("asrx_axpy_row2_bwd_acc2", _P(dx), _P(s["alpha"]), _P(g_mem), 1.0 / L, _P(s["active"]),
+                         _P(s["g"]), _P(s["ion"]), _P(s["out"]), _P(dout), _P(dgv), _P(dion), _P(dxi), B, L, D, st)
             del dxn
-            ad = lay["adapter"]
             if ad is not None:
                 dpx = G.linear_dgrad(dout, ad.weight, mtiles=s["mt"])
                 G.linear_wgrad(dout, s["px"], out=gb(ad.weight), accumulate=True, db=gb(ad.bias))
@@ -262,21 +275,29 @@
                 dpx = dout
             ln, gt = lay["ln"], lay["gate"][0]
             dSH = _E(rows, N, device=dev)
-            lib.call("asrx_msheath_row_bwd", _P(dpx), _P(xi), _P(ln.weight), _P(ln.bias), _P(s["mean"]),
-                     _P(s["rstd"]), _P(dgv), _P(s["g"]), _P(gt.weight), _P(dion), _P(s["SH"]), N, _P(s["nx"]),
-                     _P(vg.mval), _P(vg.mlp[2].weight), _P(vg.concat.weight), _P(s["kv"]), _P(s["m2"]), _P(dxi),
-                     _P(gb(ln.weight)), _P(gb(ln.bias)), _P(gb(gt.weight)), _P(gb(gt.bias)), _P(dSH),
-                     _P(gb(vg.mval)), _P(gb(vg.mlp[2].weight)), _P(gb(vg.mlp[2].bias)), _P(gb(vg.concat.weight)),
-                     _P(gb(vg.concat.bias)), _P(gb(vg.mlp[0].bias)), rows, D, M, Dh, inv_sqrt_d, _P(s["next_i"]), i,
-                     L, st)
+            row_args = (_P(dpx), _P(xi), _P(ln.weight), _P(ln.bias), _P(s["mean"]), _P(s["rstd"]), _P(dgv), _P(s["g"]),
+                        _P(gt.weight), _P(dion), _P(s["SH"]), N, _P(s["nx"]), _P(vg.mval), _P(vg.mlp[2].weight),
+                        _P(vg.concat.weight), _P(s["kv"]), _P(s["m2"]), _P(dxi), _P(gb(ln.weight)), _P(gb(ln.bias)),
+                        _P(gb(gt.weight)), _P(gb(gt.bias)), _P(dSH), _P(gb(vg.mval)), _P(gb(vg.mlp[2].weight)),
+                        _P(gb(vg.mlp[2].bias)), _P(gb(vg.concat.weight)), _P(gb(vg.concat.bias)),
+                        _P(gb(vg.mlp[0].bias)), rows, D, M, Dh, inv_sqrt_d, _P(s["next_i"]), i, L, st)
+            if mode:
+                lib.call("asrx_msheath_row_bwd2", mode, _P(dx), _P(s["alpha"]), _P(g_mem),
+                         1.0 / L, _P(s["ion"]), *row_args)
+            else:
+                lib.call("asrx_msheath_row_bwd", *row_args)
             del dout, dpx
             G.linear_dgrad(dSH, s["Wc"], out=dxi, beta=1.0, mtiles=s["mt"])
             x2 = xi.view(rows, D)
             dmk = _E(M, D, device=dev)
             lib.call("asrx_zero", _P(dmk), dmk.numel() * 4, st)
-            G.wgrad_cols(dSH, 0, M, x2, dmk)
-            lib.call("asrx_row_normalize_bwd", _P(dmk), _P(s["Wc"]), _P(s["mkn"]), _P(gb(vg.mkey)), M, D, 1, st)
-            G.wgrad_cols(dSH, M, Dh, x2, gb(vg.mlp[0].weight))
+            if fused and WGRAD_MERGED:
+                G.wgrad_cols2(dSH, M, dmk, gb(vg.mlp[0].weight), x2)
+                lib.call("asrx_row_normalize_bwd", _P(dmk), _P(s["Wc"]), _P(s["mkn"]), _P(gb(vg.mkey)), M, D, 1, st)
+            else:
+                G.wgrad_cols(dSH, 0, M, x2, dmk)
+                lib.call("asrx_row_normalize_bwd", _P(dmk), _P(s["Wc"]), _P(s["mkn"]), _P(gb(vg.mkey)), M, D, 1, st)
+                G.wgrad_cols(dSH, M, Dh, x2, gb(vg.mlp[0].weight))
             del dSH, dmk
             g_mwo = g_mem_w
             dx = dxi
diff --git a/asr-model_amd/csrc/gemm_wg.hip b/asr-model_amd/csrc/gemm_wg.hip
--- a/asr-model_amd/csrc/gemm_wg.hip
+++ b/asr-model_amd/csrc/gemm_wg.hip
@@ -20,6 +20,9 @@
   int64_t R, kchunk;
   int splitk;
   float* db;
+  float* C2 = nullptr;
+  int64_t ldc2 = 0;
+  int msplit = 0;
 };
 
 __device__ __forceinline__ int off(int row, int ch) { return 256 * row + 16 * (ch ^ (((row & 3) << 2) | ((row >> 2) & 3))); }
@@ -164,7 +167,7 @@
   }
 }
 
-template <bool ABF, bool BBF>
+template <bool ABF, bool BBF, bool SPLIT = false>
 __global__ __launch_bounds__(NT, 2) void wgrad_wr_kernel(Params p) {
   __shared__ __attribute__((aligned(16))) char Ai[2][TK * TM * 2];
   __shared__ __attribute__((aligned(16))) char Bi[2][TK * TN * 2];
@@ -228,7 +231,12 @@
 #pragma unroll
       for (int r = 0; r < 4; ++r) {
         const int m = m0 + wm * 64 + mt * 16 + lm + r;
-        if (m < p.M && nk > 0) atomicAdd(p.C + (int64_t)m * p.ldc + n, acc[mt][nt][r]);
+        if constexpr (SPLIT) {
+          float* row = m < p.msplit ? p.C + (int64_t)m * p.ldc : p.C2 + (int64_t)(m - p.msplit) * p.ldc2;
+          if (m < p.M && nk > 0) atomicAdd(row + n, acc[mt][nt][r]);
+        } else {
+          if (m < p.M && nk > 0) atomicAdd(p.C + (int64_t)m * p.ldc + n, acc[mt][nt][r]);
+        }
       }
     }
   if (dbon && nk > 0) {
@@ -510,6 +518,30 @@
   return wgrad_launch(A, 1, lda, B, b_bf16, ldb, C, ldc, M, N, R, splitk, stream);
 }
 
+extern "C" int asrx_wgrad_split(const float* A, int64_t lda, const void* B, int b_bf16, int64_t ldb, float* C,
+                                int64_t ldc, float* C2, int64_t ldc2, int64_t msplit, int64_t M, int64_t N, int64_t R,
+                                int64_t splitk, hipStream_t stream) {
+  ASRX_REQUIRE(M > 0 && N > 0 && R >= 0, "asrx_wgrad_split: empty problem");
+  ASRX_REQUIRE(msplit > 0 && msplit < M && C && C2, "asrx_wgrad_split: 0 < msplit < M and both destinations required");
+  ASRX_REQUIRE(M % 4 == 0 && N % 4 == 0 && lda % 4 == 0 && ldb % 4 == 0, "asrx_wgrad_split: M, N, lda, ldb %% 4 required");
+  ASRX_REQUIRE(!b_bf16 || (N % 8 == 0 && ldb % 8 == 0), "asrx_wgrad_split: a bf16 X needs N, ldb %% 8");
+  ASRX_REQUIRE((((uintptr_t)A | (uintptr_t)B) & 15) == 0, "asrx_wgrad_split: operands must be 16-byte aligned");
+  if (R == 0) return 0;
+  if (splitk < 1) splitk = 1;
+  int64_t kchunk = (R + splitk - 1) / splitk;
+  kchunk = (kchunk + wg::TK - 1) / wg::TK * wg::TK;
+  splitk = (R + kchunk - 1) / kchunk;
+  wg::Params p{A, (const float*)B, C, lda, ldb, ldc, (int)M, (int)N, R, kchunk, (int)splitk, nullptr, C2, ldc2,
+               (int)msplit};
+  const int64_t items = ((M + wg::TM - 1) / wg::TM) * ((N + wg::TN - 1) / wg::TN) * splitk;
+  ASRX_REQUIRE(items < (1LL << 31), "asrx_wgrad_split: too many work items");
+  if (b_bf16)
+    wg::wgrad_wr_kernel<false, true, true><<<(unsigned)items, wg::NT, 0, stream>>>(p);
+  else
+    wg::wgrad_wr_kernel<false, false, true><<<(unsigned)items, wg::NT, 0, stream>>>(p);
+  ASRX_LAUNCHED("asrx_wgrad_split");
+}
+
 extern "C" int asrx_wgrad_bias(const void* A, int a_bf16, int64_t lda, const void* B, int b_bf16, int64_t ldb,
                                float* C, int64_t ldc, float* db, int64_t M, int64_t N, int64_t R, int64_t splitk,
                                hipStream_t stream) {
diff --git a/asr-model_amd/csrc/msheath.hip b/asr-model_amd/csrc/msheath.hip
--- a/asr-model_amd/csrc/msheath.hip
+++ b/asr-model_amd/csrc/msheath.hip
@@ -467,7 +467,7 @@
         sa += gv.x * u.x + gv.y * u.y + gv.z * u.z + gv.w * u.w;
         sb += gv.x * v.x + gv.y * v.y + gv.z * v.z + gv.w * v.w;
         sgv.x += gv.x; sgv.y += gv.y; sgv.z += gv.z; sgv.w += gv.w;
-        dxn[i] = make_float4(al * gv.x, al * gv.y, al * gv.z, al * gv.w);
+        if (dxn) dxn[i] = make_float4(al * gv.x, al * gv.y, al * gv.z, al * gv.w);
         if (jo) {
           float4 o = make_float4(be * gv.x, be * gv.y, be * gv.z, be * gv.w);
           if (acc_o) {
@@ -522,7 +522,8 @@
                                                                 const float* __restrict__ s1, const float* __restrict__ s2,
                                                                 const float4* __restrict__ y, float4* __restrict__ dy,
                                                                 float* __restrict__ ds1, float* __restrict__ ds2,
-                                                                float4* __restrict__ dx, int64_t rows, int64_t L, int d4) {
+                                                                float4* __restrict__ dx, int64_t rows, int64_t L, int d4,
+                                                                const float* __restrict__ alpha = nullptr) {
   const int lane = threadIdx.x & 63;
   const float4 z4 = make_float4(0.f, 0.f, 0.f, 0.f);
   for (int64_t r = (int64_t)blockIdx.x * 4 + (threadIdx.x >> 6); r < rows; r += (int64_t)gridDim.x * 4) {
@@ -538,9 +539,11 @@
     const float a = s1[r], c = s2 ? s2[r] : 1.f;
     const float sc = a * c;
     const float4* gm4 = reinterpret_cast<const float4*>(gm + b * 4 * d4);
+    const float al = alpha ? alpha[b] : 1.f;
     float t = 0.f;
     for (int j = lane; j < d4; j += 64) {
       float4 gv = dxn[r * d4 + j];
+      if (alpha) gv = make_float4(al * gv.x, al * gv.y, al * gv.z, al * gv.w);
       if (gm) {
         const float4 m = gm4[j];
         gv.x += m.x * invL; gv.y += m.y * invL; gv.z += m.z * invL; gv.w += m.w * invL;
@@ -635,6 +638,20 @@
   ASRX_LAUNCHED("asrx_jump_select4_bwd_part");
 }
 
+int asrx_jump_select4_bwd_part2(const float* g, const float* xn, const float* orig, const float* act,
+                                const float* alpha, const float* beta, const int* has_orig, float* dxn, float* dorig,
+                                float* dx, float* part, int64_t B, int64_t L, int64_t d, hipStream_t stream) {
+  return asrx_jump_select4_bwd_part(g, xn, orig, act, alpha, beta, has_orig, dxn, dorig, dx, part, B, L, d, stream);
+}
+
+int asrx_jump_select4_bwd_acc2(const float* g, const float* xn, const float* orig, const float* act,
+                               const float* alpha, const float* beta, const int* has_orig, float* dxn, float* dorig,
+                               float* dx, float* dalpha, float* dbeta, float* dgam, int64_t B, int64_t L, int64_t d,
+                               hipStream_t stream) {
+  return asrx_jump_select4_bwd_acc(g, xn, orig, act, alpha, beta, has_orig, dxn, dorig, dx, dalpha, dbeta, dgam, B, L,
+                                   d, stream);
+}
+
 int asrx_axpy_row2_bwd_acc(const float* dxn, const float* gm, float invL, const float* act, const float* s1,
                            const float* s2, const float* y, float* dy, float* ds1, float* ds2, float* dx, int64_t B,
                            int64_t L, int64_t d, hipStream_t stream) {
@@ -645,6 +662,19 @@
       (const float4*)dxn, gm, invL, act, s1, s2, (const float4*)y, (float4*)dy, ds1, ds2, (float4*)dx, rows, L,
       (int)(d / 4));
   ASRX_LAUNCHED("asrx_axpy_row2_bwd_acc");
+}
+
+int asrx_axpy_row2_bwd_acc2(const float* g, const float* alpha, const float* gm, float invL, const float* act,
+                            const float* s1, const float* s2, const float* y, float* dy, float* ds1, float* ds2,
+                            float* dx, int64_t B, int64_t L, int64_t d, hipStream_t stream) {
+  ASRX_REQUIRE(d % 4 == 0, "asrx_axpy_row2_bwd_acc2: d % 4 != 0");
+  ASRX_REQUIRE(alpha && dx, "asrx_axpy_row2_bwd_acc2: alpha and dx required");
+  const int64_t rows = B * L;
+  if (rows == 0) return 0;
+  axpy_row2_bwd_acc_kernel<<<(unsigned)std::min<int64_t>((rows + 3) / 4, 8192), 256, 0, stream>>>(
+      (const float4*)g, gm, invL, act, s1, s2, (const float4*)y, (float4*)dy, ds1, ds2, (float4*)dx, rows, L,
+      (int)(d / 4), alpha);
+  ASRX_LAUNCHED("asrx_axpy_row2_bwd_acc2");
 }
 
 int asrx_msheath_dx_final(float* dx, const float* dorig, const int* has_orig, const float* u, int64_t B, int64_t L,
diff --git a/asr-model_amd/csrc/rowops.hip b/asr-model_amd/csrc/rowops.hip
--- a/asr-model_amd/csrc/rowops.hip
+++ b/asr-model_amd/csrc/rowops.hip
@@ -627,7 +627,7 @@
 #pragma unroll
       for (int e = 0; e < E; ++e) z[e] = 0.f;
       if (p.pxb) st_lane<E>(p.pxb + r * D, lane, z);
-      else st_lane<E>(p.px + r * D, lane, z);
+      else if (p.px) st_lane<E>(p.px + r * D, lane, z);
       if (lane == 0) {
         p.mean[r] = 0.f;
         p.rstd[r] = 0.f;
@@ -671,7 +671,7 @@
       gd += yv[e] * gwv[e];
     }
     if (p.pxb) st_lane<E>(p.pxb + r * D, lane, yv);
-    else st_lane<E>(p.px + r * D, lane, yv);
+    else if (p.px) st_lane<E>(p.px + r * D, lane, yv);
     const float ez = lane < p.M ? expf(z - zm) : 0.f;
     float se = ez;
     wave_sum2_dpp(gd, se);
@@ -786,9 +786,11 @@
   const float* next_i;
   int layer;
   int64_t L;
+  const float *gj = nullptr, *alpha = nullptr, *gm = nullptr, *ion = nullptr;
+  float invL = 0.f;
 };
 
-template <int E>
+template <int E, int MODE = 0>
 __global__ __launch_bounds__(64 * RW) void msheath_row_bwd_kernel(MSRowBwd p) {
   constexpr int D = 64 * E;
   extern __shared__ float part[];
@@ -807,8 +809,8 @@
   const float cw0 = p.cw[0], cw1 = p.cw[1];
   constexpr int HQ = (E + 1) / 2;
   struct Pre {
-    float x[E], gp[E], dx[E], h[HQ];
-    float s, gi, nx, g, dg, mu, rs, kv, m2;
+    float x[E], gp[E], dx[E], gm[E], h[HQ];
+    float s, gi, nx, g, dg, mu, rs, kv, m2, al, ion;
   };
   const int ni_off = RW * (3 * D + PN);
   if (p.next_i) {
@@ -829,12 +831,23 @@
 #pragma unroll
     for (int i = 0; i < HQ; ++i) q.h[i] = S[M + min(lane + 64 * i, Dh - 1)];
     ld_lane<E>(p.x + rc * D, lane, q.x);
-    ld_lane<E>(p.dpx + rc * D, lane, q.gp);
-    ld_lane<E>(p.dx + rc * D, lane, q.dx);
-    q.gi = p.dion[rc];
+    if constexpr (MODE != 2) ld_lane<E>(p.dpx + rc * D, lane, q.gp);
+    if constexpr (MODE == 0) {
+      ld_lane<E>(p.dx + rc * D, lane, q.dx);
+    } else {
+      const int64_t bc = (int64_t)((unsigned)rc / (unsigned)p.L);
+      ld_lane<E>(p.gj + rc * D, lane, q.dx);
+      ld_lane<E>(p.gm + bc * D, lane, q.gm);
+      q.al = p.alpha[bc];
+    }
+    if constexpr (MODE == 2) {
+      q.ion = p.ion[rc];
+    } else {
+      q.gi = p.dion[rc];
+      q.dg = p.dg[rc];
+    }
     q.nx = p.nx[rc];
     q.g = p.g[rc];
-    q.dg = p.dg[rc];
     q.mu = p.mean[rc];
     q.rs = p.rstd[rc];
     q.kv = p.kv[rc];
@@ -853,7 +866,34 @@
       for (int j = lane; j < M + Dh; j += 64) dz[j] = 0.f;
       return;
     }
-    const float gi = c.gi;
+    float base[E], gpx[E];
+    float gi_r = 0.f, dg_r = 0.f;
+#pragma unroll
+    for (int e = 0; e < E; ++e) {
+      if constexpr (MODE == 0) {
+        base[e] = c.dx[e];
+      } else {
+        const float dxn = c.al * c.dx[e];
+        const float gmL = c.gm[e] * p.invL;
+        base[e] = dxn + gmL;
+      }
+      if constexpr (MODE != 2) gpx[e] = c.gp[e];
+    }
+    if constexpr (MODE == 2) {
+      float t = 0.f;
+#pragma unroll
+      for (int e = 0; e < E; ++e) t += base[e] * __builtin_fmaf((c.x[e] - c.mu) * c.rs, wv[e], bv[e]);
+      t = wave_sum_dpp(t);
+      const float sc = c.g * c.ion;
+      gi_r = c.g * t;
+      dg_r = c.ion * t;
+#pragma unroll
+      for (int e = 0; e < E; ++e) gpx[e] = sc * base[e];
+    } else {
+      gi_r = c.gi;
+      dg_r = c.dg;
+    }
+    const float gi = gi_r;
     const float nxr = c.nx;
     const float inx = 1.0f / fmaxf(nxr, 1e-12f);
     float* dS = p.dSH + r * p.ldsh;
@@ -885,7 +925,7 @@
       }
     }
     const float gg = c.g;
-    const float dzg = c.dg * gg * (1.f - gg);
+    const float dzg = dg_r * gg * (1.f - gg);
     if (lane == 0) {
       pw[M + 2 * Dh + 0] += dm2;
       pw[M + 2 * Dh + 1] += gi * c.kv;
@@ -897,7 +937,7 @@
 #pragma unroll
     for (int e = 0; e < E; ++e) {
       xv[e] = c.x[e];
-      gv[e] = c.gp[e];
+      gv[e] = gpx[e];
     }
     const float mu = c.mu, rs = c.rs;
     const float cn = nxr > 0.f ? dnx / nxr : 0.f;
@@ -918,7 +958,7 @@
     s2 *= (1.0f / D);
     float dv[E];
 #pragma unroll
-    for (int e = 0; e < E; ++e) dv[e] = c.dx[e] + rs * (gv[e] * wv[e] - s1 - xh[e] * s2) + cn * xv[e];
+    for (int e = 0; e < E; ++e) dv[e] = base[e] + rs * (gv[e] * wv[e] - s1 - xh[e] * s2) + cn * xv[e];
     st_lane<E>(p.dx + r * D, lane, dv);
   };
   for (int64_t r = r0; r < p.rows; r += 2 * st) {
@@ -2515,6 +2555,7 @@
   ASRX_REQUIRE(ms_aligned({x, lnw, lnb, gw, (const float*)px, (const float*)xnew, (const float*)part}),
                "asrx_msheath_row_fwd3: 8-byte aligned rows required");
   ASRX_REQUIRE(part && L > 0 && rows % L == 0, "asrx_msheath_row_fwd3: part and rows = B L required");
+  ASRX_REQUIRE(px || xnew, "asrx_msheath_row_fwd3: px or xnew required");
   if (rows == 0) return 0;
   MSRowFwd p{x, lnw, lnb, gw, gb, SH, mval, w2, b2, cw, cb, tx, px, mean, rstd, nx, g, ion, kv, m2, rows, ldsh,
              (int)M, (int)Dh, eps, inv_sqrt_d, next_i, (int)layer, L, nullptr, part, xnew, (int)((L + 63) / 64),
@@ -2557,6 +2598,47 @@
   MS_DISPATCH(msheath_row_bwd_kernel, row_grid(rows, 1024), shm, p);
   ASRX_LAUNCHED("asrx_msheath_row_bwd");
 }
+
+#define MS_DISPATCH_MODE(MODE, GRID, SHM, P)                                                        \
+  switch (d) {                                                                                      \
+    case 128: msheath_row_bwd_kernel<2, MODE><<<GRID, 64 * RW, SHM, stream>>>(P); break;            \
+    case 256: msheath_row_bwd_kernel<4, MODE><<<GRID, 64 * RW, SHM, stream>>>(P); break;            \
+    case 384: msheath_row_bwd_kernel<6, MODE><<<GRID, 64 * RW, SHM, stream>>>(P); break;            \
+    case 512: msheath_row_bwd_kernel<8, MODE><<<GRID, 64 * RW, SHM, stream>>>(P); break;            \
+    case 768: msheath_row_bwd_kernel<12, MODE><<<GRID, 64 * RW, SHM, stream>>>(P); break;           \
+    case 1024: msheath_row_bwd_kernel<16, MODE><<<GRID, 64 * RW, SHM, stream>>>(P); break;          \
+    default: ASRX_REQUIRE(false, "asrx_msheath_row_bwd2: d=%ld unsupported", (long)d);              \
+  }
+
+int asrx_msheath_row_bwd2(int mode, const float* gj, const float* alpha, const float* gm, float invL,
+                          const float* ion, const float* dpx, const float* x, const float* lnw, const float* lnb,
+                          const float* mean, const float* rstd, const float* dg, const float* g, const float* gw,
+                          const float* dion, const float* SH, int64_t ldsh, const float* nx, const float* mval,
+                          const float* w2, const float* cw, const float* kv, const float* m2, float* dx, float* dlnw,
+                          float* dlnb, float* dgw, float* dgb, float* dSH, float* dmval, float* dw2, float* db2,
+                          float* dcw, float* dcb, float* db1, int64_t rows, int64_t d, int64_t M, int64_t Dh,
+                          float inv_sqrt_d, const float* next_i, int64_t layer, int64_t L, hipStream_t stream) {
+  if (mode == 0)
+    return asrx_msheath_row_bwd(dpx, x, lnw, lnb, mean, rstd, dg, g, gw, dion, SH, ldsh, nx, mval, w2, cw, kv, m2, dx,
+                                dlnw, dlnb, dgw, dgb, dSH, dmval, dw2, db2, dcw, dcb, db1, rows, d, M, Dh, inv_sqrt_d,
+                                next_i, layer, L, stream);
+  ASRX_REQUIRE(mode == 2, "asrx_msheath_row_bwd2: mode 0 or 2");
+  ASRX_REQUIRE(M <= 64 && ldsh >= M + Dh, "asrx_msheath_row_bwd2: M <= 64 and ldsh >= M + Dh required");
+  ASRX_REQUIRE(Dh <= 64 * ((d / 64 + 1) / 2), "asrx_msheath_row_bwd2: v_gate hidden size Dh <= d / 2 required");
+  ASRX_REQUIRE(gj && alpha && gm && L > 0 && rows % L == 0, "asrx_msheath_row_bwd2: gj, alpha, gm and rows = B L required");
+  ASRX_REQUIRE(ion, "asrx_msheath_row_bwd2: mode 2 reads ion");
+  ASRX_REQUIRE(ms_aligned({gj, gm, dpx, x, lnw, lnb, gw, dx}), "asrx_msheath_row_bwd2: 8-byte aligned rows required");
+  if (rows == 0) return 0;
+  MSRowBwd p{dpx, x, lnw, lnb, mean, rstd, dg, g, gw, dion, SH, nx, mval, w2, cw, kv, m2, dx, dlnw, dlnb, dgw, dgb,
+             dSH, dmval, dw2, db2, dcw, dcb, db1, rows, ldsh, (int)M, (int)Dh, inv_sqrt_d, next_i, (int)layer, L,
+             gj, alpha, gm, ion, invL};
+  const size_t nb = next_i ? (size_t)(rows / L) : 0;
+  const size_t shm = ((size_t)RW * (3 * d + M + 2 * Dh + 5) + nb) * sizeof(float);
+  ASRX_REQUIRE(shm <= 160 * 1024, "msheath_row_bwd2: %ld samples exceed the LDS budget", (long)nb);
+  MS_DISPATCH_MODE(2, row_grid(rows, 1024), shm, p);
+  ASRX_LAUNCHED("asrx_msheath_row_bwd2");
+}
+#undef MS_DISPATCH_MODE
 #undef MS_DISPATCH
 
 int asrx_tgate_fwd2(const float* G, const float* c, void* out, int out_bf16, int64_t rows, int64_t D,
diff --git a/include/asrx.h b/include/asrx.h
--- a/include/asrx.h
+++ b/include/asrx.h
@@ -189,6 +189,14 @@
                          float* dgw, float* dgb, float* dSH, float* dmval, float* dw2, float* db2, float* dcw,
                          float* dcb, float* db1, int64_t rows, int64_t d, int64_t M, int64_t Dh, float inv_sqrt_d,
                          const float* next_i, int64_t layer, int64_t L, asrx_stream_t stream);
+int asrx_msheath_row_bwd2(int mode, const float* gj, const float* alpha, const float* gm, float invL,
+                          const float* ion, const float* dpx, const float* x, const float* lnw, const float* lnb,
+                          const float* mean, const float* rstd, const float* dg, const float* g, const float* gw,
+                          const float* dion, const float* SH, int64_t ldsh, const float* nx, const float* mval,
+                          const float* w2, const float* cw, const float* kv, const float* m2, float* dx, float* dlnw,
+                          float* dlnb, float* dgw, float* dgb, float* dSH, float* dmval, float* dw2, float* db2,
+                          float* dcw, float* dcb, float* db1, int64_t rows, int64_t d, int64_t M, int64_t Dh,
+                          float inv_sqrt_d, const float* next_i, int64_t layer, int64_t L, asrx_stream_t stream);
 
 int asrx_tgate_fwd(const float* G, const float* c, float* out, int64_t rows, int64_t D, asrx_stream_t stream);
 int asrx_tgate_fwd2(const float* G, const float* c, void* out, int out_bf16, int64_t rows, int64_t D,
@@ -253,6 +261,16 @@
 int asrx_jump_select4_bwd_part(const float* g, const float* xn, const float* orig, const float* act,
                                const float* alpha, const float* beta, const int* has_orig, float* dxn, float* dorig,
                                float* dx, float* part, int64_t B, int64_t L, int64_t d, asrx_stream_t stream);
+int asrx_jump_select4_bwd_part2(const float* g, const float* xn, const float* orig, const float* act,
+                                const float* alpha, const float* beta, const int* has_orig, float* dxn, float* dorig,
+                                float* dx, float* part, int64_t B, int64_t L, int64_t d, asrx_stream_t stream);
+int asrx_jump_select4_bwd_acc2(const float* g, const float* xn, const float* orig, const float* act,
+                               const float* alpha, const float* beta, const int* has_orig, float* dxn, float* dorig,
+                               float* dx, float* dalpha, float* dbeta, float* dgam, int64_t B, int64_t L, int64_t d,
+                               asrx_stream_t stream);
+int asrx_axpy_row2_bwd_acc2(const float* g, const float* alpha, const float* gm, float invL, const float* act,
+                            const float* s1, const float* s2, const float* y, float* dy, float* ds1, float* ds2,
+                            float* dx, int64_t B, int64_t L, int64_t d, asrx_stream_t stream);
 int asrx_msheath_ctrl_bwd4(const float* part, int64_t L, const float* g_mwo, const float* mem_v, const float* mem_w,
                            int64_t ld_mem_w, const float* mem, const float* jump_s, const void* rec, int64_t layer_i,
                            int64_t layers, int64_t B, int64_t D, float* g_policy, int acc_policy, float* g_mem_w,
@@ -400,6 +418,9 @@
                        int64_t M, int64_t N, int64_t R, int64_t splitk, asrx_stream_t stream);
 int asrx_wgrad_bias(const void* A, int a_bf16, int64_t lda, const void* B, int b_bf16, int64_t ldb, float* C,
                     int64_t ldc, float* db, int64_t M, int64_t N, int64_t R, int64_t splitk, asrx_stream_t stream);
+int asrx_wgrad_split(const float* A, int64_t lda, const void* B, int b_bf16, int64_t ldb, float* C, int64_t ldc,
+                     float* C2, int64_t ldc2, int64_t msplit, int64_t M, int64_t N, int64_t R, int64_t splitk,
+                     asrx_stream_t stream);
 int asrx_bn_running(const float* mean, const float* rstd, float* rm, float* rv, int64_t* nbt, int64_t B, int64_t C,
                     int64_t T, float eps, float momentum, asrx_stream_t stream);
 int asrx_rsqrt_eps(const float* v, float* out, int64_t n, float eps, asrx_stream_t stream);
```

After: 5554 audio-sec/sec (median of 6 runs). 1.01x the previous value.
